# Annatk26/wire

Hardware: AMD Instinct MI355X
Metric: coord-samples/sec fwd+bwd, 4x256 complex WIRE MLP (higher is better)
Workload: dtype f32 (2xfp16 split operands with power-of-two scales, f16 MFMA, fp32 accumulate)

## Files before the change

wire_amd/csrc/wire_api.hip:

```cpp
#include <cmath>
#include <cstdarg>
#include <cstdio>
#include <string>

#include "wire_plan.h"

static thread_local std::string g_err;
int fail(int code, const char* fmt, ...) {
  char buf[512];
  va_list ap;
  va_start(ap, fmt);
  vsnprintf(buf, sizeof buf, fmt, ap);
  va_end(ap);
  g_err = buf;
  return code;
}
int wire_fail_(int code, const char* msg) { return fail(code, "%s", msg); }

extern "C" int wire_abi_version(void) { return WIRE_ABI_VERSION; }
extern "C" const char* wire_last_error(void) { return g_err.c_str(); }

std::mutex g_prof_mu;
std::atomic<bool> g_prof_on{false};
std::vector<ProfRec> g_prof_recs;
std::vector<std::pair<hipEvent_t, hipEvent_t>> g_prof_pool;

extern "C" int wire_prof_enable(int on) {
  std::lock_guard<std::mutex> lk(g_prof_mu);
  g_prof_on.store(on != 0);
  return WIRE_OK;
}
extern "C" int wire_prof_read(double* ms_total, int64_t* launches, double* flops_total) {
  std::lock_guard<std::mutex> lk(g_prof_mu);
  for (int i = 0; i < WIRE_PROF_CLASSES; ++i) { ms_total[i] = 0; launches[i] = 0; flops_total[i] = 0; }
  for (auto& r : g_prof_recs) {
    float ms = 0.f;
    if (hipEventSynchronize(r.b) == hipSuccess && hipEventElapsedTime(&ms, r.a, r.b) == hipSuccess) {
      ms_total[r.cls] += ms; launches[r.cls] += 1; flops_total[r.cls] += r.flops;
    }
    g_prof_pool.emplace_back(r.a, r.b);
  }
  g_prof_recs.clear();
  return WIRE_OK;
}

WireFamily wire_family_(int kind) {
  if (knob(K_SPLIT_BF16)) return FAM_X3;
  return (kind == WIRE_KIND_WIRE && knob(K_COMPLEX_3M)) ? FAM_3M : FAM_4M;
}
extern "C" int wire_tune_get(const char* key) {
  if (!key) return fail(WIRE_ERR_ARG, "null key");
  const int v = knob_get(key);
  return v >= 0 ? v : fail(WIRE_ERR_ARG, "unknown tuning key: %s", key);
}
extern "C" int wire_tune_set(const char* key, int value) {
  if (!key) return fail(WIRE_ERR_ARG, "null key");
  if (knob_set(key, value) == 0 || (g_glds_tune && g_glds_tune(key, value) == 0)) return WIRE_OK;
  return fail(WIRE_ERR_ARG, "unknown tuning key or bad value: %s=%d", key, value);
}

hipError_t layer_nt(hipStream_t s, const Plan& p, WireFamily f, const float* packed, int l, bool dg, int epi,
                    const float* A, int64_t n, GemmEpiParams ep, const unsigned* amax_a, const unsigned* amax_b,
                    unsigned* amax_out) {
  const int Pin = l == 0 ? p.Pin0 : p.P, Nc = dg ? Pin : p.Pl, Kd = dg ? p.Pl : Pin;
  switch (f) {
    case FAM_X2:
      ep.amax_a = amax_a; ep.amax_b = amax_b; ep.amax_out = amax_out;
      return launch_gemmx2h_nt(s, epi, A, Kd, packed + (dg ? p.off_dg_x2 : p.off_fwd_x2)[l], n, Nc, Kd, ep,
                               x2_waits(p.k_nt_bfirst, p.k_epi_early));
    case FAM_3M:
      return launch_gemm3m_nt(s, epi, A, Kd, packed + (dg ? p.off_dg_3m : p.off_fwd_3m)[l], Kd, n, Nc / 2, Kd / 2, ep);
    case FAM_X3: return launch_gemmx3_nt(s, epi, A, Kd, packed + (dg ? p.off_dg_x3 : p.off_fwd_x3)[l], n, Nc, Kd, ep);
    default: return launch_gemm_nt(s, epi, A, Kd, packed + (dg ? p.off_dg : p.off_fwd)[l], Kd, n, Nc, Kd, ep);
  }
}

int pack_hidden(hipStream_t s, const Plan& p, const void* const* params, float* packed, const std::vector<const float*>& hW,
                const std::vector<const float*>& hb) {
  for (int l0 = 1; l0 <= p.L; l0 += PACK_MAXB) {
    const int nb = (p.L - l0 + 1) < PACK_MAXB ? (p.L - l0 + 1) : PACK_MAXB;
    PackBatch pb{}, p3{};
    X3SplitBatch sf{}, sd{};
    for (int i = 0; i < nb; ++i) {
      const int l = l0 + i;
      pb.W[i] = hW[l];
      pb.b[i] = hb[l];
      pb.V[i] = p.per_layer == 4 ? (const float*)params[p.per_layer * l + 2] : nullptr;
      pb.c[i] = p.per_layer == 4 ? (const float*)params[p.per_layer * l + 3] : nullptr;
      pb.fwd[i] = packed + p.off_fwd[l]; pb.dg[i] = packed + p.off_dg[l]; pb.bias[i] = packed + p.off_bias[l];
      sf.src[i] = packed + p.off_fwd[l]; sf.dst[i] = packed + p.off_fwd_x3[l];
      sd.src[i] = packed + p.off_dg[l]; sd.dst[i] = packed + p.off_dg_x3[l];
      if (p.off_fwd_3m[l] >= 0) {
        p3.W[i] = pb.W[i]; p3.b[i] = pb.b[i];
        p3.fwd[i] = packed + p.off_fwd_3m[l]; p3.dg[i] = packed + p.off_dg_3m[l]; p3.bias[i] = packed + p.off_bias[l];
      }
    }
    HIPCHK(launch_pack_hidden_batch(s, p.kind, pb, nb, p.K, p.K, p.P, p.P, p.ws));
    if (p.Pl == p.P) {
      for (int i = 0; i < nb; ++i) { sf.src[nb + i] = sd.src[i]; sf.dst[nb + i] = sd.dst[i]; }
      HIPCHK(launch_x3_split_b_batch(s, sf, 2 * nb, p.P, p.Pl, p.P));
    } else {
      HIPCHK(launch_x3_split_b_batch(s, sf, nb, p.P, p.Pl, p.P));
      HIPCHK(launch_x3_split_b_batch(s, sd, nb, p.Pl, p.P, p.Pl));
    }
    if (p.off_fwd_3m[l0] >= 0)
      HIPCHK(launch_pack3m_batch(s, p3, nb, p.K, p.K, p.Kp, p.Kp));
    {
      X2AmaxBatch ab{};
      X2SplitBatch xf{}, xd{};
      for (int i = 0; i < nb; ++i) {
        const int l = l0 + i;
        unsigned* slots = reinterpret_cast<unsigned*>(packed + p.off_wamax + (int64_t)l * WIRE_AMAX_SLOTS);
        ab.src[i] = packed + p.off_fwd[l]; ab.slots[i] = slots;
        xf.src[i] = packed + p.off_fwd[l]; xf.dst[i] = packed + p.off_fwd_x2[l]; xf.slots[i] = slots;
        xd.src[i] = packed + p.off_dg[l]; xd.dst[i] = packed + p.off_dg_x2[l]; xd.slots[i] = slots;
      }
      HIPCHK(launch_amax_batch(s, ab, nb, (int64_t)p.Pl * p.P));
      HIPCHK(launch_x2_split_b_batch(s, xf, nb, p.P, p.Pl, p.P));
      HIPCHK(launch_x2_split_b_batch(s, xd, nb, p.Pl, p.P, p.Pl));
      for (int k = 0; k < p.S2 && p.off_fx >= 0 && fused_pre_scale(p.kind, p.w, pass_c(p, k)) > 0.f; ++k) {
        FxSplitBatch fx{};
        for (int i = 0; i < nb; ++i) {
          const int l = l0 + i;
          fx.src[i] = packed + p.off_fwd[l];
          fx.dst[i] = packed + fx_pass_off(p, k) + (int64_t)(l - 1) * fused_b_image_floats(p.P);
          fx.slots[i] = ab.slots[i];
        }
        HIPCHK(launch_fx_split_b_batch(s, fx, nb, p.P, p.P, fused_pre_scale(p.kind, p.w, pass_c(p, k))));
      }
      if (p.off_fxd >= 0) {
        FxSplitBatch fd{};
        int m = 0;
        for (int i = 0; i < nb; ++i) {
          const int l = l0 + i;
          fd.src[m] = packed + p.off_dg[l];
          fd.dst[m] = packed + p.off_fxd + (int64_t)(p.L - l) * fused_b_image_floats(p.P);
          fd.slots[m] = ab.slots[i];
          ++m;
        }
        if (m > 0) HIPCHK(launch_fx_split_b_batch(s, fd, m, p.Pl, p.P, 1.f));
      }
    }
  }
  return WIRE_OK;
}

extern "C" int wire_pack_params(void* stream, const wire_net_desc* d, const void* const* params,
                                float* packed) {
  Plan p; if (int rc = make_plan(d, p)) return rc;
  if (!params || !packed) return fail(WIRE_ERR_ARG, "null pointer");
  hipStream_t s = (hipStream_t)stream;
  ProfScope ps(s, 3, 0);
  for (int i = 0; i < p.ntens; ++i)
    if (!params[i]) return fail(WIRE_ERR_ARG, "params[%d] is null", i);
  HIPCHK(hipMemsetAsync(packed + p.off_wamax, 0, (size_t)(p.L + 1) * WIRE_AMAX_SLOTS * sizeof(float), s));
  if (p.first_gemm) {
    const float* W = (const float*)params[p.t0];
    const float* b = (const float*)params[p.t0 + 1];
    HIPCHK(launch_pack_hidden(s, p.kind, W, b, nullptr, nullptr, p.K, p.Din, p.P, p.Pin0, packed + p.off_fwd[0],
                              packed + p.off_dg[0], packed + p.off_bias[0]));
    HIPCHK(launch_x3_split_b(s, packed + p.off_fwd[0], p.Pin0, p.Pl, p.Pin0, packed + p.off_fwd_x3[0]));
    HIPCHK(launch_x3_split_b(s, packed + p.off_dg[0], p.Pl, p.Pin0, p.Pl, packed + p.off_dg_x3[0]));
    if (p.off_fx >= 0) {
      unsigned* slots0 = reinterpret_cast<unsigned*>(packed + p.off_wamax);
      HIPCHK(launch_amax(s, packed + p.off_fwd[0], (int64_t)p.Pl * p.Pin0, slots0));
      FxSplitBatch f0{};
      f0.src[0] = packed + p.off_fwd[0]; f0.dst[0] = packed + p.off_fx; f0.slots[0] = slots0;
      HIPCHK(launch_fx_split_b_batch(s, f0, 1, p.Pin0, p.P, 1.f, p.Pin0));
    }
    if (p.ms) {
      X2AmaxBatch ab{};
      X2SplitBatch xf{};
      ab.src[0] = xf.src[0] = packed + p.off_fwd[0];
      ab.slots[0] = reinterpret_cast<unsigned*>(packed + p.off_wamax);
      xf.dst[0] = packed + p.off_fwd_x2[0]; xf.slots[0] = ab.slots[0];
      HIPCHK(launch_amax_batch(s, ab, 1, (int64_t)p.Pl * p.Pin0));
      HIPCHK(launch_x2_split_b_batch(s, xf, 1, p.Pin0, p.Pl, p.Pin0));
    }
  }
  if (p.hier) return hier_pack(s, p, params, packed);
  if (p.mfn) return mfn_pack(s, p, params, packed);
  std::vector<const float*> hW(p.L + 1, nullptr), hb(p.L + 1, nullptr);
  for (int l = 1; l <= p.L; ++l) {
    hW[l] = (const float*)params[p.t0 + p.per_layer * l]; hb[l] = (const float*)params[p.t0 + p.per_layer * l + 1];
  }
  if (int rc = pack_hidden(s, p, params, packed, hW, hb)) return rc;
  HIPCHK(launch_pack_final(s, p.kind, (const float*)params[p.ntens - 2],
                           (const float*)params[p.ntens - 1], p.K, p.P, p.O, packed + p.off_wf,
                           packed + p.off_bf));
  if (!p.first_gemm || p.ms)
    for (int q = 0; q < p.per_layer; ++q) {
      if (q == 0 && p.ws != 1.f) {
        HIPCHK(launch_scale_copy(s, (const float*)params[first_tensor(p, 0)], p.tfloats[first_tensor(p, 0)], p.ws,
                                 packed + first_native_off(p, 0)));
        continue;
      }
      HIPCHK(hipMemcpyAsync(packed + first_native_off(p, q), params[first_tensor(p, q)], p.tfloats[first_tensor(p, q)] * 4,
                            hipMemcpyDeviceToDevice, s));
    }
  if (p.m2) {
    const M2Comb w = comb_of(p, packed);
    const float* dst[4] = {w.W1, w.b1, w.W2, w.b2};
    for (int q = 0; q < 4; ++q)
      HIPCHK(hipMemcpyAsync(const_cast<float*>(dst[q]), params[q], p.tfloats[q] * 4, hipMemcpyDeviceToDevice, s));
  }
  return WIRE_OK;
}

static FusedFwdParams fused_params(const Plan& p, const float* packed, const float* coords, int64_t n) {
  FusedFwdParams fp;
  fp.coords = coords; fp.n = n;
  if (p.first_gemm) {
    fp.pe_F = p.F; fp.bias0 = packed + p.off_bias[0]; fp.wamax0 = wamax_of(p, packed, 0);
  } else {
    fp.W0 = packed + first_native_off(p, 0); fp.b0 = packed + first_native_off(p, 1);
  }
  fp.wimg = reinterpret_cast<const unsigned char*>(packed + p.off_fx);
  fp.bias = packed + p.off_bias[1]; fp.bias_stride = p.L >= 2 ? p.off_bias[2] - p.off_bias[1] : 0;
  fp.wamax = wamax_of(p, packed, 1); fp.wamax_stride = WIRE_AMAX_SLOTS;
  fp.D = p.D; fp.K = p.K; fp.L = p.L; fp.O = p.O; fp.w1 = p.w1; fp.w = p.w; fp.s = p.s;
  fp.c_first = fused_pre_scale(p.kind, p.w1, p.s); fp.c_hidden = fused_pre_scale(p.kind, p.w, p.s);
  fp.k2_first = p.s * p.s * 1.44269502f / (fp.c_first * fp.c_first);
  fp.k2 = p.s * p.s * 1.44269502f / (fp.c_hidden * fp.c_hidden);
  return fp;
}

static int mlp_fwd_core(void* stream, const Plan& p, const Route& r, const float* packed, const float* coords, int64_t n,
                        float* y, void* act, int64_t act_bytes, const FusedFwdParams* loss = nullptr) {
  const bool save = r.mode != MODE_INFER;
  if (n < 0) return fail(WIRE_ERR_ARG, "negative n");
  if (n == 0) return WIRE_OK;
  if (!packed || !coords || (!r.fuse && !y) || !act) return fail(WIRE_ERR_ARG, "null pointer");
  const ActLayout a = act_layout(p, n, save);
  if (act_bytes < a.total * 4) return fail(WIRE_ERR_SIZE, "act buffer %lld < %lld bytes",
                                           (long long)act_bytes, (long long)a.total * 4);
  hipStream_t s = (hipStream_t)stream;
  float* A = (float*)act;
  if (r.fused_fwd) {
    FusedFwdParams fp = fused_params(p, packed, coords, n);
    fp.wf = packed + p.off_wf; fp.bfr = packed + p.off_bf; fp.y = y;
    if (p.m2) {
      for (int k = 0; k < p.S2; ++k) {
        FusedFwdParams f = fp;
        f.wimg = reinterpret_cast<const unsigned char*>(packed + fx_pass_off(p, k));
        f.s = pass_c(p, k);
        f.c_first = fused_pre_scale(p.kind, p.w1, f.s); f.c_hidden = fused_pre_scale(p.kind, p.w, f.s);
        f.y = A + a.ytr + (int64_t)k * n * p.O;
        ProfScope ps(s, 0, 2.0 * n * p.Pl * p.P * p.L);
        HIPCHK(launch_fused_fwd(s, p.kind, p.P, f));
      }
      ProfScope ps(s, 3, 0);
      HIPCHK(launch_m2_comb_fwd(s, comb_of(p, packed), p.S2, p.O, A + a.ytr, n, y));
      return WIRE_OK;
    }
    ProfScope ps(s, 0, 2.0 * n * p.Pl * p.P * p.L);
    HIPCHK(launch_fused_fwd(s, p.kind, p.P, fp));
    return WIRE_OK;
  }
  unsigned* const amax = reinterpret_cast<unsigned*>(A + a.amax);
  if (r.fam == FAM_X2)
    HIPCHK(hipMemsetAsync(amax, 0, (size_t)(p.L + 2 + (p.ms ? 1 : 0)) * WIRE_AMAX_SLOTS * sizeof(unsigned), s));
  unsigned* const pe_amax = reinterpret_cast<unsigned*>(A + a.pe_amax);
  if (p.ms) {
    MscaleC c{};
    for (int g = 0; g < p.T; ++g) c.c[g] = p.sc_c[g];
    ProfScope ps(s, 3, 0);
    HIPCHK(launch_mscale_first(s, coords, n, p.D, packed + first_native_off(p, 0), packed + first_native_off(p, 1), p.SHF,
                               c, p.ms_split, p.Pin0, r.pe_split,
                               r.fam0 == FAM_X2 && r.pe_split == 0.f ? pe_amax : nullptr, A + a.pe));
  } else if (p.first_gemm) {
    ProfScope ps(s, 3, 0);
    HIPCHK(launch_posenc(s, coords, n, p.D, p.F, p.Pin0, A + a.pe));
  }
  if (r.fused_train) {
    FusedFwdParams fp = fused_params(p, packed, coords, n);
    fp.inv_c_first = 1.f / fp.c_first; fp.inv_c_hidden = 1.f / fp.c_hidden;
    fp.lin0 = p.cplx ? nullptr : A + a.lin0;
    fp.lin = p.kind == WIRE_KIND_RELU ? nullptr : A + a.lin1; fp.lin_stride = a.np * p.Pl;
    fp.out = A + a.out0; fp.out_stride = a.np * p.P;
    fp.amax_out = amax;
    fp.rstore = r.rstore ? 1 : 0;
    if (r.fused_final) {
      fp.wf = packed + p.off_wf; fp.bfr = packed + p.off_bf;
      fp.target = loss->target; fp.idx = loss->idx; fp.first = loss->first; fp.gscale = loss->gscale;
      fp.y = loss->y; fp.rec = loss->rec; fp.g_lin = loss->g_lin; fp.part_w = loss->part_w; fp.part_b = loss->part_b;
      fp.loss_partial = loss->loss_partial; fp.amax_g = loss->amax_g;
    }
    ProfScope ps(s, 0, 2.0 * n * p.Pl * p.P * p.L);
    HIPCHK(launch_fused_fwd(s, p.kind, p.P, fp));
    return WIRE_OK;
  }
  auto out_l = [&](int l) { return save ? A + a.out0 + (int64_t)l * a.np * p.P : A + ((l & 1) ? a.pong : a.ping); };
  auto lin_l = [&](int l) -> float* {
    if (!save || p.kind == WIRE_KIND_RELU) return nullptr;
    return l == 0 ? A + a.lin0 : A + a.lin1 + (int64_t)(l - 1) * a.np * p.Pl;
  };
  auto at = [](float* b, int64_t off) -> float* { return b ? b + off : nullptr; };
  for (int k = 0; k < p.S2; ++k) {
    const float ck = pass_c(p, k);
    const int64_t ro = (int64_t)k * n;
    if (p.first_gemm) {
      GemmEpiParams ep; ep.bias = packed + p.off_bias[0]; ep.o0 = lin_l(0); ep.o1 = out_l(0);
      ep.ld0 = p.Pl; ep.ld1 = p.P; ep.omega = p.w1; ep.scale = p.s; ep.kvalid = p.K;
      if (r.fam == FAM_X2) ep.amax_out = amax;
      if (r.pe_split != 0.f) ep.a_split_inv = 1.f / r.pe_split;
      ProfScope ps(s, 0, 2.0 * n * p.Pl * p.Pin0);
      HIPCHK(layer_nt(s, p, r.fam0, packed, 0, false, epi_fwd(p.kind), A + a.pe, n, ep, pe_amax, wamax_of(p, packed, 0),
                      amax));
    } else {
      auto first = [&](int q) { return q < p.per_layer ? packed + first_native_off(p, q) : nullptr; };
      ProfScope ps(s, 3, 0);
      HIPCHK(launch_first_fwd(s, p.kind, coords, n, p.D, first(0), first(1), first(2), first(3), p.K, p.P, p.w1, ck,
                              p.cplx ? nullptr : at(lin_l(0), ro * p.P), out_l(0) + ro * p.P,
                              r.fam == FAM_X2 ? amax : nullptr));
    }
    for (int l = 1; l <= p.L; ++l) {
      GemmEpiParams ep; ep.bias = packed + p.off_bias[l]; ep.o0 = at(lin_l(l), ro * p.Pl); ep.o1 = out_l(l) + ro * p.P;
      ep.ld0 = p.Pl; ep.ld1 = p.P; ep.omega = p.w; ep.scale = ck; ep.kvalid = p.K;
      if (r.skip_out_L && l == p.L) ep.o1 = nullptr;
      const float s_in = r.out_scale[l - 1], s_out = r.out_scale[l];
      if (s_in != 0.f) ep.a_split_inv = 1.f / s_in;
      if (s_out != 0.f) ep.o1_split = s_out;
      ProfScope ps(s, 0, 2.0 * n * p.Pl * p.P);
      HIPCHK(layer_nt(s, p, r.fam, packed, l, false, epi_fwd(p.kind), out_l(l - 1) + ro * p.P, n, ep,
                      amax + (l - 1) * WIRE_AMAX_SLOTS, wamax_of(p, packed, l),
                      s_out != 0.f ? nullptr : amax + l * WIRE_AMAX_SLOTS));
    }
  }
  if (!r.fuse) {
    ProfScope ps(s, 3, 0);
    HIPCHK(launch_final_fwd(s, out_l(p.L), n * p.S2, p.P, p.O, packed + p.off_wf, packed + p.off_bf,
                            p.m2 ? A + a.ytr : y));
    if (p.m2 && r.mode != MODE_TRAIN) HIPCHK(launch_m2_comb_fwd(s, comb_of(p, packed), p.S2, p.O, A + a.ytr, n, y));
  }
  return WIRE_OK;
}

extern "C" int wire_mlp_fwd(void* stream, const wire_net_desc* d, const float* packed,
                            const float* coords, int64_t n, float* y, void* act, int64_t act_bytes,
                            int save_for_bwd) {
  Plan p; if (int rc = make_plan(d, p)) return rc;
  if (p.hier)
    return hier_fwd_core(stream, p, hier_route(p, n, save_for_bwd ? MODE_AUTOGRAD : MODE_INFER), packed, coords, n, y, act,
                         act_bytes);
  if (p.mfn)
    return mfn_fwd_core(stream, p, mfn_route(p, n, save_for_bwd ? MODE_AUTOGRAD : MODE_INFER), packed, coords, n, y, act,
                        act_bytes);
  return mlp_fwd_core(stream, p, make_route(p, n, save_for_bwd ? MODE_AUTOGRAD : MODE_INFER), packed, coords, n, y, act,
                      act_bytes);
}

namespace {
struct Bwd {
  const Plan& p; const Route& r; hipStream_t s;
  const float* packed; const float* coords; int64_t n;
  int64_t n1;
  const float* g_y;
  void* const* grads;
  float* g_coords; wire_grad_ready_fn ready; void* user;
  ActLayout a; ScratchLayout sc; CoordLayout cl;
  const float* A; float* Sx;
  float* gcur = nullptr; float* gnext = nullptr;
  int chain_rows = 0;

  const float* out_l(int l) const { return A + a.out0 + (int64_t)l * a.np * p.P; }
  const float* lin_l(int l) const { return l == 0 ? A + a.lin0 : A + a.lin1 + (int64_t)(l - 1) * a.np * p.Pl; }
  const float* first(int q) const { return packed + first_native_off(p, q); }
  unsigned* gslots(int l) const { return reinterpret_cast<unsigned*>(Sx + sc.gamax) + l * WIRE_AMAX_SLOTS; }
  const unsigned* oslots(int l) const { return reinterpret_cast<const unsigned*>(A + a.amax) + l * WIRE_AMAX_SLOTS; }
  float* grad(int t) const { return grads ? (float*)grads[t] : nullptr; }
  void done(int t, int count) const { if (ready) ready(user, t, count); }
  int64_t crp_set() const { return (int64_t)prereduce_room(colreduce_blocks(n)) * p.ldu * 5; }
  int final_stage();
  int first_point();
  int chain();
  int wgrad_batch();
  int layers();
  int coords_grad();
  int first_params();
  hipError_t hidden_tn(int l);
};

int Bwd::final_stage() {
  ProfScope ps(s, 3, 0);
  if (!r.fuse) {
    const float wL = (p.L == 0) ? p.w1 : p.w;
    if (p.L == 0 && p.cplx)
      HIPCHK(launch_final_bwd(s, p.kind, 1, g_y, n, p.O, packed + p.off_wf, nullptr, out_l(0), p.K, p.P, wL, p.s, gcur,
                              Sx + sc.fpw, Sx + sc.fpb));
    else
      for (int k = 0; k < p.S2; ++k) {
        const int64_t ro = (int64_t)k * n1, bo = (int64_t)k * final_bwd_blocks(n1);
        HIPCHK(launch_final_bwd(s, p.kind, 0, g_y + ro * p.O, n1, p.O, packed + p.off_wf, lin_l(p.L) + ro * p.Pl,
                                out_l(p.L) + ro * p.P, p.K, p.P, wL, pass_c(p, k), gcur + ro * p.P,
                                Sx + sc.fpw + bo * p.O * p.P, Sx + sc.fpb + bo * p.O,
                                r.fam == FAM_X2 ? gslots(p.L) : nullptr));
      }
    if (!grads) return WIRE_OK;
  }
  const int nbf = r.fused_final ? (int)((n + 127) / 128) : p.S2 * final_bwd_blocks(n1);
  HIPCHK(launch_final_reduce(s, p.kind, Sx + sc.fpw, Sx + sc.fpb, nbf, p.O, p.K, p.P, grad(p.ntens - 2),
                             grad(p.ntens - 1)));
  done(p.ntens - 2, 2);
  return WIRE_OK;
}

int Bwd::first_point() {
  ProfScope ps(s, 3, 0);
  if (p.kind == WIRE_KIND_WIRE)
    HIPCHK(launch_gabor_bwd_first_point(s, gcur, out_l(0), coords, p.D, first(0), first(1), n, p.K, p.P, p.w1, p.s,
                                        Sx + sc.gu, p.ldu));
  else
    HIPCHK(launch_gabor2d_bwd_first_point(s, gcur, out_l(0), coords, p.D, first(0), first(1), first(2), first(3), n, p.K,
                                          p.P, p.w1, p.s, Sx + sc.gu, p.ldu));
  return WIRE_OK;
}

int Bwd::chain() {
  const bool relu = p.kind == WIRE_KIND_RELU;
  FusedBwdParams bp;
  bp.n = n;
  bp.g = Sx + sc.gch; bp.g_stride = sc.gch_stride;
  bp.gamax = gslots(0);
  bp.aux = relu ? A + a.out0 : A + a.lin1 - a.np * p.Pl;
  bp.aux_stride = relu ? a.np * p.P : a.np * p.Pl;
  bp.wimg = reinterpret_cast<const unsigned char*>(packed + p.off_fxd);
  bp.wamax = wamax_of(p, packed, 1); bp.wamax_stride = WIRE_AMAX_SLOTS;
  bp.L = p.L; bp.w = p.w; bp.s = p.s;
  bp.rstore = r.rstore ? 1 : 0; bp.c_hidden = fused_pre_scale(p.kind, p.w, p.s);
  bp.aux0 = relu ? A + a.out0 : A + a.lin0;
  bp.w1 = p.w1;
  if (!p.first_gemm) { bp.coords = coords; bp.D = p.D; bp.crp = Sx + sc.crp; bp.C = p.K; }
  if (p.m2) {
    bp.n = n1;
    for (int k = 0; k < p.S2; ++k) {
      const int64_t ro = (int64_t)k * n1;
      FusedBwdParams b = bp;
      b.g = bp.g + ro * p.P; b.aux = bp.aux + ro * p.P; b.aux0 = bp.aux0 + ro * p.P;
      b.s = pass_c(p, k); b.c_hidden = fused_pre_scale(p.kind, p.w, pass_c(p, k));
      if (k > 0) b.crp = bp.crp + (int64_t)k * ((n1 + chain_rows - 1) / chain_rows) * p.K * 5;
      ProfScope ps(s, 1, 2.0 * n1 * p.Pl * p.P * p.L);
      HIPCHK(launch_fused_bwd(s, p.kind, p.P, b, &chain_rows));
    }
    return WIRE_OK;
  }
  ProfScope ps(s, 1, 2.0 * n * p.Pl * p.P * p.L);
  HIPCHK(launch_fused_bwd(s, p.kind, p.P, bp, &chain_rows));
  return WIRE_OK;
}

int Bwd::wgrad_batch() {
  const int l0 = r.wb_l0, nb = r.wb_n;
  const bool rs = r.rstore;
  const float s_z = rs ? 0.f : r.out_scale[l0 - 1];
  ProfScope ps(s, 2, 2.0 * n * p.Pl * p.P * nb);
  HIPCHK(launch_gemmx2_tn(s, Sx + sc.gch + l0 * sc.gch_stride, p.Pl, rs ? lin_l(l0 - 1) : out_l(l0 - 1), rs ? p.Pl : p.P,
                          n, p.Pl, p.P, r.wb_S, Sx + sc.slab, Sx + sc.bslab, gslots(l0), oslots(l0 - 1),
                          rs ? 1.f / 16384.f : (s_z != 0.f ? 1.f / s_z : 0.f), rs ? known_kind(p.kind).z_act : 0,
                          nb, sc.gch_stride, rs ? a.np * p.Pl : a.np * p.P, WIRE_AMAX_SLOTS));
  return WIRE_OK;
}

hipError_t Bwd::hidden_tn(int l) {
  const int S = r.tn_S;
  float* slab = Sx + sc.slab;
  float* bslab = Sx + sc.bslab;
  switch (r.tn_fam) {
    case FAM_3M: return launch_gemm3m_tn(s, gcur, p.P, out_l(l - 1), p.P, n, p.Kp, p.Kp, S, slab, bslab);
    case FAM_X2:
      if (r.rstore)
        return launch_gemmx2_tn(s, gcur, p.Pl, lin_l(l - 1), p.Pl, n, p.Pl, p.P, S, slab, bslab, gslots(l), nullptr,
                                1.f / 16384.f, known_kind(p.kind).z_act);
      return launch_gemmx2_tn(s, gcur, p.Pl, out_l(l - 1), p.P, n, p.Pl, p.P, S, slab, bslab, gslots(l), oslots(l - 1),
                              r.out_scale[l - 1] != 0.f ? 1.f / r.out_scale[l - 1] : 0.f);
    case FAM_X3: return launch_gemmx3_tn(s, gcur, p.Pl, out_l(l - 1), p.P, n, p.Pl, p.P, S, slab, bslab);
    default: return launch_gemm_tn(s, gcur, p.Pl, out_l(l - 1), p.P, n, p.Pl, p.P, S, slab, bslab);
  }
}

int Bwd::layers() {
  const int pl = p.per_layer;
  for (int l = p.L; l >= 1; --l) {
    if (r.chain) gcur = Sx + sc.gch + (int64_t)l * sc.gch_stride;
    if (grads) {
      const bool own = l < r.wb_l0;
      if (own) {
        ProfScope ps(s, 2, 2.0 * n * p.Pl * p.P);
        HIPCHK(hidden_tn(l));
      }
      const int S = own ? r.tn_S : r.wb_S;
      const int64_t m = own ? 0 : l - r.wb_l0;
      float* const slab = Sx + sc.slab + m * S * p.Pl * p.P;
      float* const bslab = Sx + sc.bslab + m * S * p.Pl;
      auto g = [&](int q) { return q < pl ? grad(p.t0 + pl * l + q) : nullptr; };
      ProfScope ps(s, 3, 0);
      if (r.tn_fam == FAM_3M)
        HIPCHK(launch_wgrad3m_reduce(s, slab, bslab, S, p.K, p.K, p.Kp, p.Kp, g(0), g(1)));
      else
        HIPCHK(launch_wgrad_reduce(s, p.kind, slab, bslab, S, p.K, p.K, p.Pl, p.P, g(0), g(1), g(2), g(3), p.ws));
      done(p.t0 + pl * l, pl);
    }
    if (r.chain) continue;
    const bool first_sums = grads && r.first_sums;
    GemmEpiParams ep;
    ep.scale = p.s; ep.kvalid = p.K; ep.ld1 = p.P; ep.i1 = out_l(l - 1);
    int epi;
    if (l > 1 || !p.cplx) {
      epi = epi_bwd(p.kind);
      ep.omega = (l - 1 == 0) ? p.w1 : p.w;
      ep.i0 = lin_l(l - 1); ep.o0 = gnext; ep.ld0 = p.Pl;
      ep.recompute_out = r.recompute_out && l >= 2;
      ep.lookahead = r.bwd_lookahead && ep.recompute_out;
      if (l == 1 && first_sums) { ep.coords = coords; ep.D = p.D; ep.cr_partial = Sx + sc.crp; ep.cr_C = p.K; }
    } else {
      epi = (p.kind == WIRE_KIND_WIRE) ? EPI_GABOR_BWD_FIRST : EPI_GABOR2D_BWD_FIRST;
      ep.omega = p.w1;
      ep.coords = coords; ep.D = p.D; ep.ldu = p.ldu; ep.o0 = Sx + sc.gu;
      if (first_sums) { ep.cr_partial = Sx + sc.crp; ep.cr_C = p.K; ep.cr_set = crp_set(); }
      ep.recompute_out = r.recompute_out0;
      ep.first_dn = r.first_dn;
      ep.W0 = first(0); ep.b0 = first(1);
      if (pl == 4) { ep.W0b = first(2); ep.b0b = first(3); }
    }
    if (!p.cplx && l == 1) ep.ld0 = p.P;
    if (l == 1 && g_coords && r.cg_epi) {
      ep.cg_partial = Sx + cl.cgp; ep.D = p.D;
      if (!p.cplx) ep.W0 = first(0);
    }
    for (int k = 0; k < p.S2; ++k) {
      const int64_t ro = (int64_t)k * n1;
      GemmEpiParams e = ep;
      if (k > 0) { e.scale = pass_c(p, k); e.i0 += ro * p.Pl; e.i1 += ro * p.P; e.o0 += ro * e.ld0; }
      ProfScope ps(s, 1, 2.0 * n1 * p.Pl * p.P);
      HIPCHK(layer_nt(s, p, r.fam, packed, l, true, epi, gcur + ro * p.Pl, n1, e, gslots(l), wamax_of(p, packed, l),
                      l >= 2 || r.tn0 == FAM_X2 ? gslots(l - 1) : nullptr));
    }
    float* t = gcur; gcur = gnext; gnext = t;
  }
  return WIRE_OK;
}

int Bwd::coords_grad() {
  if (!g_coords) return WIRE_OK;
  const float* gu = Sx + sc.gu;
  if (r.cg_epi) {
    HIPCHK(launch_coordgrad_reduce(s, Sx + cl.cgp, cl.ntiles, n, p.D, g_coords));
  } else if (p.kind == WIRE_KIND_WIRE) {
    HIPCHK(launch_coordgrad_rows(s, gu, p.ldu, nullptr, first(0), nullptr, p.K, p.D, n, g_coords));
  } else if (p.kind == WIRE_KIND_WIRE2D) {
    HIPCHK(launch_coordgrad_rows(s, gu, 2 * p.ldu, gu + p.ldu, first(0), first(2), p.K, p.D, n, g_coords));
  } else if (p.m2) {
    HIPCHK(launch_coordgrad_rows(s, gcur, p.P, nullptr, first(0), nullptr, p.K, p.D, n, Sx + cl.cgp));
    HIPCHK(launch_m2_sum_passes(s, Sx + cl.cgp, p.S2, n1, p.D, g_coords));
  } else if (!p.first_gemm) {
    HIPCHK(launch_coordgrad_rows(s, gcur, p.P, nullptr, first(0), nullptr, p.K, p.D, n, g_coords));
  } else {
    GemmEpiParams ep;
    ep.o0 = Sx + cl.gpe; ep.ld0 = p.Pin0;
    HIPCHK(layer_nt(s, p, FAM_4M, packed, 0, true, EPI_STORE, gcur, n, ep));
    HIPCHK(launch_posenc_bwd(s, coords, n, p.D, p.F, Sx + cl.gpe, p.Pin0, g_coords));
  }
  return WIRE_OK;
}

int Bwd::first_params() {
  if (!grads) return WIRE_OK;
  float* const crp = Sx + sc.crp;
  if (p.cplx) {
    const float* gu = Sx + sc.gu;
    if (r.first_sums) {
      HIPCHK(launch_colreduce_final(s, p.K, p.D, n, crp, grad(0), grad(1)));
      if (p.kind == WIRE_KIND_WIRE2D) HIPCHK(launch_colreduce_final(s, p.K, p.D, n, crp + crp_set(), grad(2), grad(3)));
    } else if (p.kind == WIRE_KIND_WIRE) {
      HIPCHK(launch_colreduce(s, gu, p.ldu, p.K, coords, p.D, n, crp, grad(0), grad(1)));
    } else {
      HIPCHK(launch_colreduce(s, gu, 2 * p.ldu, p.K, coords, p.D, n, crp, grad(0), grad(1)));
      HIPCHK(launch_colreduce(s, gu + p.ldu, 2 * p.ldu, p.K, coords, p.D, n, crp, grad(2), grad(3)));
    }
  } else if (!p.first_gemm && r.chain) {
    HIPCHK(launch_colreduce_final_blocks(s, p.K, p.D, p.S2 * (int)((n1 + chain_rows - 1) / chain_rows), crp, grad(p.t0),
                                         grad(p.t0 + 1), p.ws));
  } else if (!p.first_gemm && r.first_sums) {
    HIPCHK(launch_colreduce_final(s, p.K, p.D, n, crp, grad(0), grad(1), p.ws));
  } else if (!p.first_gemm) {
    HIPCHK(launch_colreduce(s, gcur, p.P, p.K, coords, p.D, n, crp, grad(p.t0), grad(p.t0 + 1), p.ws));
  } else if (r.tn0 == FAM_X2) {
    const int S = gemmx2_tn_splits(n, p.P, p.Pin0, sc.S);
    HIPCHK(launch_gemmx2_tn(s, gcur, p.P, A + a.pe, p.Pin0, n, p.P, p.Pin0, S, Sx + sc.slab, Sx + sc.bslab, gslots(0),
                            nullptr, 1.f / r.pe_split));
    HIPCHK(launch_wgrad_reduce(s, p.kind, Sx + sc.slab, Sx + sc.bslab, S, p.K, p.Din, p.P, p.Pin0, grad(p.t0),
                               grad(p.t0 + 1), nullptr, nullptr));
  } else {
    const float* g0 = r.chain ? Sx + sc.gch : gcur;
    const bool x3 = r.tn0 == FAM_X3;
    const int S = x3 ? gemmx3_tn_splits(n, p.P, p.Pin0, sc.S) : gemm_tn_splits(n, p.P, p.Pin0, sc.S);
    HIPCHK(x3 ? launch_gemmx3_tn(s, g0, p.P, A + a.pe, p.Pin0, n, p.P, p.Pin0, S, Sx + sc.slab, Sx + sc.bslab)
              : launch_gemm_tn(s, g0, p.P, A + a.pe, p.Pin0, n, p.P, p.Pin0, S, Sx + sc.slab, Sx + sc.bslab));
    HIPCHK(launch_wgrad_reduce(s, p.kind, Sx + sc.slab, Sx + sc.bslab, S, p.K, p.Din, p.P, p.Pin0, grad(p.t0),
                               grad(p.t0 + 1), nullptr, nullptr));
  }
  done(p.t0, p.per_layer);
  if (p.ms) done(0, 2);
  return WIRE_OK;
}
}

static int mlp_bwd_core(void* stream, const Plan& p, const Route& r, const float* packed, const float* coords, int64_t n,
                        const float* g_y, const void* act, int64_t act_bytes, void* scratch, int64_t scratch_bytes,
                        void* const* grads, wire_grad_ready_fn ready = nullptr, void* user = nullptr,
                        float* g_coords = nullptr, bool comb_done = false) {
  if (n <= 0) return fail(WIRE_ERR_ARG, "backward needs n > 0");
  if (!packed || !coords || (!r.fuse && !g_y && !comb_done) || !act || !scratch || (!grads && !g_coords))
    return fail(WIRE_ERR_ARG, "null pointer");
  if (grads)
    for (int i = p.ms ? p.t0 : 0; i < p.ntens; ++i) if (!grads[i]) return fail(WIRE_ERR_ARG, "grads[%d] is null", i);
  if (p.ms && g_coords) return fail(WIRE_ERR_ARG, "no coordinate gradient through the frozen first stage of kind %d",
                                    (int)WIRE_KIND_BSPLINE_MS);
  Bwd c{p, r, (hipStream_t)stream, packed, coords, n * p.S2, n, g_y, grads, g_coords, ready, user, act_layout(p, n, 1),
        scratch_layout(p, n), coord_layout(p, n), (const float*)act, (float*)scratch};
  const int64_t need = g_coords ? c.cl.total : c.sc.total;
  if (act_bytes < c.a.total * 4) return fail(WIRE_ERR_SIZE, "act buffer too small");
  if (scratch_bytes < need * 4) return fail(WIRE_ERR_SIZE, "scratch %lld < %lld bytes",
                                            (long long)scratch_bytes, (long long)need * 4);
  c.gcur = c.Sx + c.sc.ga;
  c.gnext = c.Sx + c.sc.gb;
  if (p.m2) {
    ProfScope ps(c.s, 3, 0);
    float* const part = c.Sx + c.sc.cpart;
    if (!comb_done)
      HIPCHK(launch_m2_comb_bwd(c.s, comb_of(p, packed), p.S2, p.O, c.A + c.a.ytr, n, M2Loss{}, g_y, c.Sx + c.sc.gtr,
                                grads ? part : nullptr, nullptr));
    if (r.chain) c.gcur = c.Sx + c.sc.gch + (int64_t)p.L * c.sc.gch_stride;
    if (grads) {
      HIPCHK(launch_m2_comb_reduce(c.s, part, n, p.S2, p.O,
                                   M2Grads{c.grad(0), c.grad(1), c.grad(2), c.grad(3)}));
      c.done(0, 4);
      for (int k = 0; k < p.S2 && !r.chain; ++k)
        HIPCHK(hipMemcpyAsync(c.Sx + c.sc.crep + (int64_t)k * n * p.D, coords, (size_t)n * p.D * sizeof(float),
                              hipMemcpyDeviceToDevice, c.s));
      if (!r.chain) c.coords = c.Sx + c.sc.crep;
    }
    c.g_y = c.Sx + c.sc.gtr;
  }
  if (r.fam == FAM_X2 && !r.fuse)
    HIPCHK(hipMemsetAsync(c.gslots(0), 0, (size_t)(p.L + 2) * WIRE_AMAX_SLOTS * sizeof(unsigned), c.s));
  int rc = c.final_stage();
  if (!rc && p.L == 0 && p.cplx) rc = c.first_point();
  if (!rc && r.chain) rc = c.chain();
  if (!rc && r.wb_n > 0) rc = c.wgrad_batch();
  if (!rc) rc = c.layers();
  if (rc) return rc;
  ProfScope ps(c.s, 3, 0);
  rc = c.coords_grad();
  return rc ? rc : c.first_params();
}

extern "C" int wire_mlp_bwd(void* stream, const wire_net_desc* d, const float* packed,
                            const float* coords, int64_t n, const float* g_y, const void* act,
                            int64_t act_bytes, void* scratch, int64_t scratch_bytes,
                            void* const* grads) {
  Plan p; if (int rc = make_plan(d, p)) return rc;
  if (!grads) return fail(WIRE_ERR_ARG, "null pointer");
  if (p.hier)
    return hier_bwd_core(stream, p, hier_route(p, n, MODE_AUTOGRAD), packed, coords, n, g_y, act, act_bytes, scratch,
                         scratch_bytes, grads, nullptr, nullptr, nullptr);
  if (p.mfn)
    return mfn_bwd_core(stream, p, mfn_route(p, n, MODE_AUTOGRAD), packed, coords, n, g_y, act, act_bytes, scratch,
                        scratch_bytes, grads, nullptr, nullptr, nullptr);
  return mlp_bwd_core(stream, p, make_route(p, n, MODE_AUTOGRAD), packed, coords, n, g_y, act, act_bytes, scratch,
                      scratch_bytes, grads);
}

extern "C" int wire_mlp_bwd_coords(void* stream, const wire_net_desc* d, const float* packed, const float* coords,
                                   int64_t n, const float* g_y, const void* act, int64_t act_bytes, void* scratch,
                                   int64_t scratch_bytes, void* const* grads_host, float* g_coords) {
  Plan p; if (int rc = make_plan(d, p)) return rc;
  if (!grads_host && !g_coords) return fail(WIRE_ERR_ARG, "wire_mlp_bwd_coords: neither grads_host nor g_coords");
  if (p.hier)
    return hier_bwd_core(stream, p, hier_route(p, n, MODE_AUTOGRAD), packed, coords, n, g_y, act, act_bytes, scratch,
                         scratch_bytes, grads_host, nullptr, nullptr, g_coords);
  if (p.mfn)
    return mfn_bwd_core(stream, p, mfn_route(p, n, MODE_AUTOGRAD), packed, coords, n, g_y, act, act_bytes, scratch,
                        scratch_bytes, grads_host, nullptr, nullptr, g_coords);
  return mlp_bwd_core(stream, p, make_route(p, n, MODE_AUTOGRAD), packed, coords, n, g_y, act, act_bytes, scratch,
                      scratch_bytes, grads_host, nullptr, nullptr, g_coords);
}

extern "C" int wire_train_fwd_bwd_hooked(void* stream, const wire_net_desc* d, const float* packed,
                                         const float* coords, int64_t n, const float* target, const int64_t* idx,
                                         int64_t first, float weight, float* y, float* g_y, float* loss_out,
                                         float* rec, float* partial, void* act, int64_t act_bytes, void* scratch,
                                         int64_t scratch_bytes, void* const* grads, wire_grad_ready_fn ready,
                                         void* user) {
  Plan p; if (int rc = make_plan(d, p)) return rc;
  if (n <= 0) return fail(WIRE_ERR_ARG, "wire_train_fwd_bwd needs n > 0");
  if (!target || !y || !g_y || !loss_out || !partial) return fail(WIRE_ERR_ARG, "null pointer");
  hipStream_t s = (hipStream_t)stream;
  if (p.hier) {
    const Route hr = hier_route(p, n, MODE_TRAIN);
    const HierScratch sc = hier_scratch(p, n);
    if (!scratch || scratch_bytes < sc.total * 4) return fail(WIRE_ERR_SIZE, "scratch too small");
    float* Sx = (float*)scratch;
    const double inv_no = 1.0 / ((double)n * (double)p.O);
    M2Loss ls;
    ls.target = target; ls.idx = idx; ls.first = first; ls.gscale = (float)(weight * 2.0 * inv_no);
    ls.y = y; ls.g_y = g_y; ls.rec = rec;
    if (int rc = hier_fwd_core(stream, p, hr, packed, coords, n, y, act, act_bytes, &ls, Sx + sc.lpart)) return rc;
    { ProfScope ps(s, 3, 0);
      HIPCHK(launch_mse_final(s, Sx + sc.lpart, hier_head_blocks(n), (float)(weight * inv_no), loss_out)); }
    return hier_bwd_core(stream, p, hr, packed, coords, n, g_y, act, act_bytes, scratch, scratch_bytes, grads, ready, user,
                         nullptr);
  }
  if (p.mfn) {
    const Route mr = mfn_route(p, n, MODE_TRAIN);
    if (int rc = mfn_fwd_core(stream, p, mr, packed, coords, n, y, act, act_bytes)) return rc;
    { ProfScope ps(s, 3, 0);
      HIPCHK(launch_mse_grad(s, y, target, idx, first, n, p.O, weight, g_y, loss_out, rec, partial)); }
    return mfn_bwd_core(stream, p, mr, packed, coords, n, g_y, act, act_bytes, scratch, scratch_bytes, grads, ready, user,
                        nullptr);
  }
  const Route r = make_route(p, n, MODE_TRAIN);
  if (p.m2) {
    const ScratchLayout sc = scratch_layout(p, n);
    if (!scratch || scratch_bytes < sc.total * 4) return fail(WIRE_ERR_SIZE, "scratch too small");
    if (!act || act_bytes < act_layout(p, n, 1).total * 4) return fail(WIRE_ERR_SIZE, "act buffer too small");
    if (int rc = mlp_fwd_core(stream, p, r, packed, coords, n, y, act, act_bytes)) return rc;
    float* Sx = (float*)scratch;
    const int nblk = m2_comb_blocks(n);
    float* const loss_part = Sx + sc.cpart + (int64_t)nblk * m2_comb_grad_floats(p.S2, p.O);
    const double inv_no = 1.0 / ((double)n * (double)p.O);
    M2Loss ls;
    ls.target = target; ls.idx = idx; ls.first = first; ls.gscale = (float)(weight * 2.0 * inv_no);
    ls.y = y; ls.g_y = g_y; ls.rec = rec;
    { ProfScope ps(s, 3, 0);
      HIPCHK(launch_m2_comb_bwd(s, comb_of(p, packed), p.S2, p.O, (const float*)act + act_layout(p, n, 1).ytr, n, ls,
                                nullptr, Sx + sc.gtr, Sx + sc.cpart, loss_part));
      HIPCHK(launch_mse_final(s, loss_part, nblk, (float)(weight * inv_no), loss_out)); }
    return mlp_bwd_core(stream, p, r, packed, coords, n, nullptr, act, act_bytes, scratch, scratch_bytes, grads, ready, user,
                        nullptr, true);
  }
  if (!r.fuse) {
    if (int rc = mlp_fwd_core(stream, p, r, packed, coords, n, y, act, act_bytes)) return rc;
    { ProfScope ps(s, 3, 0);
      HIPCHK(launch_mse_grad(s, y, target, idx, first, n, p.O, weight, g_y, loss_out, rec, partial)); }
    return mlp_bwd_core(stream, p, r, packed, coords, n, g_y, act, act_bytes, scratch, scratch_bytes, grads, ready, user);
  }
  const ActLayout a = act_layout(p, n, 1);
  const ScratchLayout sc = scratch_layout(p, n);
  if (!scratch || scratch_bytes < sc.total * 4) return fail(WIRE_ERR_SIZE, "scratch too small");
  const float* A = (const float*)act;
  float* Sx = (float*)scratch;
  unsigned* const gamax = reinterpret_cast<unsigned*>(Sx + sc.gamax);
  if (r.fam == FAM_X2) HIPCHK(hipMemsetAsync(gamax, 0, (size_t)(p.L + 2) * WIRE_AMAX_SLOTS * sizeof(unsigned), s));
  float* gL = r.chain ? Sx + sc.gch + (int64_t)p.L * sc.gch_stride : Sx + sc.ga;
  FusedFwdParams lp;
  const int fblocks = (int)((n + 127) / 128);
  const double inv_no = 1.0 / ((double)n * (double)p.O);
  lp.target = target; lp.idx = idx; lp.first = first; lp.gscale = (float)(weight * 2.0 * inv_no);
  lp.y = y; lp.rec = rec; lp.g_lin = gL; lp.part_w = Sx + sc.fpw; lp.part_b = Sx + sc.fpb; lp.loss_partial = Sx + sc.crp;
  lp.amax_g = gamax + p.L * WIRE_AMAX_SLOTS;
  if (int rc = mlp_fwd_core(stream, p, r, packed, coords, n, nullptr, act, act_bytes, &lp)) return rc;
  if (r.fused_final) {
    ProfScope ps(s, 3, 0);
    HIPCHK(launch_mse_final(s, Sx + sc.crp, fblocks, (float)(weight * inv_no), loss_out));
  } else {
    ProfScope ps(s, 3, 0);
    const float* linL = p.kind == WIRE_KIND_RELU ? nullptr : A + a.lin1 + (int64_t)(p.L - 1) * a.np * p.Pl;
    HIPCHK(launch_final_fused(s, p.kind, r.skip_out_L ? nullptr : A + a.out0 + (int64_t)p.L * a.np * p.P, linL, n, p.P,
                              p.O, p.K, packed + p.off_wf, packed + p.off_bf, target, idx, first, weight,
                              p.w, p.s, y, rec, gL, Sx + sc.fpw, Sx + sc.fpb, Sx + sc.crp, loss_out,
                              r.fam == FAM_X2 ? gamax + p.L * WIRE_AMAX_SLOTS : nullptr));
  }
  return mlp_bwd_core(stream, p, r, packed, coords, n, nullptr, act, act_bytes, scratch, scratch_bytes, grads, ready, user);
}
extern "C" int wire_train_fwd_bwd(void* stream, const wire_net_desc* d, const float* packed,
                                  const float* coords, int64_t n, const float* target, const int64_t* idx,
                                  int64_t first, float weight, float* y, float* g_y, float* loss_out,
                                  float* rec, float* partial, void* act, int64_t act_bytes, void* scratch,
                                  int64_t scratch_bytes, void* const* grads) {
  return wire_train_fwd_bwd_hooked(stream, d, packed, coords, n, target, idx, first, weight, y, g_y, loss_out, rec, partial,
                                   act, act_bytes, scratch, scratch_bytes, grads, nullptr, nullptr);
}
```

wire_amd/csrc/wire_final.hip:

```cpp
#include "wire_dev.h"
#include "wire_point.h"

__global__ __launch_bounds__(256) void final_fwd_kernel(const float* __restrict__ z, long long n,
                                                        int P, int O, const float* __restrict__ wf,
                                                        const float* __restrict__ bfr,
                                                        float* __restrict__ y) {
  extern __shared__ __attribute__((aligned(16))) float swf[];
  for (int i = threadIdx.x; i < O * P; i += blockDim.x) swf[i] = wf[i];
  __syncthreads();
  const int lane = threadIdx.x & 63;
  const int wave = threadIdx.x >> 6;
  const long long wstride = (long long)gridDim.x * 4;
  for (long long row = (long long)blockIdx.x * 4 + wave; row < n; row += wstride) {
    float acc[WIRE_MAXO];
#pragma unroll
    for (int o = 0; o < WIRE_MAXO; ++o) acc[o] = 0.f;
    const float* zr = z + row * P;
    for (int c = lane * 4; c < P; c += 256) {
      const f32x4 zv = *reinterpret_cast<const f32x4*>(zr + c);
#pragma unroll
      for (int o = 0; o < WIRE_MAXO; ++o)
        if (o < O) {
          const f32x4 wv = *reinterpret_cast<const f32x4*>(&swf[o * P + c]);
          acc[o] += zv[0] * wv[0] + zv[1] * wv[1] + zv[2] * wv[2] + zv[3] * wv[3];
        }
    }
#pragma unroll
    for (int o = 0; o < WIRE_MAXO; ++o)
      if (o < O) {
        float v = acc[o];
#pragma unroll
        for (int sft = 32; sft >= 1; sft >>= 1) v += __shfl_xor(v, sft);
        if (lane == o) y[row * O + o] = v + bfr[o];
      }
  }
}

hipError_t launch_final_fwd(hipStream_t s, const float* z, int64_t n, int P, int O,
                            const float* wf, const float* bfr, float* y) {
  if (n <= 0) return hipSuccess;
  if (O > WIRE_MAXO || (P & 3) || (int64_t)O * P > WIRE_FINAL_MAX_OP) return hipErrorInvalidValue;
  unsigned grid = cdiv(n, 4);
  if (grid > 4096) grid = 4096;
  hipLaunchKernelGGL(final_fwd_kernel, dim3(grid), dim3(256), (size_t)O * P * sizeof(float), s, z,
                     (long long)n, P, O, wf, bfr, y);
  return hipGetLastError();
}

int final_bwd_blocks(int64_t n) { return (int)((n + WIRE_FB_ROWS - 1) / WIRE_FB_ROWS); }

template <int KIND, bool RAW>
__global__ __launch_bounds__(256) void final_bwd_kernel(
    const float* __restrict__ g_y, long long n, int O, const float* __restrict__ wf,
    const float* __restrict__ lin, const float* __restrict__ out, int K, int P, float omega,
    float scale, float* __restrict__ g_lin, float* __restrict__ part_w,
    float* __restrict__ part_b, unsigned* __restrict__ amax_g) {
  constexpr bool cplx = (KIND == NK_WIRE || KIND == NK_WIRE2D);
  __shared__ float sgy[WIRE_FB_ROWS * WIRE_MAXO];
  float amx = 0.f;
  const long long r0 = (long long)blockIdx.x * WIRE_FB_ROWS;
  long long r1 = r0 + WIRE_FB_ROWS;
  if (r1 > n) r1 = n;
  const int nr = (int)(r1 - r0);
  for (int i = threadIdx.x; i < nr * O; i += blockDim.x) sgy[i] = g_y[r0 * O + i];
  __syncthreads();

  const int nfeat = cplx ? (P >> 1) : P;
  const int f = blockIdx.y * blockDim.x + threadIdx.x;
  if (f < nfeat) {
    const int c0 = cplx ? blk_col(f, 0) : f;
    float w0[WIRE_MAXO], w1[WIRE_MAXO], a0[WIRE_MAXO], a1[WIRE_MAXO];
#pragma unroll
    for (int o = 0; o < WIRE_MAXO; ++o) {
      w0[o] = 0.f; w1[o] = 0.f; a0[o] = 0.f; a1[o] = 0.f;
      if (o < O) {
        w0[o] = wf[(size_t)o * P + c0];
        if (cplx) w1[o] = wf[(size_t)o * P + c0 + 32];
      }
    }
    const float m2s2 = -2.f * scale * scale;
    const int Pl = (KIND == NK_WIRE2D) ? 2 * P : P;
    const int lc = (KIND == NK_WIRE2D) ? (((f >> 5) << 7) + (f & 31)) : c0;
    constexpr int RB = 8;
    for (int rb = 0; rb < nr; rb += RB) {
      float pr[RB], pi[RB], l0[RB], l1[RB], l2[RB], l3[RB];
#pragma unroll
      for (int q = 0; q < RB; ++q) {
        const int r = rb + q < nr ? rb + q : nr - 1;
        const long long row = r0 + r;
        pr[q] = out[row * P + c0];
        pi[q] = cplx ? out[row * P + c0 + 32] : 0.f;
        l0[q] = l1[q] = l2[q] = l3[q] = 0.f;
        if (!RAW) {
          if (KIND == NK_WIRE2D) {
            const float* L = lin + row * Pl + lc;
            l0[q] = L[0]; l1[q] = L[32]; l2[q] = L[64]; l3[q] = L[96];
          } else if (KIND != NK_RELU) {
            l0[q] = lin[row * P + c0];
            if (KIND == NK_WIRE) l1[q] = lin[row * P + c0 + 32];
          }
        }
      }
#pragma unroll
      for (int q = 0; q < RB; ++q) {
        const int r = rb + q;
        if (r < nr) {
          const long long row = r0 + r;
          float gr = 0.f, gi = 0.f;
#pragma unroll
          for (int o = 0; o < WIRE_MAXO; ++o)
            if (o < O) {
              const float g = sgy[r * O + o];
              gr = __builtin_fmaf(g, w0[o], gr);
              if (cplx) gi = __builtin_fmaf(g, w1[o], gi);
              a0[o] = __builtin_fmaf(g, pr[q], a0[o]);
              if (cplx) a1[o] = __builtin_fmaf(g, pi[q], a1[o]);
            }
          if (RAW) {
            g_lin[row * P + c0] = gr;
            if (cplx) g_lin[row * P + c0 + 32] = gi;
          } else if (KIND == NK_WIRE) {
            float gl_re, gl_im;
            gabor_bwd(gr, gi, l0[q], l1[q], pr[q], pi[q], omega, m2s2, gl_re, gl_im);
            g_lin[row * P + c0] = gl_re;
            g_lin[row * P + c0 + 32] = gl_im;
            amx = __builtin_fmaxf(amx, __builtin_fmaxf(__builtin_fabsf(gl_re), __builtin_fabsf(gl_im)));
          } else if (KIND == NK_WIRE2D) {
            const float c_r = __builtin_fmaf(pr[q], gr, pi[q] * gi);
            const float c_i = __builtin_fmaf(pr[q], gi, -(pi[q] * gr));
            const float t = m2s2 * c_r;
            float* Gp = g_lin + row * Pl + lc;
            const float g0 = __builtin_fmaf(t, l0[q], omega * c_i), g1 = __builtin_fmaf(t, l1[q], -(omega * c_r));
            const float g2 = t * l2[q], g3 = t * l3[q];
            Gp[0] = g0; Gp[32] = g1; Gp[64] = g2; Gp[96] = g3;
            amx = __builtin_fmaxf(amx, __builtin_fmaxf(__builtin_fmaxf(__builtin_fabsf(g0), __builtin_fabsf(g1)),
                                                       __builtin_fmaxf(__builtin_fabsf(g2), __builtin_fabsf(g3))));
          } else {
            constexpr int ACT = nk_real_act(KIND);
            const float gl = real_act_bwd<ACT>(gr, l0[q], pr[q], omega, scale);
            g_lin[row * P + c0] = gl;
            amx = __builtin_fmaxf(amx, __builtin_fabsf(gl));
          }
        }
      }
    }
    float* pw = part_w + (size_t)blockIdx.x * O * P;
#pragma unroll
    for (int o = 0; o < WIRE_MAXO; ++o)
      if (o < O) {
        pw[(size_t)o * P + c0] = a0[o];
        if (cplx) pw[(size_t)o * P + c0 + 32] = a1[o];
      }
  }
  if (blockIdx.y == 0 && threadIdx.x < O) {
    float sacc = 0.f;
    for (int r = 0; r < nr; ++r) sacc += sgy[r * O + threadIdx.x];
    part_b[(size_t)blockIdx.x * O + threadIdx.x] = sacc;
  }
  if (amax_g) wire_amax_publish(amax_g, amx, threadIdx.x & 63);
}

hipError_t launch_final_bwd(hipStream_t s, int kind, int raw, const float* g_y, int64_t n, int O,
                            const float* wf, const float* lin, const float* out, int K, int P,
                            float omega, float scale, float* g_lin, float* part_w,
                            float* part_b, unsigned* amax_g) {
  if (n <= 0) return hipSuccess;
  if (O > WIRE_MAXO) return hipErrorInvalidValue;
  const bool cplx = kind_is_cplx(kind);
  const int nfeat = cplx ? P / 2 : P;
  dim3 grid((unsigned)final_bwd_blocks(n), cdiv(nfeat, 256));
#define FB_LAUNCH(KK, RR)                                                                        \
  hipLaunchKernelGGL((final_bwd_kernel<KK, RR>), grid, dim3(256), 0, s, g_y, (long long)n, O, wf, \
                     lin, out, K, P, omega, scale, g_lin, part_w, part_b, amax_g)
  if (raw) {
    if (cplx) FB_LAUNCH(NK_WIRE, true); else FB_LAUNCH(NK_RELU, true);
    return hipGetLastError();
  }
  return with_kind(kind, [&](auto k) -> hipError_t {
    FB_LAUNCH(decltype(k)::value, false);
    return hipGetLastError();
  });
#undef FB_LAUNCH
}

#define FF_MAXO 4
#define FF_MAXPASS 2
#define FF_MAXROWS 512
static size_t final_fused_shm(int P, int O) {
  return ((size_t)4 * O * P + 4 * (FF_MAXO + 1) + (size_t)FF_MAXROWS * FF_MAXO) * sizeof(float) + (size_t)FF_MAXROWS * 8;
}
bool final_fused_supported(int P, int O) {
  return (P % 64) == 0 && P <= 512 * FF_MAXPASS && O <= FF_MAXO && final_fused_shm(P, O) <= 65536;
}

WIRE_DEVINL void ff_amax4(float& m, const f32x4& v) {
  m = __builtin_fmaxf(m, __builtin_fmaxf(__builtin_fmaxf(__builtin_fabsf(v[0]), __builtin_fabsf(v[1])),
                                         __builtin_fmaxf(__builtin_fabsf(v[2]), __builtin_fabsf(v[3]))));
}
template <int NPASS, int KIND, bool RECOMP, int OT, int RPW>
__global__ __launch_bounds__(256) void final_fused_kernel(
    const float* __restrict__ out, const float* __restrict__ lin, long long n, int P, int O, int kvalid,
    const float* __restrict__ wf, const float* __restrict__ bfr, const float* __restrict__ target,
    const int64_t* __restrict__ idx, long long first, float gscale, float omega, float scale,
    float* __restrict__ y, float* __restrict__ rec, float* __restrict__ g_lin, float* __restrict__ part_w,
    float* __restrict__ part_b, float* __restrict__ loss_partial, int rows_pb, unsigned* __restrict__ amax_g) {
  static_assert(!RECOMP || KIND != NK_RELU, "relu keeps out and has no lin to recompute it from");
  float amx = 0.f;
  static_assert(RPW == 1 || (RPW == 2 && NPASS == 1), "two rows per wave slot: one pass of at most 256 columns");
  constexpr int RL = 64 / RPW;
  constexpr bool HAS_LIN = (KIND != NK_RELU);
  constexpr int NL = (KIND == NK_WIRE2D) ? 4 : 2;
  extern __shared__ float sm[];
  const int lane = threadIdx.x & 63, wave = threadIdx.x >> 6;
  const int sub = lane / RL, lr_ = lane & (RL - 1);
  const int ngrp = P >> 6;
  const int Pl = (KIND == NK_WIRE2D) ? 2 * P : P;
  const long long r0 = (long long)blockIdx.x * rows_pb;
  long long r1 = r0 + rows_pb;
  if (r1 > n) r1 = n;
  const float m2s2 = -2.f * scale * scale;

  int col[NPASS], lcol[NPASS];
  bool live[NPASS];
  f32x4 wre[NPASS][OT], wim[NPASS][OT];
  f32x4 are[NPASS][OT], aim[NPASS][OT];
#pragma unroll
  for (int ps = 0; ps < NPASS; ++ps) {
    const int g = (lr_ >> 3) + 8 * ps;
    live[ps] = g < ngrp;
    col[ps] = (g << 6) + 4 * (lr_ & 7);
    lcol[ps] = (KIND == NK_WIRE2D) ? (g << 7) + 4 * (lr_ & 7) : col[ps];
#pragma unroll
    for (int o = 0; o < OT; ++o) {
      const f32x4 z4 = {0.f, 0.f, 0.f, 0.f};
      wre[ps][o] = z4; wim[ps][o] = z4; are[ps][o] = z4; aim[ps][o] = z4;
      if (live[ps] && o < O) {
        wre[ps][o] = *reinterpret_cast<const f32x4*>(wf + (size_t)o * P + col[ps]);
        wim[ps][o] = *reinterpret_cast<const f32x4*>(wf + (size_t)o * P + col[ps] + 32);
      }
    }
  }
  float bsum[OT];
#pragma unroll
  for (int o = 0; o < OT; ++o) bsum[o] = 0.f;
  float lsum = 0.f;

  float* s_tg = sm + (size_t)4 * O * P + 4 * (FF_MAXO + 1);
  long long* s_src = reinterpret_cast<long long*>(s_tg + FF_MAXROWS * FF_MAXO);
  for (int t = threadIdx.x; t < rows_pb; t += 256) {
    const long long grow = r0 + t;
    if (grow < r1) {
      const long long src = idx ? idx[grow] : first + grow;
      s_src[t] = src;
#pragma unroll
      for (int o = 0; o < OT; ++o)
        if (o < O) s_tg[t * FF_MAXO + o] = target[src * O + o];
    }
  }
  __syncthreads();

  constexpr int PF = RECOMP ? 3 : 2;
  f32x4 nzr[PF][NPASS], nzi[PF][NPASS], nl[PF][NPASS][NL];
  auto load_row = [&](const int slot, long long row) {
    row += sub;
#pragma unroll
    for (int ps = 0; ps < NPASS; ++ps) {
      const f32x4 z4 = {0.f, 0.f, 0.f, 0.f};
      nzr[slot][ps] = z4; nzi[slot][ps] = z4;
#pragma unroll
      for (int c = 0; c < NL; ++c) nl[slot][ps][c] = z4;
      if (live[ps] && row < r1) {
        if (!RECOMP) {
          const size_t o_ = (size_t)row * P + col[ps];
          nzr[slot][ps] = *reinterpret_cast<const f32x4*>(out + o_);
          nzi[slot][ps] = *reinterpret_cast<const f32x4*>(out + o_ + 32);
        }
        if (HAS_LIN) {
          const float* Lp = lin + (size_t)row * Pl + lcol[ps];
#pragma unroll
          for (int c = 0; c < NL; ++c) nl[slot][ps][c] = *reinterpret_cast<const f32x4*>(Lp + 32 * c);
        }
      }
    }
  };
  auto process = [&](const long long row_slot, f32x4 (&zr)[NPASS], f32x4 (&zi)[NPASS],
                     const f32x4 (&ll)[NPASS][NL]) {
    const long long row = row_slot + sub;
    const bool rl = row < r1;
    if (RECOMP && (KIND == NK_WIRE || KIND == NK_WIRE2D)) {
      const float w0l2e = omega * 1.44269502f, ns2l2e = -(scale * scale) * 1.44269502f;
#pragma unroll
      for (int ps = 0; ps < NPASS; ++ps) {
        const int f0 = ((col[ps] >> 6) << 5) + (col[ps] & 31);
#pragma unroll
        for (int j = 0; j < 4; ++j) {
          float a_, b_;
          if (KIND == NK_WIRE2D)
            gabor2d_fwd_lean(ll[ps][0][j], ll[ps][1][j], ll[ps][NL - 2][j], ll[ps][NL - 1][j], omega, scale, a_, b_);
          else
            gabor_fwd_lean(ll[ps][0][j], ll[ps][1][j], omega, w0l2e, ns2l2e, a_, b_);
          const bool valid = live[ps] && f0 + j < kvalid;
          zr[ps][j] = valid ? a_ : 0.f;
          zi[ps][j] = valid ? b_ : 0.f;
        }
      }
    } else if (RECOMP) {
      constexpr int ACT = nk_real_act(KIND);
#pragma unroll
      for (int ps = 0; ps < NPASS; ++ps)
#pragma unroll
        for (int j = 0; j < 4; ++j) {
          const float a_ = real_act_fwd_lean<ACT>(ll[ps][0][j], omega, scale);
          const float b_ = real_act_fwd_lean<ACT>(ll[ps][1][j], omega, scale);
          zr[ps][j] = (live[ps] && col[ps] + j < kvalid) ? a_ : 0.f;
          zi[ps][j] = (live[ps] && col[ps] + 32 + j < kvalid) ? b_ : 0.f;
        }
    }
    float yo[OT];
#pragma unroll
    for (int o = 0; o < OT; ++o) {
      float acc = 0.f;
#pragma unroll
      for (int ps = 0; ps < NPASS; ++ps)
#pragma unroll
        for (int j = 0; j < 4; ++j)
          acc = __builtin_fmaf(zr[ps][j], wre[ps][o][j], __builtin_fmaf(zi[ps][j], wim[ps][o][j], acc));
      yo[o] = acc;
    }
#pragma unroll
    for (int o = 0; o < OT; ++o)
      if (o < O) {
#pragma unroll
        for (int sft = RL / 2; sft >= 1; sft >>= 1) yo[o] += __shfl_xor(yo[o], sft);
      }
    const int lrow = rl ? (int)(row - r0) : 0;
    const long long src = s_src[lrow];
    float gy[OT];
#pragma unroll
    for (int o = 0; o < OT; ++o) {
      gy[o] = 0.f;
      if (o < O) {
        const float yy = yo[o] + bfr[o];
        const float dlt = rl ? yy - s_tg[lrow * FF_MAXO + o] : 0.f;
        gy[o] = gscale * dlt;
        if (lr_ == o && rl) {
          y[row * O + o] = yy;
          if (rec) rec[src * O + o] = yy;
        }
        lsum = __builtin_fmaf(dlt, dlt, lsum);
        bsum[o] += gy[o];
      }
    }
#pragma unroll
    for (int ps = 0; ps < NPASS; ++ps) {
      if (!live[ps] || !rl) continue;
      f32x4 gr = {0.f, 0.f, 0.f, 0.f}, gi = {0.f, 0.f, 0.f, 0.f};
#pragma unroll
      for (int o = 0; o < OT; ++o)
        if (o < O) {
          gr += gy[o] * wre[ps][o];
          gi += gy[o] * wim[ps][o];
          are[ps][o] += gy[o] * zr[ps];
          aim[ps][o] += gy[o] * zi[ps];
        }
      float* Gp = g_lin + (size_t)row * Pl + lcol[ps];
      if (KIND == NK_WIRE) {
        f32x4 glr, gli;
#pragma unroll
        for (int j = 0; j < 4; ++j) {
          float a_, b_;
          gabor_bwd(gr[j], gi[j], ll[ps][0][j], ll[ps][1][j], zr[ps][j], zi[ps][j], omega, m2s2, a_, b_);
          glr[j] = a_; gli[j] = b_;
        }
        *reinterpret_cast<f32x4*>(Gp) = glr;
        *reinterpret_cast<f32x4*>(Gp + 32) = gli;
        ff_amax4(amx, glr); ff_amax4(amx, gli);
      } else if (KIND == NK_WIRE2D) {
        f32x4 g0, g1, g2, g3;
#pragma unroll
        for (int j = 0; j < 4; ++j) {
          const float c_r = __builtin_fmaf(zr[ps][j], gr[j], zi[ps][j] * gi[j]);
          const float c_i = __builtin_fmaf(zr[ps][j], gi[j], -(zi[ps][j] * gr[j]));
          const float t = m2s2 * c_r;
          g0[j] = __builtin_fmaf(t, ll[ps][0][j], omega * c_i);
          g1[j] = __builtin_fmaf(t, ll[ps][1][j], -(omega * c_r));
          g2[j] = t * ll[ps][NL - 2][j];
          g3[j] = t * ll[ps][NL - 1][j];
        }
        *reinterpret_cast<f32x4*>(Gp) = g0;
        *reinterpret_cast<f32x4*>(Gp + 32) = g1;
        *reinterpret_cast<f32x4*>(Gp + 64) = g2;
        *reinterpret_cast<f32x4*>(Gp + 96) = g3;
        ff_amax4(amx, g0); ff_amax4(amx, g1); ff_amax4(amx, g2); ff_amax4(amx, g3);
      } else {
        constexpr int ACT = nk_real_act(KIND);
        f32x4 glr, gli;
#pragma unroll
        for (int j = 0; j < 4; ++j) {
          glr[j] = real_act_bwd<ACT>(gr[j], ll[ps][0][j], zr[ps][j], omega, scale);
          gli[j] = real_act_bwd<ACT>(gi[j], ll[ps][1][j], zi[ps][j], omega, scale);
        }
        *reinterpret_cast<f32x4*>(Gp) = glr;
        *reinterpret_cast<f32x4*>(Gp + 32) = gli;
        ff_amax4(amx, glr); ff_amax4(amx, gli);
      }
    }
  };
#pragma unroll
  for (int d = 0; d < PF; ++d) load_row(d, r0 + (wave + 4 * d) * RPW);
  for (long long row = r0 + wave * RPW; row < r1; row += 4 * RPW * PF) {
#pragma unroll
    for (int d = 0; d < PF; ++d) {
      const long long rr_ = row + 4 * RPW * d;
      if (rr_ < r1) {
        f32x4 zr[NPASS], zi[NPASS], ll[NPASS][NL];
#pragma unroll
        for (int ps = 0; ps < NPASS; ++ps) {
          zr[ps] = nzr[d][ps]; zi[ps] = nzi[d][ps];
#pragma unroll
          for (int c = 0; c < NL; ++c) ll[ps][c] = nl[d][ps][c];
        }
        load_row(d, rr_ + 4 * RPW * PF);
        process(rr_, zr, zi, ll);
      }
    }
  }

  float* swf = sm;
  float* sb = sm + 4 * O * P;
  if (RPW == 2) {
#pragma unroll
    for (int o = 0; o < OT; ++o) {
#pragma unroll
      for (int ps = 0; ps < NPASS; ++ps)
#pragma unroll
        for (int j = 0; j < 4; ++j) {
          are[ps][o][j] += __shfl_xor(are[ps][o][j], 32);
          aim[ps][o][j] += __shfl_xor(aim[ps][o][j], 32);
        }
      bsum[o] += __shfl_xor(bsum[o], 32);
    }
    lsum += __shfl_xor(lsum, 32);
  }
#pragma unroll
  for (int ps = 0; ps < NPASS; ++ps)
    if (live[ps] && sub == 0)
#pragma unroll
      for (int o = 0; o < OT; ++o)
        if (o < O) {
          *reinterpret_cast<f32x4*>(swf + ((size_t)wave * O + o) * P + col[ps]) = are[ps][o];
          *reinterpret_cast<f32x4*>(swf + ((size_t)wave * O + o) * P + col[ps] + 32) = aim[ps][o];
        }
  if (lane == 0) {
#pragma unroll
    for (int o = 0; o < OT; ++o) sb[wave * (FF_MAXO + 1) + o] = bsum[o];
    sb[wave * (FF_MAXO + 1) + FF_MAXO] = lsum;
  }
  __syncthreads();
  float* pw = part_w + (size_t)blockIdx.x * O * P;
  for (int e = threadIdx.x; e < O * P; e += 256)
    pw[e] = (swf[e] + swf[O * P + e]) + (swf[2 * O * P + e] + swf[3 * O * P + e]);
  if (threadIdx.x < O)
    part_b[(size_t)blockIdx.x * O + threadIdx.x] =
        (sb[threadIdx.x] + sb[(FF_MAXO + 1) + threadIdx.x]) +
        (sb[2 * (FF_MAXO + 1) + threadIdx.x] + sb[3 * (FF_MAXO + 1) + threadIdx.x]);
  if (threadIdx.x == 0)
    loss_partial[blockIdx.x] = (sb[FF_MAXO] + sb[(FF_MAXO + 1) + FF_MAXO]) +
                               (sb[2 * (FF_MAXO + 1) + FF_MAXO] + sb[3 * (FF_MAXO + 1) + FF_MAXO]);
  if (amax_g) wire_amax_publish(amax_g, amx, lane);
}

hipError_t launch_final_fused(hipStream_t s, int kind, const float* out, const float* lin, int64_t n, int P, int O,
                              int kvalid, const float* wf, const float* bfr, const float* target, const int64_t* idx,
                              int64_t first, float weight, float omega, float scale, float* y, float* rec,
                              float* g_lin, float* part_w, float* part_b, float* loss_partial,
                              float* loss_out, unsigned* amax_g) {
  if (n <= 0) return hipSuccess;
  if (!final_fused_supported(P, O)) return hipErrorInvalidValue;
  if (!out && kind == NK_RELU) return hipErrorInvalidValue;
  const int nbf = final_bwd_blocks(n);
  int rows_pb = WIRE_FB_ROWS;
  if (nbf > 768) {
    rows_pb = (int)((n + 767) / 768);
    rows_pb = (rows_pb + 7) & ~7;
    if (rows_pb > FF_MAXROWS) rows_pb = FF_MAXROWS;
  }
  const int nblk = (int)((n + rows_pb - 1) / rows_pb);
  if (nblk < nbf) {
    hipError_t e = hipMemsetAsync(part_w + (size_t)nblk * O * P, 0, (size_t)(nbf - nblk) * O * P * sizeof(float), s);
    if (e == hipSuccess) e = hipMemsetAsync(part_b + (size_t)nblk * O, 0, (size_t)(nbf - nblk) * O * sizeof(float), s);
    if (e != hipSuccess) return e;
  }
  const float inv = (float)(1.0 / ((double)n * (double)O));
  const size_t shm = final_fused_shm(P, O);
#define FF_LAUNCH(NP, RW, KD, RC, OT)                                                                        \
  hipLaunchKernelGGL((final_fused_kernel<NP, KD, RC, OT, RW>), dim3((unsigned)nblk), dim3(256), shm, s, out, \
                     lin, (long long)n, P, O, kvalid, wf, bfr, target, idx, (long long)first,                \
                     weight * 2.f * inv, omega, scale, y, rec, g_lin, part_w, part_b, loss_partial, rows_pb, amax_g)
#define FF_LAUNCH_O(NP, RW, KD, RC)                                                                          \
  switch (O) {                                                                                               \
    case 1: FF_LAUNCH(NP, RW, KD, RC, 1); break;                                                             \
    case 2: case 3: FF_LAUNCH(NP, RW, KD, RC, 3); break;                                                     \
    default: FF_LAUNCH(NP, RW, KD, RC, 4); break;                                                            \
  }
#define FF_LAUNCH_K(NP, RW)                                                                                  \
  if constexpr (KD == NK_RELU) { FF_LAUNCH_O(NP, RW, KD, false); }                                           \
  else if (out) { FF_LAUNCH_O(NP, RW, KD, false); } else { FF_LAUNCH_O(NP, RW, KD, true); }
  const hipError_t err = with_kind(kind, [&](auto k) -> hipError_t {
    constexpr int KD = decltype(k)::value;
    if (P <= 256) { FF_LAUNCH_K(1, 2) } else if (P <= 512) { FF_LAUNCH_K(1, 1) } else { FF_LAUNCH_K(2, 1) }
    return hipSuccess;
  });
  if (err != hipSuccess) return err;
#undef FF_LAUNCH_K
#undef FF_LAUNCH_O
#undef FF_LAUNCH
  return launch_mse_final(s, loss_partial, nblk, weight * inv, loss_out);
}
```

wire_amd/csrc/wire_knobs.h:

```cpp
#pragma once
#include <atomic>

enum Knob {
  K_COMPLEX_3M, K_SPLIT_BF16, K_SPLIT_F16, K_SPLIT_OUT, K_RECOMPUTE_OUT, K_FIRST_SUMS, K_FIRST_DN, K_BWD_LOOKAHEAD, K_FUSED_RSTORE, K_WGRAD_BATCH,
  K_FUSED_FWD, K_FUSED_TRAIN, K_FUSED_TRAIN_P384, K_FUSED_FINAL, K_FUSED_BWD, K_FUSED_BWD_W,
  K_NT_BK, K_X2_AMODE, K_NT_BFIRST, K_EPI_EARLY, K_X2_TN_ROWS, K_X2_TN_P384, K_X3_TALL, K_X3_TALL_REAL, K_X3_TN_TALL, K_X3_TN16, K_X3_H16,
  K_X3H_STAGGER,
  K_FX_ABLATE, K_FXB_ABLATE, K_TN_ABL,
  K_COUNT
};

extern std::atomic<int> g_knob[K_COUNT];
inline int knob(Knob k) { return g_knob[k].load(std::memory_order_relaxed); }

int knob_get(const char* key);
int knob_set(const char* key, int value);
```

wire_amd/csrc/wire_knobs.hip:

```cpp
#include <cerrno>
#include <climits>
#include <cstdio>
#include <cstdlib>
#include <cstring>
#include <string>

#include "wire_knobs.h"

std::atomic<int> g_knob[K_COUNT];

namespace {
struct KnobDef {
  Knob id;
  const char* key;
  const char* env;
  int dflt;
  bool flag;
  int lo, hi;
  int a, b;
};
constexpr KnobDef flag_knob(Knob id, const char* key, const char* env, int dflt) { return {id, key, env, dflt, true, 0, 1, -1, -1}; }
constexpr KnobDef range_knob(Knob id, const char* key, const char* env, int dflt, int lo, int hi, int a = -1) {
  return {id, key, env, dflt, false, lo, hi, a, -1};
}
constexpr KnobDef choice_knob(Knob id, const char* key, const char* env, int dflt, int a, int b) { return {id, key, env, dflt, false, 1, 0, a, b}; }
constexpr bool accepts(const KnobDef& d, int v) {
  return d.flag || (d.lo <= v && v <= d.hi) || (v >= 0 && (v == d.a || v == d.b));
}
#ifdef WIRE_FX_ABLATE
#define FX_ABLATE_KEY(k) k
#else
#define FX_ABLATE_KEY(k) nullptr
#endif

constexpr KnobDef kKnobs[] = {
    flag_knob(K_COMPLEX_3M, "complex_3m", nullptr, 1),
    flag_knob(K_SPLIT_BF16, "split_bf16", "WIRE_SPLIT_BF16", 1),
    flag_knob(K_SPLIT_F16, "split_f16", "WIRE_SPLIT_F16", 1),
    flag_knob(K_SPLIT_OUT, "split_out", "WIRE_SPLIT_OUT", 1),
    flag_knob(K_RECOMPUTE_OUT, "recompute_out", "WIRE_RECOMPUTE_OUT", 1),
    flag_knob(K_FIRST_SUMS, "first_sums", "WIRE_FIRST_SUMS", 1),
    flag_knob(K_FIRST_DN, "first_dn", "WIRE_FIRST_DN", 1),
    flag_knob(K_BWD_LOOKAHEAD, "bwd_lookahead", "WIRE_BWD_LOOKAHEAD", 1),
    flag_knob(K_FUSED_RSTORE, "fused_rstore", "WIRE_FUSED_RSTORE", 1),
    flag_knob(K_WGRAD_BATCH, "wgrad_batch", "WIRE_WGRAD_BATCH", 1),
    range_knob(K_FUSED_FWD, "fused_fwd", "WIRE_FUSED_FWD", 1, 0, 1),
    range_knob(K_FUSED_TRAIN, "fused_train", "WIRE_FUSED_TRAIN", 1, 0, 1),
    flag_knob(K_FUSED_TRAIN_P384, "fused_train_p384", "WIRE_FUSED_TRAIN_P384", 0),
    range_knob(K_FUSED_FINAL, "fused_final", "WIRE_FUSED_FINAL", 0, 0, 1),
    range_knob(K_FUSED_BWD, "fused_bwd", "WIRE_FUSED_BWD", 1, 0, 1),
    choice_knob(K_FUSED_BWD_W, "fused_bwd_w", "WIRE_FUSED_BWD_W", 8, 4, 8),
    choice_knob(K_NT_BK, "nt_bk", "WIRE_NT_BK", 16, 16, 32),
    range_knob(K_X2_AMODE, "x2_amode", "WIRE_X2_AMODE", 2, 0, 2),
    flag_knob(K_NT_BFIRST, "nt_bfirst", "WIRE_NT_BFIRST", 1),
    flag_knob(K_EPI_EARLY, "epi_early", "WIRE_EPI_EARLY", 1),
    range_knob(K_X2_TN_ROWS, "x2_tn_rows", "WIRE_X2_TN_ROWS", 0, 256, INT_MAX, 0),
    choice_knob(K_X2_TN_P384, "x2_tn_p384", "WIRE_X2_TN_P384", 8, 6, 8),
    range_knob(K_X3_TALL, "x3_tall", "WIRE_X3_TALL", 1, 0, 1),
    range_knob(K_X3_TALL_REAL, "x3_tall_real", "WIRE_X3_TALL_REAL", 0, 0, 1),
    range_knob(K_X3_TN_TALL, "x3_tn_tall", "WIRE_X3_TN_TALL", 0, 0, 1),
    range_knob(K_X3_TN16, "x3_tn16", "WIRE_X3_TN16", 1, 0, 1),
    range_knob(K_X3_H16, "x3_h16", "WIRE_X3_H16", 15, 0, 15),
    range_knob(K_X3H_STAGGER, "x3h_stagger", "WIRE_X3H_STAGGER", 0, 0, INT_MAX),
    range_knob(K_FX_ABLATE, FX_ABLATE_KEY("fx_ablate"), nullptr, 0, 0, 15),
    range_knob(K_FXB_ABLATE, FX_ABLATE_KEY("fxb_ablate"), nullptr, 0, 0, 127),
    range_knob(K_TN_ABL, nullptr, "WIRE_TN_ABL", 0, 0, 15),
};

constexpr bool rows_valid() {
  for (int i = 0; i < K_COUNT; ++i)
    if (kKnobs[i].id != i || !accepts(kKnobs[i], kKnobs[i].dflt)) return false;
  return true;
}
static_assert(sizeof kKnobs / sizeof kKnobs[0] == K_COUNT && rows_valid(), "one row per Knob, in enum order, default accepted");

const KnobDef* find(const char* key) {
  for (const KnobDef& d : kKnobs)
    if (d.key && !strcmp(d.key, key)) return &d;
  return nullptr;
}
std::string accepted(const KnobDef& d) {
  if (d.flag) return "any integer, 0 = off";
  std::string s;
  for (const int v : {d.a, d.b})
    if (v >= 0) s += (s.empty() ? "" : " or ") + std::to_string(v);
  if (d.lo <= d.hi) s += (s.empty() ? "" : " or ") + std::to_string(d.lo) + (d.hi == INT_MAX ? ".." : ".." + std::to_string(d.hi));
  return s;
}
int from_env(const KnobDef& d) {
  const char* s = d.env ? getenv(d.env) : nullptr;
  if (!s) return d.dflt;
  char* end = nullptr;
  errno = 0;
  const long v = strtol(s, &end, 10);
  if (end != s && *end == '\0' && errno == 0 && v >= INT_MIN && v <= INT_MAX && accepts(d, (int)v))
    return d.flag ? v != 0 : (int)v;
  fprintf(stderr, "libwire_hip: ignoring %s=%s (accepted: %s); using the default %d\n", d.env, s, accepted(d).c_str(), d.dflt);
  return d.dflt;
}
struct KnobLoader {
  KnobLoader() {
    for (const KnobDef& d : kKnobs) g_knob[d.id].store(from_env(d), std::memory_order_relaxed);
  }
} g_knob_loader;
}

int knob_get(const char* key) {
  const KnobDef* d = find(key);
  return d ? knob(d->id) : -1;
}
int knob_set(const char* key, int value) {
  const KnobDef* d = find(key);
  if (!d || !accepts(*d, value)) return -1;
  g_knob[d->id].store(d->flag ? value != 0 : value, std::memory_order_relaxed);
  return 0;
}
```

wire_amd/csrc/wire_pack.hip:

```cpp
#include "wire_dev.h"
#include "wire_point.h"

template <bool WS>
WIRE_DEVINL void pack_hidden_body(int kind, const float* __restrict__ W, const float* __restrict__ b,
                                  const float* __restrict__ V, const float* __restrict__ c, int K,
                                  int Kin, int P, int Pin, int Nc, float* __restrict__ Bt_fwd,
                                  float* __restrict__ Bt_dgrad, float* __restrict__ bias, float ws) {
  const int k = blockIdx.x * blockDim.x + threadIdx.x;
  const int j = blockIdx.y;
  if (k >= Pin) return;
  float val = 0.f, bv = 0.f;
  if (kind == NK_WIRE || kind == NK_WIRE2D) {
    int o, part;
    const float* Wm = W;
    const float* bm = b;
    if (kind == NK_WIRE) {
      blk_decode(j, o, part);
    } else {
      const int sub = (j >> 5) & 3;
      o = ((j >> 7) << 5) + (j & 31);
      part = sub & 1;
      if (sub >= 2) { Wm = V; bm = c; }
    }
    int i, ipart;
    blk_decode(k, i, ipart);
    if (o < K) {
      bv = bm[2 * o + part];
      if (i < Kin) {
        const float wr = Wm[((size_t)o * Kin + i) * 2];
        const float wi = Wm[((size_t)o * Kin + i) * 2 + 1];
        val = part == 0 ? (ipart == 0 ? wr : -wi) : (ipart == 0 ? wi : wr);
      }
    }
  } else {
    if (j < K) {
      bv = b[j];
      if (k < Kin) val = WS ? ws * W[(size_t)j * Kin + k] : W[(size_t)j * Kin + k];
    }
  }
  Bt_fwd[(size_t)j * Pin + k] = val;
  Bt_dgrad[(size_t)k * Nc + j] = val;
  if (k == 0) bias[j] = bv;
}
template <bool WS>
__global__ void pack_hidden_kernel(int kind, const float* __restrict__ W, const float* __restrict__ b,
                                   const float* __restrict__ V, const float* __restrict__ c, int K,
                                   int Kin, int P, int Pin, int Nc, float* __restrict__ Bt_fwd,
                                   float* __restrict__ Bt_dgrad, float* __restrict__ bias, float ws) {
  pack_hidden_body<WS>(kind, W, b, V, c, K, Kin, P, Pin, Nc, Bt_fwd, Bt_dgrad, bias, ws);
}
template <bool WS>
__global__ void pack_hidden_batch_kernel(int kind, PackBatch pb, int K, int Kin, int P, int Pin, int Nc, float ws) {
  const int z = blockIdx.z;
  pack_hidden_body<WS>(kind, pb.W[z], pb.b[z], pb.V[z], pb.c[z], K, Kin, P, Pin, Nc, pb.fwd[z], pb.dg[z], pb.bias[z], ws);
}
hipError_t launch_pack_hidden_batch(hipStream_t s, int kind, const PackBatch& pb, int nb, int K, int Kin, int P,
                                    int Pin, float wscale) {
  if (nb < 1 || nb > PACK_MAXB) return hipErrorInvalidValue;
  const int Nc = (kind == NK_WIRE2D) ? 2 * P : P;
  dim3 grid(cdiv(Pin, 128), (unsigned)Nc, (unsigned)nb);
  if (wscale != 1.f)
    hipLaunchKernelGGL(pack_hidden_batch_kernel<true>, grid, dim3(128), 0, s, kind, pb, K, Kin, P, Pin, Nc, wscale);
  else
    hipLaunchKernelGGL(pack_hidden_batch_kernel<false>, grid, dim3(128), 0, s, kind, pb, K, Kin, P, Pin, Nc, 1.f);
  return hipGetLastError();
}

hipError_t launch_pack_hidden(hipStream_t s, int kind, const float* W, const float* b,
                              const float* V, const float* c, int K, int Kin, int P, int Pin,
                              float* Bt_fwd, float* Bt_dgrad, float* bias, float wscale) {
  const int Nc = (kind == NK_WIRE2D) ? 2 * P : P;
  dim3 grid(cdiv(Pin, 128), (unsigned)Nc);
  if (wscale != 1.f)
    hipLaunchKernelGGL(pack_hidden_kernel<true>, grid, dim3(128), 0, s, kind, W, b, V, c, K, Kin, P, Pin,
                       Nc, Bt_fwd, Bt_dgrad, bias, wscale);
  else
    hipLaunchKernelGGL(pack_hidden_kernel<false>, grid, dim3(128), 0, s, kind, W, b, V, c, K, Kin, P, Pin,
                       Nc, Bt_fwd, Bt_dgrad, bias, 1.f);
  return hipGetLastError();
}

__global__ void scale_copy_kernel(const float* __restrict__ src, long long n, float c, float* __restrict__ dst) {
  const long long i = (long long)blockIdx.x * blockDim.x + threadIdx.x;
  if (i < n) dst[i] = c * src[i];
}
hipError_t launch_scale_copy(hipStream_t s, const float* src, int64_t n, float c, float* dst) {
  if (n <= 0) return hipSuccess;
  hipLaunchKernelGGL(scale_copy_kernel, dim3(cdiv(n, 256)), dim3(256), 0, s, src, (long long)n, c, dst);
  return hipGetLastError();
}

__global__ void pack_final_kernel(int kind, const float* __restrict__ Wf, const float* __restrict__ bf,
                                  int K, int P, int O, float* __restrict__ wf, float* __restrict__ bfr) {
  const int c = blockIdx.x * blockDim.x + threadIdx.x;
  const int o = blockIdx.y;
  if (c >= P) return;
  float val = 0.f;
  if (kind == NK_WIRE || kind == NK_WIRE2D) {
    int i, part;
    blk_decode(c, i, part);
    if (i < K) {
      const float w = Wf[((size_t)o * K + i) * 2 + part];
      val = part == 0 ? w : -w;
    }
    if (c == 0) bfr[o] = bf[2 * o];
  } else {
    if (c < K) val = Wf[(size_t)o * K + c];
    if (c == 0) bfr[o] = bf[o];
  }
  wf[(size_t)o * P + c] = val;
}

hipError_t launch_pack_final(hipStream_t s, int kind, const float* Wf, const float* bf, int K,
                             int P, int O, float* wf, float* bfr) {
  dim3 grid(cdiv(P, 128), (unsigned)O);
  hipLaunchKernelGGL(pack_final_kernel, grid, dim3(128), 0, s, kind, Wf, bf, K, P, O, wf, bfr);
  return hipGetLastError();
}

WIRE_DEVINL void pack3m_body(const float* __restrict__ W, const float* __restrict__ b, int K, int Kin,
                             int Kp, int Kpin, float* __restrict__ Wb_fwd, float* __restrict__ Wb_dg,
                             float* __restrict__ bias) {
  const int i = blockIdx.x * blockDim.x + threadIdx.x;
  const int o = blockIdx.y;
  if (i >= Kpin) return;
  float wr = 0.f, wi = 0.f;
  if (o < K && i < Kin) {
    wr = W[((size_t)o * Kin + i) * 2];
    wi = W[((size_t)o * Kin + i) * 2 + 1];
  }
  const int ci = blk_col(i, 0), co = blk_col(o, 0);
  Wb_fwd[(size_t)o * (2 * Kpin) + ci] = wr;
  Wb_fwd[(size_t)o * (2 * Kpin) + ci + 32] = wi;
  Wb_dg[(size_t)i * (2 * Kp) + co] = wr;
  Wb_dg[(size_t)i * (2 * Kp) + co + 32] = -wi;
  if (i == 0) {
    bias[co] = o < K ? b[2 * o] : 0.f;
    bias[co + 32] = o < K ? b[2 * o + 1] : 0.f;
  }
}
__global__ void pack3m_kernel(const float* __restrict__ W, const float* __restrict__ b, int K, int Kin,
                              int Kp, int Kpin, float* __restrict__ Wb_fwd, float* __restrict__ Wb_dg,
                              float* __restrict__ bias) {
  pack3m_body(W, b, K, Kin, Kp, Kpin, Wb_fwd, Wb_dg, bias);
}
__global__ void pack3m_batch_kernel(PackBatch pb, int K, int Kin, int Kp, int Kpin) {
  const int z = blockIdx.z;
  pack3m_body(pb.W[z], pb.b[z], K, Kin, Kp, Kpin, pb.fwd[z], pb.dg[z], pb.bias[z]);
}
hipError_t launch_pack3m_batch(hipStream_t s, const PackBatch& pb, int nb, int K, int Kin, int Kp, int Kpin) {
  if (nb < 1 || nb > PACK_MAXB) return hipErrorInvalidValue;
  dim3 grid(cdiv(Kpin, 64), (unsigned)Kp, (unsigned)nb);
  hipLaunchKernelGGL(pack3m_batch_kernel, grid, dim3(64), 0, s, pb, K, Kin, Kp, Kpin);
  return hipGetLastError();
}
hipError_t launch_pack3m(hipStream_t s, const float* W, const float* b, int K, int Kin, int Kp, int Kpin,
                         float* Wb_fwd, float* Wb_dg, float* bias) {
  dim3 grid(cdiv(Kpin, 64), (unsigned)Kp);
  hipLaunchKernelGGL(pack3m_kernel, grid, dim3(64), 0, s, W, b, K, Kin, Kp, Kpin, Wb_fwd, Wb_dg, bias);
  return hipGetLastError();
}
```

wire_amd/csrc/wire_plan.h:

```cpp
#pragma once
#include <hip/hip_runtime.h>

#include <atomic>
#include <mutex>
#include <utility>
#include <vector>

#include "../../include/wire_hip.h"
#include "wire_gemm.h"
#include "wire_point.h"

#ifndef WIRE_AMAX_SLOTS
#define WIRE_AMAX_SLOTS 64
#endif

int fail(int code, const char* fmt, ...);
int wire_fail_(int code, const char* msg);
#define HIPCHK(expr)                                                                   \
  do {                                                                                 \
    hipError_t e_ = (expr);                                                            \
    if (e_ != hipSuccess)                                                              \
      return fail(WIRE_ERR_HIP, "%s failed: %s (%s:%d)", #expr, hipGetErrorString(e_), \
                  __FILE__, __LINE__);                                                 \
  } while (0)

struct ProfRec { hipEvent_t a, b; int cls; double flops; };
extern std::mutex g_prof_mu;
extern std::atomic<bool> g_prof_on;
extern std::vector<ProfRec> g_prof_recs;
extern std::vector<std::pair<hipEvent_t, hipEvent_t>> g_prof_pool;

struct ProfScope {
  hipStream_t s; int cls; double flops; bool on; hipEvent_t a{}, b{};
  ProfScope(hipStream_t s_, int cls_, double flops_) : s(s_), cls(cls_), flops(flops_), on(false) {
    if (!g_prof_on.load(std::memory_order_relaxed)) return;
    std::lock_guard<std::mutex> lk(g_prof_mu);
    if (!g_prof_on.load(std::memory_order_relaxed)) return;
    on = true;
    if (!g_prof_pool.empty()) {
      a = g_prof_pool.back().first; b = g_prof_pool.back().second; g_prof_pool.pop_back();
    } else {
      (void)hipEventCreate(&a); (void)hipEventCreate(&b);
    }
    (void)hipEventRecord(a, s);
  }
  ~ProfScope() {
    if (!on) return;
    (void)hipEventRecord(b, s);
    std::lock_guard<std::mutex> lk(g_prof_mu);
    g_prof_recs.push_back({a, b, cls, flops});
  }
};

inline int rup(int v, int m) { return (v + m - 1) / m * m; }

struct Plan {
  int kind, D, K, L, O, F;
  float w1, w, s;
  float ws = 1.f;
  bool cplx, first_gemm, m3, x3, x2;
  int P, Pl, Din, Pin0, ldu, ntens, per_layer, Kp;
  int nsc = 0;
  float sc_c[WIRE_MS_MAX_SCALES] = {};
  bool ms = false;
  int SHF = 0, T = 0, ms_split = 0, t0 = 0;
  bool m2 = false;
  int S2 = 1;
  int64_t off_comb = -1;
  bool hier = false;
  int HS = 0, HL = 0;
  int64_t hj_fwd[WIRE_MS_MAX_SCALES] = {}, hj_fwd_x3[WIRE_MS_MAX_SCALES] = {}, hj_fwd_x2[WIRE_MS_MAX_SCALES] = {},
          hj_bias[WIRE_MS_MAX_SCALES] = {}, hj_half[WIRE_MS_MAX_SCALES] = {}, hj_wamax = -1, h_nat = -1;
  bool mfn = false;
  int64_t mf_tab = -1;
  std::vector<int64_t> off_fwd, off_dg, off_bias, off_fwd_x3, off_dg_x3, off_fwd_3m, off_dg_3m, off_fwd_x2, off_dg_x2;
  int64_t off_wf, off_bf, off_first, off_wamax, total_packed;
  int64_t off_fx;
  bool k_split_out, k_recompute_out, k_first_sums, k_first_dn, k_bwd_lookahead, k_nt_bfirst, k_epi_early, k_rstore, k_wgrad_batch, k_fused_fwd, k_fused_train, k_fused_bwd, k_fused_final,
       k_fused_train_p384;
  int64_t off_fxd;
  std::vector<int64_t> tfloats;
};

inline int first_tensor(const Plan& p, int q) { return p.ms ? q : p.t0 + q; }

inline int mfn_tw(const Plan& p, int l) { return 4 * (p.L + 1) + 2 * (l - 1); }
inline const float* mfn_tab(const Plan& p, const float* packed, int i) { return packed + p.mf_tab + (int64_t)i * p.P * 12; }

inline int hier_last(const Plan& p, int st) { return st == 0 ? p.HL : 2; }
inline int hier_t(const Plan& p, int st, int l) {
  return st == 0 ? 2 * l : 2 * (p.HL + 1) + 6 * (st - 1) + 2 * l;
}
inline int hier_th(const Plan& p, int st) { return 2 * (p.HL + 1) + 6 * (p.HS - 1) + 2 * st; }
inline int hier_v(const Plan& p, int st, int l) { return st == 0 ? l : p.HL + 3 * (st - 1) + 1; }
inline int hier_vhalf(const Plan& p, int st, int half) { return p.HL + 3 * (st - 1) + 2 + half; }
inline int64_t hier_nat_stride(const Plan& p) {
  return rup(p.K * p.D, 4) + rup(p.K, 4) + rup(p.O * p.K, 4) + rup(p.O, 4);
}
struct HierNat { const float* W0; const float* b0; const float* Wh; const float* bh; };
inline HierNat hier_nat(const Plan& p, const float* packed, int st) {
  HierNat h;
  const float* c = packed + p.h_nat + (int64_t)st * hier_nat_stride(p);
  h.W0 = c; c += rup(p.K * p.D, 4);
  h.b0 = c; c += rup(p.K, 4);
  h.Wh = c; c += rup(p.O * p.K, 4);
  h.bh = c;
  return h;
}

int make_plan(const wire_net_desc* d, Plan& p);

inline int64_t fx_hidden_off(const Plan& p) { return p.off_fx + (p.first_gemm ? (int64_t)p.P * p.Pin0 : 0); }
inline int64_t fx_pass_off(const Plan& p, int k) { return fx_hidden_off(p) + (int64_t)k * p.L * fused_b_image_floats(p.P); }
inline float pass_c(const Plan& p, int k) { return p.m2 ? p.sc_c[k] : p.s; }
inline int64_t first_native_off(const Plan& p, int q) {
  int64_t off = p.off_first;
  for (int i = 0; i < q; ++i) off += rup((int)p.tfloats[first_tensor(p, i)], 4);
  return off;
}
inline M2Comb comb_of(const Plan& p, const float* packed) {
  M2Comb w;
  const float* c = packed + p.off_comb;
  w.W1 = c; c += rup((int)p.tfloats[0], 4);
  w.b1 = c; c += rup((int)p.tfloats[1], 4);
  w.W2 = c; c += rup((int)p.tfloats[2], 4);
  w.b2 = c;
  return w;
}

struct ActLayout {
  int64_t pe, out0, lin0, lin1, total;
  int64_t ping, pong;
  int64_t amax;
  int64_t pe_amax;
  int64_t ytr;
  int64_t np;
};
ActLayout act_layout(const Plan& p, int64_t n1, int save);

struct ScratchLayout { int64_t ga, gb, gu, slab, bslab, fpw, fpb, crp, gamax, gch, gch_stride, gtr, cpart, crep, mh, mfp, total; int S; };
ScratchLayout scratch_layout(const Plan& p, int64_t n1);

struct CoordLayout { int64_t cgp, gpe, total; int ntiles; };
CoordLayout coord_layout(const Plan& p, int64_t n);

inline int epi_fwd(int kind) { return known_kind(kind).epi_fwd; }
inline int epi_bwd(int kind) { return known_kind(kind).epi_bwd; }

enum RouteMode { MODE_INFER, MODE_AUTOGRAD, MODE_TRAIN };
struct Route {
  RouteMode mode;
  WireFamily fam;
  WireFamily fam0;
  WireFamily tn0;
  float pe_split;
  WireFamily tn_fam;
  int tn_S;
  bool fused_fwd;
  bool fuse;
  bool fused_train;
  bool fused_final;
  bool chain;
  bool rstore;
  bool skip_out_L;
  bool recompute_out;
  bool recompute_out0;
  bool first_sums;
  bool cg_epi;
  bool bwd_lookahead;
  bool first_dn;
  int wb_l0, wb_n, wb_S;
  float act_scale;
  float out_scale[65];
};
Route make_route(const Plan& p, int64_t n, RouteMode mode);

inline const unsigned* wamax_of(const Plan& p, const float* packed, int l) {
  return reinterpret_cast<const unsigned*>(packed + p.off_wamax + (int64_t)l * WIRE_AMAX_SLOTS);
}
hipError_t layer_nt(hipStream_t s, const Plan& p, WireFamily f, const float* packed, int l, bool dg, int epi,
                    const float* A, int64_t n, GemmEpiParams ep, const unsigned* amax_a = nullptr,
                    const unsigned* amax_b = nullptr, unsigned* amax_out = nullptr);

Route mfn_route(const Plan& p, int64_t n, RouteMode mode);
int mfn_pack(hipStream_t s, const Plan& p, const void* const* params, float* packed);
int mfn_fwd_core(void* stream, const Plan& p, const Route& r, const float* packed, const float* coords, int64_t n, float* y,
                 void* act, int64_t act_bytes);
int mfn_bwd_core(void* stream, const Plan& p, const Route& r, const float* packed, const float* coords, int64_t n,
                 const float* g_y, const void* act, int64_t act_bytes, void* scratch, int64_t scratch_bytes,
                 void* const* grads, wire_grad_ready_fn ready, void* user, float* g_coords);

struct HierOut { int64_t off; int ld; int aset; };
struct HierAct {
  int64_t amax, total;
  std::vector<std::vector<int64_t>> lin;
  std::vector<std::vector<HierOut>> out;
  std::vector<int64_t> cat;
};
struct HierScratch { int64_t gamax, g[3], slab, bslab, fpw, fpb, crp, lpart, total, cgp, total_coords; int S; };

HierAct hier_act(const Plan& p, int64_t n, int save);
HierScratch hier_scratch(const Plan& p, int64_t n);
Route hier_route(const Plan& p, int64_t n, RouteMode mode);
int pack_hidden(hipStream_t s, const Plan& p, const void* const* params, float* packed, const std::vector<const float*>& hW,
                const std::vector<const float*>& hb);
int hier_pack(hipStream_t s, const Plan& p, const void* const* params, float* packed);
int hier_fwd_core(void* stream, const Plan& p, const Route& r, const float* packed, const float* coords, int64_t n, float* y,
                  void* act, int64_t act_bytes, const M2Loss* loss = nullptr, float* loss_part = nullptr);
int hier_bwd_core(void* stream, const Plan& p, const Route& r, const float* packed, const float* coords, int64_t n,
                  const float* g_y, const void* act, int64_t act_bytes, void* scratch, int64_t scratch_bytes,
                  void* const* grads, wire_grad_ready_fn ready, void* user, float* g_coords);
```

wire_amd/csrc/wire_point.h:

```cpp
#pragma once
#include <hip/hip_runtime.h>
#include <stdint.h>

#include "wire_gemm.h"

#define WIRE_MAXO 8
#define WIRE_FINAL_MAX_OP 16384
#define WIRE_FB_ROWS 256
static inline unsigned cdiv(int64_t a, int64_t b) { return (unsigned)((a + b - 1) / b); }
#define PRE_CHUNKS 32
static inline int prereduce_room(int nblk) { return nblk + PRE_CHUNKS; }

hipError_t launch_pack_hidden(hipStream_t s, int kind, const float* W, const float* b,
                              const float* V, const float* c, int K, int Kin, int P, int Pin,
                              float* Bt_fwd, float* Bt_dgrad, float* bias, float wscale = 1.f);
#define PACK_MAXB 16
struct PackBatch {
  const float* W[PACK_MAXB]; const float* b[PACK_MAXB]; const float* V[PACK_MAXB]; const float* c[PACK_MAXB];
  float* fwd[PACK_MAXB]; float* dg[PACK_MAXB]; float* bias[PACK_MAXB];
};
hipError_t launch_pack_hidden_batch(hipStream_t s, int kind, const PackBatch& pb, int nb, int K, int Kin, int P,
                                    int Pin, float wscale = 1.f);
hipError_t launch_scale_copy(hipStream_t s, const float* src, int64_t n, float c, float* dst);
hipError_t launch_pack3m_batch(hipStream_t s, const PackBatch& pb, int nb, int K, int Kin, int Kp, int Kpin);
hipError_t launch_pack_final(hipStream_t s, int kind, const float* Wf, const float* bf, int K,
                             int P, int O, float* wf, float* bfr);
hipError_t launch_pack3m(hipStream_t s, const float* W, const float* b, int K, int Kin, int Kp, int Kpin,
                         float* Wb_fwd, float* Wb_dg, float* bias);

hipError_t launch_first_fwd(hipStream_t s, int kind, const float* coords, int64_t n, int D,
                            const float* W0, const float* b0, const float* V0, const float* c0,
                            int K, int P, float omega, float scale, float* lin, float* out,
                            unsigned* amax_out = nullptr);

hipError_t launch_posenc(hipStream_t s, const float* coords, int64_t n, int D, int F, int Pin,
                         float* dst);

struct MscaleC { float c[8]; };
hipError_t launch_mscale_first(hipStream_t s, const float* coords, int64_t n, int D, const float* W0, const float* b0,
                               int SHF, const MscaleC& c, int split, int ld, float split_scale, unsigned* amax,
                               float* dst);

hipError_t launch_coordgrad_rows(hipStream_t s, const float* G, int ldg, const float* G2, const float* W, const float* V,
                                 int K, int D, int64_t n, float* g_x);
hipError_t launch_coordgrad_reduce(hipStream_t s, const float* partial, int ntiles, int64_t n, int D, float* g_x);
hipError_t launch_posenc_bwd(hipStream_t s, const float* coords, int64_t n, int D, int F, const float* g_pe, int ldpe,
                             float* g_x);

hipError_t launch_final_fwd(hipStream_t s, const float* z, int64_t n, int P, int O,
                            const float* wf, const float* bfr, float* y);

int final_bwd_blocks(int64_t n);
hipError_t launch_final_bwd(hipStream_t s, int kind, int raw, const float* g_y, int64_t n, int O,
                            const float* wf, const float* lin, const float* out, int K, int P,
                            float omega, float scale, float* g_lin, float* part_w,
                            float* part_b, unsigned* amax_g = nullptr);

bool final_fused_supported(int P, int O);
hipError_t launch_final_fused(hipStream_t s, int kind, const float* out, const float* lin, int64_t n, int P, int O,
                              int kvalid, const float* wf, const float* bfr, const float* target, const int64_t* idx,
                              int64_t first, float weight, float omega, float scale, float* y, float* rec,
                              float* g_lin, float* part_w, float* part_b, float* loss_partial,
                              float* loss_out, unsigned* amax_g = nullptr);

hipError_t launch_final_reduce(hipStream_t s, int kind, float* part_w, float* part_b,
                               int nblk, int O, int K, int P, float* gWf, float* gbf);

hipError_t launch_wgrad_reduce(hipStream_t s, int kind, const float* slab, const float* bslab,
                               int S, int K, int Kin, int Pm, int Pn, float* gW, float* gb,
                               float* gV, float* gc, float wscale = 1.f);

int colreduce_blocks(int64_t n);
hipError_t launch_colreduce_final(hipStream_t s, int C, int D, int64_t n, float* partial, float* gW0, float* gb0,
                                  float wscale = 1.f);
hipError_t launch_colreduce_final_blocks(hipStream_t s, int C, int D, int nblk, float* partial, float* gW0, float* gb0,
                                         float wscale = 1.f);
hipError_t launch_colreduce(hipStream_t s, const float* G, int ldg, int C, const float* x, int D,
                            int64_t n, float* partial, float* gW0, float* gb0, float wscale = 1.f);

hipError_t launch_wgrad3m_reduce(hipStream_t s, const float* slab, const float* bslab, int S, int K, int Kin,
                                 int Kp_o, int Kp_i, float* gW, float* gb);

hipError_t launch_c64_to_blocked(hipStream_t s, const float* src, int64_t n, int K, int P, float* dst);
hipError_t launch_blocked_to_c64(hipStream_t s, const float* src, int64_t n, int K, int P, float* dst);
hipError_t launch_pad_rows(hipStream_t s, const float* src, int64_t n, int K, int P, float* dst);
hipError_t launch_unpad_rows(hipStream_t s, const float* src, int64_t n, int K, int P, float* dst);

hipError_t launch_gabor_bwd_point(hipStream_t s, const float* g, const float* lin, const float* out,
                                  int64_t n, int P, float omega, float scale, float* g_lin);
hipError_t launch_gabor_bwd_first_point(hipStream_t s, const float* g, const float* out,
                                        const float* coords, int D, const float* W0, const float* b0,
                                        int64_t n, int K, int P, float omega, float scale, float* g_u,
                                        int ldu);

hipError_t launch_gabor2d_bwd_point(hipStream_t s, const float* g, const float* linsy, const float* out,
                                    int64_t n, int P, float omega, float scale, float* g_linsy);
hipError_t launch_gabor2d_bwd_first_point(hipStream_t s, const float* g, const float* out, const float* coords,
                                          int D, const float* W0, const float* b0, const float* V0,
                                          const float* c0, int64_t n, int K, int P, float omega, float scale,
                                          float* g_up, int ldu);

hipError_t launch_real_act_bwd_point(hipStream_t s, int kind, const float* g, const float* lin,
                                     const float* out, int64_t n, int P, float omega, float scale,
                                     float* g_lin);

int hparam_blocks(int64_t n);
hipError_t launch_gabor_hparam_grad(hipStream_t s, const float* g, const float* lin, const float* out, int64_t n,
                                    int K, int P, int is_first, float scale, float* partial, float* out2);
hipError_t launch_gabor2d_hparam_grad(hipStream_t s, const float* g, const float* linsy, const float* out, int64_t n,
                                      int K, int P, int is_first, float scale, float* partial, float* out2);

hipError_t launch_perm_indices(hipStream_t s, uint64_t seed, int64_t n_total, int64_t first, int64_t count,
                               int64_t* idx_out);
hipError_t launch_coords(hipStream_t s, const int64_t* idx, int64_t first, int64_t n,
                         const float* tx, int W, const float* ty, int H, const float* tz, int T,
                         float* coords);
hipError_t launch_mse_final(hipStream_t s, const float* partial, int nb, float lscale, float* loss_out);
hipError_t launch_mse_grad(hipStream_t s, const float* y, const float* target, const int64_t* idx,
                           int64_t first, int64_t n, int O, float weight, float* g_y,
                           float* loss_out, float* rec, float* partial);
hipError_t launch_avgpool_mse_grad(hipStream_t s, const float* y, int H, int W, int O, int scale,
                                   const float* gt_lr, float* g_y, float* rec_lr, float* loss_out,
                                   float* partial);
hipError_t launch_avgpool_mse_grad_frames(hipStream_t s, const float* y, int B, int H, int W, int O, int scale,
                                          const float* gt_lr, const float* mask, float* g_y, float* rec_lr,
                                          float* loss_out, float* partial);
hipError_t launch_coded_mse_grad(hipStream_t s, const float* y, int64_t p0, int64_t n_pix, int64_t NP, int T, int O,
                                 int nframes, int dup_last, const float* mask, const float* gt, float* g_y, float* est,
                                 float* loss_out, float* partial);
hipError_t launch_coded_fwd(hipStream_t s, const float* video, const float* masks, int T, int64_t NP, int nframes,
                            int dup_last, float* coded);
hipError_t launch_coded_bwd(hipStream_t s, const float* g_coded, const float* masks, int T, int64_t NP, int nframes,
                            int dup_last, float* g_video);
hipError_t launch_affine_coords(hipStream_t s, const double* mats, int B, int H, int W, float* coords);
hipError_t launch_adam(hipStream_t s, float* p, const float* g, float* m, float* v, int64_t count,
                       float step_size, float beta1, float beta2, float eps, float inv_sqrt_bc2);

hipError_t launch_metric(hipStream_t s, int mode, const float* rec, const float* gt, int64_t count, float thres,
                         float* out, float* partial);
#define SSIM_MAX_TAPS 11
struct SsimWin { float w[SSIM_MAX_TAPS]; };
int64_t ssim_tiles(int H, int W, int taps);
hipError_t launch_ssim(hipStream_t s, const float* x, const float* y, int H, int W, int O, int taps, const SsimWin& win,
                       float cov, float c1, float c2, float* out1, float* map, float* partial);
int64_t ssim_bwd_tiles(int H, int W);
int64_t ssim_loss_partials(int H, int W);
hipError_t launch_ssim_bwd(hipStream_t s, const float* x, const float* y, int H, int W, int O, int taps,
                           const SsimWin& win, float cov, float c1, float c2, const float* g_ssim, float* g_y);
hipError_t launch_ssim_mse_grad(hipStream_t s, const float* y, int H, int W, int O, const float* target, int taps,
                                const SsimWin& win, float cov, float c1, float c2, const int64_t* idx, int64_t first,
                                int64_t n_mse, float lambda, float* g_y, float* loss_out, float* rec, float* partial);

bool tv_shape_ok(int planes, int H, int W, int64_t pix_stride, int64_t plane_stride);
hipError_t launch_tv_fwd(hipStream_t s, const float* x, int planes, int H, int W, int64_t pix_stride,
                         int64_t plane_stride, float* tv_out, float* partial);
hipError_t launch_tv_bwd(hipStream_t s, const float* x, int planes, int H, int W, int64_t pix_stride,
                         int64_t plane_stride, const float* g_tv, float* g_x);
hipError_t launch_tv_mse_grad(hipStream_t s, const float* y, int H, int W, int O, const float* target,
                              const int64_t* idx, int64_t first, int64_t n_mse, float lambda_tv, float* g_y,
                              float* loss_out, float* rec, float* partial);
hipError_t launch_tv_add_grad(hipStream_t s, const float* y, int H, int W, int T, int O, float lambda_s,
                              float lambda_t, const float* data_loss, float* g_y, float* loss_out, float* partial);

hipError_t launch_track_best(hipStream_t s, const float* metric, float* best, int force, const float* src,
                             float* dst, int64_t count, int* updated);
hipError_t launch_sigmoid(hipStream_t s, float* x, int64_t count);

hipError_t launch_radon_fwd(hipStream_t s, const float* img, const float* angles, int H, int W, int A, float* sino);
hipError_t launch_radon_bwd(hipStream_t s, const float* g_sino, const float* angles, int H, int W, int A,
                            float* g_img);

#define M2_MAX_SCALES 8
#define M2_H 128
#define M2_COMB_MAXBLK 512
struct M2Comb { const float* W1; const float* b1; const float* W2; const float* b2; };
struct M2Grads { float* W1; float* b1; float* W2; float* b2; };
struct M2Loss {
  const float* target = nullptr; const int64_t* idx = nullptr; int64_t first = 0; float gscale = 0.f;
  float* y = nullptr; float* g_y = nullptr; float* rec = nullptr;
};
__host__ __device__ inline int m2_comb_grad_floats(int S, int O) {
  return M2_H * S * O + M2_H + O * M2_H + O;
}
int m2_comb_blocks(int64_t n);
hipError_t launch_m2_comb_fwd(hipStream_t s, const M2Comb& w, int S, int O, const float* t, int64_t n, float* y);
hipError_t launch_m2_comb_bwd(hipStream_t s, const M2Comb& w, int S, int O, const float* t, int64_t n, const M2Loss& ls,
                              const float* g_y, float* g_t, float* part, float* loss_part);
hipError_t launch_m2_comb_reduce(hipStream_t s, const float* part, int64_t n, int S, int O, const M2Grads& g);
hipError_t launch_m2_sum_passes(hipStream_t s, const float* g, int S, int64_t n, int D, float* out);

hipError_t launch_hier_first_fwd(hipStream_t s, const float* coords, int64_t n, int D, const float* W0, const float* b0,
                                 int K, int P, float c, float* lin, float* out, int ldo, unsigned* amax_out);
#define HIER_HEAD_MAXBLK 1024
int hier_head_blocks(int64_t n);
hipError_t launch_hier_head_fwd(hipStream_t s, const float* x, int ldx, const float* Wh, const float* bh, int64_t n, int K,
                                int P, int O, int acc, float* y, const M2Loss& ls, float* loss_part);
hipError_t launch_hier_head_bwd(hipStream_t s, const float* g_y, int64_t n, int O, const float* Wh, const float* x, int ldx,
                                const float* lin, const float* add, int K, int P, float c, float* g_lin, float* part_w,
                                float* part_b, unsigned* amax_g);
hipError_t launch_hier_pack_join(hipStream_t s, const float* W, const float* b, int K, int P, float* fwd, float* bias,
                                 float* Wa, float* Wb);
hipError_t launch_hier_join_reduce(hipStream_t s, const float* slab, const float* bslab, int S, int K, int P, float* gW,
                                   float* gb);

hipError_t launch_mfn_pack_table(hipStream_t s, const float* mu, const float* gamma, const float* w, const float* c, int K,
                                 int D, int P, float* tab);
hipError_t launch_mfn_filter_fwd(hipStream_t s, const float* tab, const float* coords, int64_t n, int D, int K, int P,
                                 const float* mul, float* out, unsigned* amax_out);
hipError_t launch_mfn_filter_fwd_native(hipStream_t s, const float* mu, const float* gamma, const float* w, const float* c,
                                        const float* coords, int64_t n, int D, int K, float* out);
hipError_t launch_mfn_final_bwd(hipStream_t s, const float* g_y, int64_t n, int O, const float* wf, const float* z,
                                const float* lin, const float* tab, const float* coords, int D, int P, float* g_lin,
                                float* hbuf, float* part_w, float* part_b, unsigned* amax_g);
int mfn_sums_blocks(int64_t n);
hipError_t launch_mfn_filter_sums(hipStream_t s, const float* tab, const float* coords, int64_t n, int D, int K,
                                  const float* hbuf, int ldh, float* part, float* g_mu, float* g_gamma, float* g_w,
                                  float* g_c);
hipError_t launch_mfn_filter_sums_native(hipStream_t s, const float* mu, const float* gamma, const float* w, const float* c,
                                         const float* coords, int64_t n, int D, int K, const float* hbuf, float* part,
                                         float* g_mu, float* g_gamma, float* g_w, float* g_c);
hipError_t launch_mfn_filter_gx(hipStream_t s, const float* tab, const float* coords, int64_t n, int D, int K,
                                const float* hbuf, int ldh, int acc, float* g_x);
hipError_t launch_mfn_filter_gx_native(hipStream_t s, const float* mu, const float* gamma, const float* w, const float* c,
                                       const float* coords, int64_t n, int D, int K, const float* hbuf, float* g_x);
```

wire_amd/csrc/wire_reduce.hip:

```cpp
#include "wire_dev.h"
#include "wire_point.h"

__global__ __launch_bounds__(256) void prereduce_kernel(const float* __restrict__ in, int nblk, int C, int per,
                                                        float* __restrict__ out) {
  const int c = blockIdx.x * 256 + threadIdx.x;
  const int ch = blockIdx.y;
  if (c >= C) return;
  const int b0 = ch * per;
  int b1 = b0 + per;
  if (b1 > nblk) b1 = nblk;
  float a0 = 0.f, a1 = 0.f, a2 = 0.f, a3 = 0.f;
  int b = b0;
  for (; b + 3 < b1; b += 4) {
    a0 += in[(size_t)b * C + c];
    a1 += in[(size_t)(b + 1) * C + c];
    a2 += in[(size_t)(b + 2) * C + c];
    a3 += in[(size_t)(b + 3) * C + c];
  }
  for (; b < b1; ++b) a0 += in[(size_t)b * C + c];
  out[(size_t)ch * C + c] = (a0 + a1) + (a2 + a3);
}
static int prereduce(hipStream_t s, const float* in, int nblk, int C, float* out) {
  if (nblk <= 2 * PRE_CHUNKS) return nblk;
  const int per = (nblk + PRE_CHUNKS - 1) / PRE_CHUNKS;
  const int nch = (nblk + per - 1) / per;
  hipLaunchKernelGGL(prereduce_kernel, dim3(cdiv(C, 256), (unsigned)nch), dim3(256), 0, s, in, nblk, C, per, out);
  return nch;
}

__global__ __launch_bounds__(256) void final_reduce_kernel(int kind, const float* __restrict__ part_w,
                                    const float* __restrict__ part_b, int nblk, int O, int K, int P,
                                    float* __restrict__ gWf, float* __restrict__ gbf) {
  __shared__ float red[2][4][64];
  const int tx = threadIdx.x & 63, ty = threadIdx.x >> 6;
  const int i = blockIdx.x * 64 + tx;
  const int o = blockIdx.y;
  const bool cplx = (kind == NK_WIRE || kind == NK_WIRE2D);
  float sr = 0.f, si = 0.f;
  if (i < K) {
    const int c = cplx ? blk_col(i, 0) : i;
    for (int b = ty; b < nblk; b += 4) {
      const float* pw = part_w + ((size_t)b * O + o) * P;
      sr += pw[c];
      if (cplx) si += pw[c + 32];
    }
  }
  red[0][ty][tx] = sr;
  red[1][ty][tx] = si;
  __syncthreads();
  if (ty == 0 && i < K) {
    sr = (red[0][0][tx] + red[0][1][tx]) + (red[0][2][tx] + red[0][3][tx]);
    si = (red[1][0][tx] + red[1][1][tx]) + (red[1][2][tx] + red[1][3][tx]);
    if (cplx) {
      gWf[((size_t)o * K + i) * 2] = sr;
      gWf[((size_t)o * K + i) * 2 + 1] = -si;
    } else {
      gWf[(size_t)o * K + i] = sr;
    }
  }
  if (blockIdx.x == 0 && threadIdx.x == 0) {
    float sb = 0.f;
    for (int b = 0; b < nblk; ++b) sb += part_b[(size_t)b * O + o];
    if (cplx) { gbf[2 * o] = sb; gbf[2 * o + 1] = 0.f; } else gbf[o] = sb;
  }
}

hipError_t launch_final_reduce(hipStream_t s, int kind, float* part_w, float* part_b,
                               int nblk, int O, int K, int P, float* gWf, float* gbf) {
  float* w2 = part_w + (size_t)nblk * O * P;
  float* b2 = part_b + (size_t)nblk * O;
  const int nw = prereduce(s, part_w, nblk, O * P, w2);
  const int nb = prereduce(s, part_b, nblk, O, b2);
  dim3 grid(cdiv(K, 64), (unsigned)O);
  hipLaunchKernelGGL(final_reduce_kernel, grid, dim3(256), 0, s, kind, nw == nblk ? part_w : w2,
                     nb == nblk ? part_b : b2, nw == nblk ? nblk : nw, O, K, P, gWf, gbf);
  return hipGetLastError();
}

template <bool WS>
__global__ __launch_bounds__(256) void wgrad_reduce_kernel(int kind, const float* __restrict__ slab,
                                    const float* __restrict__ bslab, int S, int K, int Kin, int Pm,
                                    int Pn, float* __restrict__ gW, float* __restrict__ gb,
                                    float* __restrict__ gV, float* __restrict__ gc, float ws) {
  __shared__ float red[4][4][64];
  const int tx = threadIdx.x & 63, q = threadIdx.x >> 6;
  const int i = blockIdx.x * 64 + tx;
  const int o = blockIdx.y;
  const size_t sstride = (size_t)Pm * Pn;
  const bool cplx = (kind == NK_WIRE || kind == NK_WIRE2D);
  const int nmat = (kind == NK_WIRE2D) ? 2 : 1;
  for (int mat = 0; mat < nmat; ++mat) {
    int r_re, r_im = 0;
    if (kind == NK_WIRE) { r_re = blk_col(o, 0); r_im = r_re + 32; }
    else if (kind == NK_WIRE2D) { r_re = ((o >> 5) << 7) + 64 * mat + (o & 31); r_im = r_re + 32; }
    else r_re = o;
    float sr = 0.f, si = 0.f, br = 0.f, bi = 0.f;
    if (i < Kin) {
      if (cplx) {
        const int c_re = blk_col(i, 0), c_im = c_re + 32;
        const size_t a = (size_t)r_re * Pn + c_re, b = (size_t)r_im * Pn + c_im, c = (size_t)r_im * Pn + c_re,
                     d = (size_t)r_re * Pn + c_im;
#pragma unroll 4
        for (int sp = q; sp < S; sp += 4) {
          const float* m = slab + sp * sstride;
          sr += m[a] + m[b];
          si += m[c] - m[d];
        }
      } else {
        const size_t a = (size_t)o * Pn + i;
#pragma unroll 4
        for (int sp = q; sp < S; sp += 4) sr += slab[sp * sstride + a];
      }
    }
    if (tx == 0 && blockIdx.x == 0)
      for (int sp = q; sp < S; sp += 4) {
        br += bslab[(size_t)sp * Pm + r_re];
        if (cplx) bi += bslab[(size_t)sp * Pm + r_im];
      }
    red[0][q][tx] = sr; red[1][q][tx] = si; red[2][q][tx] = br; red[3][q][tx] = bi;
    __syncthreads();
    if (q == 0) {
      float* gWm = mat == 0 ? gW : gV;
      float* gbm = mat == 0 ? gb : gc;
      const float wr = (red[0][0][tx] + red[0][1][tx]) + (red[0][2][tx] + red[0][3][tx]);
      const float wi = (red[1][0][tx] + red[1][1][tx]) + (red[1][2][tx] + red[1][3][tx]);
      if (i < Kin) {
        if (cplx) {
          gWm[((size_t)o * Kin + i) * 2] = wr;
          gWm[((size_t)o * Kin + i) * 2 + 1] = wi;
        } else {
          gWm[(size_t)o * Kin + i] = WS ? ws * wr : wr;
        }
      }
      if (tx == 0 && blockIdx.x == 0) {
        const float b0 = (red[2][0][0] + red[2][1][0]) + (red[2][2][0] + red[2][3][0]);
        const float b1 = (red[3][0][0] + red[3][1][0]) + (red[3][2][0] + red[3][3][0]);
        if (cplx) { gbm[2 * o] = b0; gbm[2 * o + 1] = b1; }
        else gbm[o] = b0;
      }
    }
    __syncthreads();
  }
}

hipError_t launch_wgrad_reduce(hipStream_t s, int kind, const float* slab, const float* bslab,
                               int S, int K, int Kin, int Pm, int Pn, float* gW, float* gb,
                               float* gV, float* gc, float wscale) {
  dim3 grid(cdiv(Kin, 64), (unsigned)K);
  if (wscale != 1.f)
    hipLaunchKernelGGL(wgrad_reduce_kernel<true>, grid, dim3(256), 0, s, kind, slab, bslab, S, K, Kin, Pm,
                       Pn, gW, gb, gV, gc, wscale);
  else
    hipLaunchKernelGGL(wgrad_reduce_kernel<false>, grid, dim3(256), 0, s, kind, slab, bslab, S, K, Kin, Pm,
                       Pn, gW, gb, gV, gc, 1.f);
  return hipGetLastError();
}

#define CR_ROWS 256
int colreduce_blocks(int64_t n) { return (int)((n + CR_ROWS - 1) / CR_ROWS); }

__global__ __launch_bounds__(256) void colreduce_kernel(const float* __restrict__ G, int ldg, int C,
                                                        const float* __restrict__ x, int D,
                                                        long long n, float* __restrict__ partial) {
  __shared__ float red[4][64][20];
  const int tx = threadIdx.x & 63, ty = threadIdx.x >> 6;
  const int c0 = (blockIdx.y * 64 + tx) * 4;
  const long long r0 = (long long)blockIdx.x * CR_ROWS;
  long long r1 = r0 + CR_ROWS;
  if (r1 > n) r1 = n;
  float acc[4][5];
#pragma unroll
  for (int q = 0; q < 4; ++q)
#pragma unroll
    for (int d = 0; d < 5; ++d) acc[q][d] = 0.f;
  if (c0 < ldg) {
    for (long long row = r0 + ty; row < r1; row += 4) {
      const f32x4 g = *reinterpret_cast<const f32x4*>(G + row * ldg + c0);
      float xv[4] = {0.f, 0.f, 0.f, 0.f};
      for (int d = 0; d < D; ++d) xv[d] = x[row * D + d];
#pragma unroll
      for (int q = 0; q < 4; ++q) {
#pragma unroll
        for (int d = 0; d < 4; ++d) acc[q][d] = __builtin_fmaf(g[q], xv[d], acc[q][d]);
        acc[q][4] += g[q];
      }
    }
  }
#pragma unroll
  for (int q = 0; q < 4; ++q)
#pragma unroll
    for (int d = 0; d < 5; ++d) red[ty][tx][q * 5 + d] = acc[q][d];
  __syncthreads();
  if (ty == 0) {
#pragma unroll
    for (int q = 0; q < 4; ++q) {
      const int c = c0 + q;
      if (c < C) {
        float* p = partial + ((size_t)blockIdx.x * C + c) * 5;
#pragma unroll
        for (int d = 0; d < 5; ++d)
          p[d] = (red[0][tx][q * 5 + d] + red[1][tx][q * 5 + d]) + (red[2][tx][q * 5 + d] + red[3][tx][q * 5 + d]);
      }
    }
  }
}

template <bool WS>
__global__ __launch_bounds__(256) void colreduce_final_kernel(const float* __restrict__ partial, int nblk,
                                                              int C, int D, float* __restrict__ gW0,
                                                              float* __restrict__ gb0, float ws) {
  __shared__ float red[4][64][5];
  const int tx = threadIdx.x & 63, ty = threadIdx.x >> 6;
  const int c = blockIdx.x * 64 + tx;
  float acc[5] = {0.f, 0.f, 0.f, 0.f, 0.f};
  if (c < C) {
    for (int b = ty; b < nblk; b += 4) {
      const float* p = partial + ((size_t)b * C + c) * 5;
#pragma unroll
      for (int d = 0; d < 5; ++d) acc[d] += p[d];
    }
  }
#pragma unroll
  for (int d = 0; d < 5; ++d) red[ty][tx][d] = acc[d];
  __syncthreads();
  if (ty == 0 && c < C) {
#pragma unroll
    for (int d = 0; d < 5; ++d) acc[d] = (red[0][tx][d] + red[1][tx][d]) + (red[2][tx][d] + red[3][tx][d]);
    for (int d = 0; d < D; ++d) gW0[c * D + d] = WS ? ws * acc[d] : acc[d];
    gb0[c] = acc[4];
  }
}

hipError_t launch_colreduce_final(hipStream_t s, int C, int D, int64_t n, float* partial, float* gW0, float* gb0,
                                  float wscale) {
  return launch_colreduce_final_blocks(s, C, D, colreduce_blocks(n), partial, gW0, gb0, wscale);
}
hipError_t launch_colreduce_final_blocks(hipStream_t s, int C, int D, int nblk, float* partial, float* gW0, float* gb0,
                                         float wscale) {
  if (D > 4 || nblk < 1) return hipErrorInvalidValue;
  float* p2 = partial + (size_t)nblk * C * 5;
  const int nb = prereduce(s, partial, nblk, C * 5, p2);
  if (wscale != 1.f)
    hipLaunchKernelGGL(colreduce_final_kernel<true>, dim3(cdiv(C, 64)), dim3(256), 0, s, nb == nblk ? partial : p2, nb,
                       C, D, gW0, gb0, wscale);
  else
    hipLaunchKernelGGL(colreduce_final_kernel<false>, dim3(cdiv(C, 64)), dim3(256), 0, s, nb == nblk ? partial : p2, nb,
                       C, D, gW0, gb0, 1.f);
  return hipGetLastError();
}
hipError_t launch_colreduce(hipStream_t s, const float* G, int ldg, int C, const float* x, int D,
                            int64_t n, float* partial, float* gW0, float* gb0, float wscale) {
  if (D > 4 || (ldg & 3)) return hipErrorInvalidValue;
  const int nblk = colreduce_blocks(n);
  dim3 grid((unsigned)nblk, cdiv(C, 256));
  hipLaunchKernelGGL(colreduce_kernel, grid, dim3(256), 0, s, G, ldg, C, x, D, (long long)n, partial);
  return launch_colreduce_final(s, C, D, n, partial, gW0, gb0, wscale);
}

__global__ __launch_bounds__(256) void wgrad3m_reduce_kernel(const float* __restrict__ slab,
                                      const float* __restrict__ bslab, int S, int K, int Kin, int Kp_o,
                                      int Kp_i, float* __restrict__ gW, float* __restrict__ gb) {
  __shared__ float red[2][4][64];
  const int tx = threadIdx.x & 63, ty = threadIdx.x >> 6;
  const int i = blockIdx.x * 64 + tx;
  const int o = blockIdx.y;
  const size_t plane = (size_t)Kp_o * Kp_i;
  float sr = 0.f, si = 0.f;
  if (i < Kin) {
    for (int s = ty; s < S; s += 4) {
      const float* p = slab + (size_t)s * 3 * plane + (size_t)o * Kp_i + i;
      const float p1 = p[0], p2 = p[plane], p3 = p[2 * plane];
      sr += p1 + p2;
      si += (p3 - p1) + p2;
    }
  }
  red[0][ty][tx] = sr;
  red[1][ty][tx] = si;
  __syncthreads();
  if (ty == 0 && i < Kin) {
    gW[((size_t)o * Kin + i) * 2] = (red[0][0][tx] + red[0][1][tx]) + (red[0][2][tx] + red[0][3][tx]);
    gW[((size_t)o * Kin + i) * 2 + 1] = (red[1][0][tx] + red[1][1][tx]) + (red[1][2][tx] + red[1][3][tx]);
  }
  if (blockIdx.x == 0 && threadIdx.x == 0) {
    float br = 0.f, bi = 0.f;
    for (int s = 0; s < S; ++s) {
      br += bslab[((size_t)s * 2 + 0) * Kp_o + o];
      bi += bslab[((size_t)s * 2 + 1) * Kp_o + o];
    }
    gb[2 * o] = br;
    gb[2 * o + 1] = bi;
  }
}
hipError_t launch_wgrad3m_reduce(hipStream_t s, const float* slab, const float* bslab, int S, int K, int Kin,
                                 int Kp_o, int Kp_i, float* gW, float* gb) {
  dim3 grid(cdiv(Kin, 64), (unsigned)K);
  hipLaunchKernelGGL(wgrad3m_reduce_kernel, grid, dim3(256), 0, s, slab, bslab, S, K, Kin, Kp_o, Kp_i, gW, gb);
  return hipGetLastError();
}
```

wire_amd/csrc/wire_train.hip:

```cpp
#include "wire_dev.h"
#include "wire_point.h"

__device__ __host__ inline unsigned long long perm_splitmix(unsigned long long z) {
  z += 0x9e3779b97f4a7c15ull;
  z = (z ^ (z >> 30)) * 0xbf58476d1ce4e5b9ull;
  z = (z ^ (z >> 27)) * 0x94d049bb133111ebull;
  return z ^ (z >> 31);
}
struct PermKeys { unsigned long long m[4], k[4]; };
__device__ inline unsigned long long perm_apply(unsigned long long x, unsigned long long n, int b, int sh,
                                                const PermKeys& K) {
  const unsigned long long mask = (b >= 64) ? ~0ull : ((1ull << b) - 1ull);
  do {
#pragma unroll
    for (int r = 0; r < 4; ++r) {
      x = (x * K.m[r] + K.k[r]) & mask;
      x ^= x >> sh;
    }
  } while (x >= n);
  return x;
}
__global__ void perm_indices_kernel(PermKeys K, long long n_total, int b, int sh, long long first, long long count,
                                    int64_t* __restrict__ idx_out) {
  const long long r = (long long)blockIdx.x * blockDim.x + threadIdx.x;
  if (r >= count) return;
  idx_out[r] = (int64_t)perm_apply((unsigned long long)(first + r), (unsigned long long)n_total, b, sh, K);
}
hipError_t launch_perm_indices(hipStream_t s, uint64_t seed, int64_t n_total, int64_t first, int64_t count,
                               int64_t* idx_out) {
  if (count <= 0) return hipSuccess;
  if (n_total < 1 || first < 0 || first + count > n_total) return hipErrorInvalidValue;
  int b = 0;
  while (b < 63 && (1ull << b) < (unsigned long long)n_total) ++b;
  if (b == 0) b = 1;
  const int sh = b / 2 > 0 ? b / 2 : 1;
  PermKeys K;
  for (int r = 0; r < 4; ++r) {
    K.m[r] = perm_splitmix(seed * 8 + r) | 1ull;
    K.k[r] = perm_splitmix(seed * 8 + 4 + r);
  }
  hipLaunchKernelGGL(perm_indices_kernel, dim3(cdiv(count, 256)), dim3(256), 0, s, K, (long long)n_total, b, sh,
                     (long long)first, (long long)count, idx_out);
  return hipGetLastError();
}

__global__ void coords_kernel(const int64_t* __restrict__ idx, long long first, long long n,
                              const float* __restrict__ tx, int W, const float* __restrict__ ty,
                              int H, const float* __restrict__ tz, int T,
                              float* __restrict__ coords) {
  const long long r = (long long)blockIdx.x * blockDim.x + threadIdx.x;
  if (r >= n) return;
  long long id = idx ? idx[r] : first + r;
  if (tz) {
    const long long k = id % T;
    id /= T;
    const long long j = id % W, i = id / W;
    coords[r * 3 + 0] = tx[j];
    coords[r * 3 + 1] = ty[i];
    coords[r * 3 + 2] = tz[k];
  } else {
    const long long j = id % W, i = id / W;
    coords[r * 2 + 0] = tx[j];
    coords[r * 2 + 1] = ty[i];
  }
}
hipError_t launch_coords(hipStream_t s, const int64_t* idx, int64_t first, int64_t n,
                         const float* tx, int W, const float* ty, int H, const float* tz, int T,
                         float* coords) {
  if (n <= 0) return hipSuccess;
  hipLaunchKernelGGL(coords_kernel, dim3(cdiv(n, 256)), dim3(256), 0, s, idx, (long long)first,
                     (long long)n, tx, W, ty, H, tz, T, coords);
  return hipGetLastError();
}

#define MSE_BLOCKS 1024
__global__ __launch_bounds__(256) void mse_grad_kernel(const float* __restrict__ y,
                                                       const float* __restrict__ target,
                                                       const int64_t* __restrict__ idx,
                                                       long long first, long long n, int O,
                                                       float gscale, float* __restrict__ g_y,
                                                       float* __restrict__ rec,
                                                       float* __restrict__ partial) {
  __shared__ float red[256];
  const long long total = n * O;
  float acc = 0.f;
  for (long long e = (long long)blockIdx.x * blockDim.x + threadIdx.x; e < total;
       e += (long long)gridDim.x * blockDim.x) {
    const long long r = e / O;
    const int o = (int)(e - r * O);
    const long long src = idx ? idx[r] : first + r;
    const float yy = y[e];
    const float d = yy - target[src * O + o];
    g_y[e] = gscale * d;
    if (rec) rec[src * O + o] = yy;
    acc = __builtin_fmaf(d, d, acc);
  }
  acc = wire_block_tree_sum(acc, red);
  if (threadIdx.x == 0) partial[blockIdx.x] = acc;
}
__global__ void mse_final_kernel(const float* __restrict__ partial, int nb, float lscale,
                                 float* __restrict__ loss_out) {
  __shared__ float red[256];
  float acc = 0.f;
  for (int i = threadIdx.x; i < nb; i += 256) acc += partial[i];
  acc = wire_block_tree_sum(acc, red);
  if (threadIdx.x == 0) loss_out[0] = acc * lscale;
}
static unsigned mse_blocks(long long n) { return n < (long long)MSE_BLOCKS * 256 ? cdiv(n, 256) : MSE_BLOCKS; }
hipError_t launch_mse_final(hipStream_t s, const float* partial, int nb, float lscale, float* loss_out) {
  hipLaunchKernelGGL(mse_final_kernel, dim3(1), dim3(256), 0, s, partial, nb, lscale, loss_out);
  return hipGetLastError();
}
hipError_t launch_mse_grad(hipStream_t s, const float* y, const float* target, const int64_t* idx,
                           int64_t first, int64_t n, int O, float weight, float* g_y,
                           float* loss_out, float* rec, float* partial) {
  if (n <= 0) return hipSuccess;
  const unsigned nb = mse_blocks(n * O);
  const float inv = (float)(1.0 / ((double)n * (double)O));
  hipLaunchKernelGGL(mse_grad_kernel, dim3(nb), dim3(256), 0, s, y, target, idx, (long long)first,
                     (long long)n, O, weight * 2.f * inv, g_y, rec, partial);
  return launch_mse_final(s, partial, (int)nb, weight * inv, loss_out);
}

__global__ __launch_bounds__(256) void avgpool_mse_grad_kernel(const float* __restrict__ y, int H, int W, int O,
                                                               int sc, int H2, int W2,
                                                               const float* __restrict__ gt_lr, float gscale,
                                                               float* __restrict__ g_y,
                                                               float* __restrict__ rec_lr,
                                                               float* __restrict__ partial) {
  __shared__ float red[256];
  const long long total = (long long)H2 * W2 * O;
  const float inv = 1.f / (float)(sc * sc);
  float acc = 0.f;
  for (long long e = (long long)blockIdx.x * blockDim.x + threadIdx.x; e < total;
       e += (long long)gridDim.x * blockDim.x) {
    const long long pix = e / O;
    const int o = (int)(e - pix * O);
    const int pi = (int)(pix / W2), pj = (int)(pix - (long long)pi * W2);
    const float* src = y + ((size_t)(pi * sc) * W + (size_t)pj * sc) * O + o;
    float sum = 0.f;
    for (int a = 0; a < sc; ++a)
      for (int b = 0; b < sc; ++b) sum += src[((size_t)a * W + b) * O];
    const float pool = sum * inv;
    const float d = pool - gt_lr[e];
    if (rec_lr) rec_lr[e] = pool;
    const float g = gscale * d;
    float* dst = g_y + ((size_t)(pi * sc) * W + (size_t)pj * sc) * O + o;
    for (int a = 0; a < sc; ++a)
      for (int b = 0; b < sc; ++b) dst[((size_t)a * W + b) * O] = g;
    acc = __builtin_fmaf(d, d, acc);
  }
  acc = wire_block_tree_sum(acc, red);
  if (threadIdx.x == 0) partial[blockIdx.x] = acc;
}
hipError_t launch_avgpool_mse_grad(hipStream_t s, const float* y, int H, int W, int O, int scale,
                                   const float* gt_lr, float* g_y, float* rec_lr, float* loss_out,
                                   float* partial) {
  const int H2 = H / scale, W2 = W / scale;
  if (H2 < 1 || W2 < 1) return hipErrorInvalidValue;
  if (H2 * scale != H || W2 * scale != W) {
    hipError_t e = hipMemsetAsync(g_y, 0, (size_t)H * W * O * sizeof(float), s);
    if (e != hipSuccess) return e;
  }
  const long long total = (long long)H2 * W2 * O;
  const unsigned nb = mse_blocks(total);
  const double invn = 1.0 / (double)total;
  hipLaunchKernelGGL(avgpool_mse_grad_kernel, dim3(nb), dim3(256), 0, s, y, H, W, O, scale, H2, W2, gt_lr,
                     (float)(2.0 * invn / ((double)scale * scale)), g_y, rec_lr, partial);
  return launch_mse_final(s, partial, (int)nb, (float)invn, loss_out);
}

#define APF_CAP 1024
__global__ __launch_bounds__(256) void avgpool_frames_kernel(const float* __restrict__ y, int B, int H, int W, int O,
                                                             int sc, int H2, int W2, int TP, int ntile,
                                                             const float* __restrict__ gt_lr,
                                                             const float* __restrict__ mask, float gscale,
                                                             float* __restrict__ g_y, float* __restrict__ rec_lr,
                                                             float* __restrict__ partial) {
  __shared__ float colsum[APF_CAP], gpool[APF_CAP], red[256];
  const long long rowf = (long long)W * O;
  const int pf = sc * O;
  const float inv = 1.f / ((float)sc * (float)sc);
  const long long njobs = (long long)B * H2 * ntile;
  const int tid = threadIdx.x;
  float acc = 0.f;
  for (long long job = blockIdx.x; job < njobs; job += gridDim.x) {
    const int t = (int)(job % ntile);
    const long long fr = job / ntile;
    const int pi = (int)(fr % H2);
    const long long f = fr / H2;
    const int p0 = t * TP;
    const int np = W2 - p0 < TP ? W2 - p0 : TP;
    const int nx = np * pf;
    const long long x0 = (long long)p0 * pf;
    const long long hr0 = (f * H + (long long)pi * sc) * rowf + x0;
    for (int x = tid; x < nx; x += 256) {
      const float* src = y + hr0 + x;
      float s = 0.f;
      for (int a = 0; a < sc; ++a) s += src[a * rowf];
      colsum[x] = s;
    }
    __syncthreads();
    const long long pbase = ((f * H2 + pi) * W2 + p0) * O;
    for (int e = tid; e < np * O; e += 256) {
      const int pl = e / O, o = e - pl * O;
      const float* cs = colsum + pl * pf + o;
      float s = 0.f;
      for (int b = 0; b < sc; ++b) s += cs[b * O];
      const float pool = s * inv;
      const float m = mask ? mask[pbase + e] : 1.f;
      const float d = __fmul_rn(pool, m) - __fmul_rn(gt_lr[pbase + e], m);
      if (rec_lr) rec_lr[pbase + e] = pool;
      gpool[e] = gscale * (d * m);
      acc = __builtin_fmaf(d, d, acc);
    }
    __syncthreads();
    const int nxw = t == ntile - 1 ? (int)(rowf - x0) : nx;
    for (int a = 0; a < sc; ++a) {
      float* dst = g_y + hr0 + a * rowf;
      for (int x = tid; x < nxw; x += 256) {
        const int pl = x / pf;
        dst[x] = x < nx ? gpool[pl * O + (x - pl * pf) % O] : 0.f;
      }
    }
    if (pi == H2 - 1)
      for (int i = H2 * sc; i < H; ++i) {
        float* dst = g_y + (f * H + i) * rowf + x0;
        for (int x = tid; x < nxw; x += 256) dst[x] = 0.f;
      }
  }
  acc = wire_block_tree_sum(acc, red);
  if (tid == 0) partial[blockIdx.x] = acc;
}
__global__ __launch_bounds__(256) void avgpool_frames_direct_kernel(const float* __restrict__ y, int B, int H, int W,
                                                                    int O, int sc, int H2, int W2,
                                                                    const float* __restrict__ gt_lr,
                                                                    const float* __restrict__ mask, float gscale,
                                                                    float* __restrict__ g_y,
                                                                    float* __restrict__ rec_lr,
                                                                    float* __restrict__ partial) {
  __shared__ float red[256];
  const long long total = (long long)B * H2 * W2 * O;
  const long long rowf = (long long)W * O;
  const float inv = 1.f / ((float)sc * (float)sc);
  float acc = 0.f;
  for (long long e = (long long)blockIdx.x * blockDim.x + threadIdx.x; e < total;
       e += (long long)gridDim.x * blockDim.x) {
    const long long pix = e / O;
    const int o = (int)(e - pix * O);
    const int pj = (int)(pix % W2);
    const long long fr = pix / W2;
    const int pi = (int)(fr % H2);
    const long long f = fr / H2;
    const long long off = (f * H + (long long)pi * sc) * rowf + (long long)pj * sc * O + o;
    float sum = 0.f;
    for (int a = 0; a < sc; ++a)
      for (int b = 0; b < sc; ++b) sum += y[off + a * rowf + (long long)b * O];
    const float pool = sum * inv;
    const float m = mask ? mask[e] : 1.f;
    const float d = __fmul_rn(pool, m) - __fmul_rn(gt_lr[e], m);
    if (rec_lr) rec_lr[e] = pool;
    const float g = gscale * (d * m);
    for (int a = 0; a < sc; ++a)
      for (int b = 0; b < sc; ++b) g_y[off + a * rowf + (long long)b * O] = g;
    acc = __builtin_fmaf(d, d, acc);
  }
  acc = wire_block_tree_sum(acc, red);
  if (threadIdx.x == 0) partial[blockIdx.x] = acc;
}
hipError_t launch_avgpool_mse_grad_frames(hipStream_t s, const float* y, int B, int H, int W, int O, int scale,
                                          const float* gt_lr, const float* mask, float* g_y, float* rec_lr,
                                          float* loss_out, float* partial) {
  const int H2 = H / scale, W2 = W / scale;
  if (B < 1 || O < 1 || H2 < 1 || W2 < 1) return hipErrorInvalidValue;
  const double total = (double)B * H2 * W2 * O;
  const float gscale = (float)(2.0 / total / ((double)scale * scale));
  unsigned nb;
  if ((long long)scale * O <= APF_CAP) {
    const int cap = APF_CAP / (scale * O);
    const int TP = W2 < cap ? W2 : cap;
    const int ntile = (W2 + TP - 1) / TP;
    const long long njobs = (long long)B * H2 * ntile;
    nb = njobs < MSE_BLOCKS ? (unsigned)njobs : MSE_BLOCKS;
    hipLaunchKernelGGL(avgpool_frames_kernel, dim3(nb), dim3(256), 0, s, y, B, H, W, O, scale, H2, W2, TP, ntile,
                       gt_lr, mask, gscale, g_y, rec_lr, partial);
  } else {
    if (H2 * scale != H || W2 * scale != W) {
      hipError_t e = hipMemsetAsync(g_y, 0, (size_t)B * H * W * O * sizeof(float), s);
      if (e != hipSuccess) return e;
    }
    const long long n = (long long)total;
    nb = mse_blocks(n);
    hipLaunchKernelGGL(avgpool_frames_direct_kernel, dim3(nb), dim3(256), 0, s, y, B, H, W, O, scale, H2, W2, gt_lr,
                       mask, gscale, g_y, rec_lr, partial);
  }
  return launch_mse_final(s, partial, (int)nb, (float)(1.0 / total), loss_out);
}

#define CV_CAP 1024
__global__ __launch_bounds__(256) void coded_mse_grad_kernel(const float* __restrict__ y, long long p0,
                                                             long long n_pix, long long NP, int T, int O, int nf,
                                                             int C, int dup, int TP, int PS,
                                                             const float* __restrict__ mask,
                                                             const float* __restrict__ gt, float gscale,
                                                             float* __restrict__ g_y, float* __restrict__ est,
                                                             float* __restrict__ partial) {
  __shared__ float ym[CV_CAP], ms[CV_CAP], gd[CV_CAP], red[256];
  const int pf = T * O;
  const long long njobs = (n_pix + TP - 1) / TP;
  const long long cstride = NP * O;
  const int tid = threadIdx.x;
  float acc = 0.f;
  for (long long job = blockIdx.x; job < njobs; job += gridDim.x) {
    const long long l0 = job * TP;
    const int np = n_pix - l0 < TP ? (int)(n_pix - l0) : TP;
    const int nx = np * pf;
    const long long base = l0 * pf;
    const float* mrow = mask + (p0 + l0) * T;
    for (int x = tid; x < nx; x += 256) {
      const int pl = x / pf, r = x - pl * pf;
      const float m = mrow[pl * T + r / O];
      ms[pl * PS + r] = m;
      ym[pl * PS + r] = m * y[base + x];
    }
    __syncthreads();
    const int ne = np * O;
    const long long cbase = (p0 + l0) * O;
    for (int e = tid; e < C * ne; e += 256) {
      const int c = e / ne, r = e - c * ne;
      const int pl = r / O, o = r - pl * O;
      const int k0 = c * nf, k1 = k0 + nf < T ? k0 + nf : T;
      const float* src = ym + pl * PS + o;
      float s = 0.f;
      for (int k = k0; k < k1; ++k) s += src[k * O];
      const long long ci = c * cstride + cbase + r;
      float d = s - gt[ci];
      if (est) est[ci] = s;
      acc = __builtin_fmaf(d, d, acc);
      if (dup && c == C - 1) {
        const float d2 = s - gt[ci + cstride];
        if (est) est[ci + cstride] = s;
        acc = __builtin_fmaf(d2, d2, acc);
        d += d2;
      }
      gd[e] = gscale * d;
    }
    __syncthreads();
    for (int x = tid; x < nx; x += 256) {
      const int pl = x / pf, r = x - pl * pf;
      const int k = r / O, o = r - k * O;
      g_y[base + x] = ms[pl * PS + r] * gd[(k / nf) * ne + pl * O + o];
    }
    __syncthreads();
  }
  acc = wire_block_tree_sum(acc, red);
  if (tid == 0) partial[blockIdx.x] = acc;
}
__global__ __launch_bounds__(256) void coded_mse_grad_direct_kernel(const float* __restrict__ y, long long p0,
                                                                    long long n_pix, long long NP, int T, int O,
                                                                    int nf, int C, int dup,
                                                                    const float* __restrict__ mask,
                                                                    const float* __restrict__ gt, float gscale,
                                                                    float* __restrict__ g_y, float* __restrict__ est,
                                                                    float* __restrict__ partial) {
  __shared__ float red[256];
  const long long total = n_pix * O;
  const long long cstride = NP * O;
  float acc = 0.f;
  for (long long e = (long long)blockIdx.x * blockDim.x + threadIdx.x; e < total;
       e += (long long)gridDim.x * blockDim.x) {
    const long long pl = e / O;
    const int o = (int)(e - pl * O);
    const float* yp = y + pl * T * O + o;
    float* gp = g_y + pl * T * O + o;
    const float* mp = mask + (p0 + pl) * T;
    for (int c = 0; c < C; ++c) {
      const int k0 = c * nf, k1 = k0 + nf < T ? k0 + nf : T;
      float s = 0.f;
      for (int k = k0; k < k1; ++k) s += mp[k] * yp[(long long)k * O];
      const long long ci = c * cstride + (p0 + pl) * O + o;
      float d = s - gt[ci];
      if (est) est[ci] = s;
      acc = __builtin_fmaf(d, d, acc);
      if (dup && c == C - 1) {
        const float d2 = s - gt[ci + cstride];
        if (est) est[ci + cstride] = s;
        acc = __builtin_fmaf(d2, d2, acc);
        d += d2;
      }
      const float g = gscale * d;
      for (int k = k0; k < k1; ++k) gp[(long long)k * O] = mp[k] * g;
    }
  }
  acc = wire_block_tree_sum(acc, red);
  if (threadIdx.x == 0) partial[blockIdx.x] = acc;
}
hipError_t launch_coded_mse_grad(hipStream_t s, const float* y, int64_t p0, int64_t n_pix, int64_t NP, int T, int O,
                                 int nframes, int dup_last, const float* mask, const float* gt, float* g_y, float* est,
                                 float* loss_out, float* partial) {
  if (T < 1 || O < 1 || nframes < 1 || n_pix < 1 || NP < 1) return hipErrorInvalidValue;
  const int C = (int)(((long long)T + nframes - 1) / nframes);
  const double count = (double)(C + dup_last) * (double)NP * O;
  const float gscale = (float)(2.0 / count);
  const long long pf = (long long)T * O;
  const long long PS = pf | 1;
  unsigned nb;
  if (PS <= CV_CAP) {
    const long long cap = CV_CAP / PS;
    const int TP = (int)(n_pix < cap ? n_pix : cap);
    const long long njobs = (n_pix + TP - 1) / TP;
    nb = njobs < MSE_BLOCKS ? (unsigned)njobs : MSE_BLOCKS;
    hipLaunchKernelGGL(coded_mse_grad_kernel, dim3(nb), dim3(256), 0, s, y, (long long)p0, (long long)n_pix,
                       (long long)NP, T, O, nframes, C, dup_last, TP, (int)PS, mask, gt, gscale, g_y, est, partial);
  } else {
    const long long n = (long long)n_pix * O;
    nb = mse_blocks(n);
    hipLaunchKernelGGL(coded_mse_grad_direct_kernel, dim3(nb), dim3(256), 0, s, y, (long long)p0, (long long)n_pix,
                       (long long)NP, T, O, nframes, C, dup_last, mask, gt, gscale, g_y, est, partial);
  }
  return launch_mse_final(s, partial, (int)nb, (float)(1.0 / count), loss_out);
}

__global__ __launch_bounds__(256) void coded_fwd_kernel(const float* __restrict__ video, const float* __restrict__ masks,
                                                        int T, long long NP, int nf, int C, int dup,
                                                        float* __restrict__ coded) {
  const long long e = (long long)blockIdx.x * blockDim.x + threadIdx.x;
  if (e >= C * NP) return;
  const int c = (int)(e / NP);
  const long long p = e - c * NP;
  const int k0 = c * nf, k1 = k0 + nf < T ? k0 + nf : T;
  float s = 0.f;
  for (int k = k0; k < k1; ++k) s += video[k * NP + p] * masks[k * NP + p];
  coded[e] = s;
  if (dup && c == C - 1) coded[e + NP] = s;
}
__global__ __launch_bounds__(256) void coded_bwd_kernel(const float* __restrict__ g_coded,
                                                        const float* __restrict__ masks, int T, long long NP, int nf,
                                                        int C, int dup, float* __restrict__ g_video) {
  const long long e = (long long)blockIdx.x * blockDim.x + threadIdx.x;
  if (e >= T * NP) return;
  const int k = (int)(e / NP);
  const long long p = e - k * NP;
  const int c = k / nf;
  float g = g_coded[c * NP + p];
  if (dup && c == C - 1) g += g_coded[C * NP + p];
  g_video[e] = masks[e] * g;
}
hipError_t launch_coded_fwd(hipStream_t s, const float* video, const float* masks, int T, int64_t NP, int nframes,
                            int dup_last, float* coded) {
  const int C = (int)(((long long)T + nframes - 1) / nframes);
  hipLaunchKernelGGL(coded_fwd_kernel, dim3(cdiv((long long)C * NP, 256)), dim3(256), 0, s, video, masks, T,
                     (long long)NP, nframes, C, dup_last, coded);
  return hipGetLastError();
}
hipError_t launch_coded_bwd(hipStream_t s, const float* g_coded, const float* masks, int T, int64_t NP, int nframes,
                            int dup_last, float* g_video) {
  const int C = (int)(((long long)T + nframes - 1) / nframes);
  hipLaunchKernelGGL(coded_bwd_kernel, dim3(cdiv((long long)T * NP, 256)), dim3(256), 0, s, g_coded, masks, T,
                     (long long)NP, nframes, C, dup_last, g_video);
  return hipGetLastError();
}

__global__ void affine_coords_kernel(const double* __restrict__ mats, long long n, int H, int W,
                                     float* __restrict__ coords) {
#pragma clang fp contract(off)
  const long long r = (long long)blockIdx.x * blockDim.x + threadIdx.x;
  if (r >= n) return;
  const long long hw = (long long)H * W;
  const long long f = r / hw, p = r - f * hw;
  const double i = (double)(p / W), j = (double)(p % W);
  const double* m = mats + f * 6;
  const double xn = m[0] * j + m[1] * i + m[2];
  const double yn = m[3] * j + m[4] * i + m[5];
  coords[r * 2 + 0] = (float)(2.0 * xn / (double)W - 1.0);
  coords[r * 2 + 1] = (float)(2.0 * yn / (double)H - 1.0);
}
hipError_t launch_affine_coords(hipStream_t s, const double* mats, int B, int H, int W, float* coords) {
  const long long n = (long long)B * H * W;
  hipLaunchKernelGGL(affine_coords_kernel, dim3(cdiv(n, 256)), dim3(256), 0, s, mats, n, H, W, coords);
  return hipGetLastError();
}

__global__ void adam_kernel(float* __restrict__ p, const float* __restrict__ g,
                            float* __restrict__ m, float* __restrict__ v, long long count,
                            float step_size, float beta1, float beta2, float eps,
                            float inv_sqrt_bc2) {
  const long long i = (long long)blockIdx.x * blockDim.x + threadIdx.x;
  if (i >= count) return;
  const float gg = g[i];
  const float mm = __builtin_fmaf(beta1, m[i], (1.f - beta1) * gg);
  const float vv = __builtin_fmaf(beta2, v[i], (1.f - beta2) * gg * gg);
  m[i] = mm;
  v[i] = vv;
  const float denom = __builtin_fmaf(__builtin_sqrtf(vv), inv_sqrt_bc2, eps);
  p[i] = p[i] - step_size * (mm / denom);
}
hipError_t launch_adam(hipStream_t s, float* p, const float* g, float* m, float* v, int64_t count,
                       float step_size, float beta1, float beta2, float eps, float inv_sqrt_bc2) {
  if (count <= 0) return hipSuccess;
  hipLaunchKernelGGL(adam_kernel, dim3(cdiv(count, 256)), dim3(256), 0, s, p, g, m, v,
                     (long long)count, step_size, beta1, beta2, eps, inv_sqrt_bc2);
  return hipGetLastError();
}

#define MET_BLOCKS 1024
__global__ __launch_bounds__(256) void metric_kernel(int mode, const float* __restrict__ rec,
                                                     const float* __restrict__ gt, long long count,
                                                     float thres, float* __restrict__ partial) {
  __shared__ float r0[256], r1[256];
  float a = 0.f, b = mode == 0 ? -3.4e38f : 0.f;
  for (long long e = (long long)blockIdx.x * 256 + threadIdx.x; e < count; e += (long long)gridDim.x * 256) {
    const float x = gt[e], y = rec[e];
    if (mode == 0) {
      const float d = x - y;
      a = __builtin_fmaf(d, d, a);
      b = x > b ? x : b;
    } else {
      const bool p = y >= thres, q = x != 0.f;
      a += (p && q) ? 1.f : 0.f;
      b += (p || q) ? 1.f : 0.f;
    }
  }
  r0[threadIdx.x] = a; r1[threadIdx.x] = b;
  __syncthreads();
  for (int sft = 128; sft >= 1; sft >>= 1) {
    if (threadIdx.x < sft) {
      r0[threadIdx.x] += r0[threadIdx.x + sft];
      r1[threadIdx.x] = mode == 0 ? (r1[threadIdx.x] > r1[threadIdx.x + sft] ? r1[threadIdx.x] : r1[threadIdx.x + sft])
                                  : r1[threadIdx.x] + r1[threadIdx.x + sft];
    }
    __syncthreads();
  }
  if (threadIdx.x == 0) { partial[2 * blockIdx.x] = r0[0]; partial[2 * blockIdx.x + 1] = r1[0]; }
}
__global__ void metric_final_kernel(int mode, const float* __restrict__ partial, int nb, float* __restrict__ out) {
  __shared__ float r0[256], r1[256];
  float a = 0.f, b = mode == 0 ? -3.4e38f : 0.f;
  for (int i = threadIdx.x; i < nb; i += 256) {
    a += partial[2 * i];
    const float v = partial[2 * i + 1];
    b = mode == 0 ? (v > b ? v : b) : b + v;
  }
  r0[threadIdx.x] = a; r1[threadIdx.x] = b;
  __syncthreads();
  for (int sft = 128; sft >= 1; sft >>= 1) {
    if (threadIdx.x < sft) {
      r0[threadIdx.x] += r0[threadIdx.x + sft];
      r1[threadIdx.x] = mode == 0 ? (r1[threadIdx.x] > r1[threadIdx.x + sft] ? r1[threadIdx.x] : r1[threadIdx.x + sft])
                                  : r1[threadIdx.x] + r1[threadIdx.x + sft];
    }
    __syncthreads();
  }
  if (threadIdx.x == 0) { out[0] = r0[0]; out[1] = r1[0]; }
}
hipError_t launch_metric(hipStream_t s, int mode, const float* rec, const float* gt, int64_t count, float thres,
                         float* out, float* partial) {
  if (count <= 0) return hipErrorInvalidValue;
  unsigned nb = cdiv(count, 256);
  if (nb > MET_BLOCKS) nb = MET_BLOCKS;
  hipLaunchKernelGGL(metric_kernel, dim3(nb), dim3(256), 0, s, mode, rec, gt, (long long)count, thres, partial);
  hipLaunchKernelGGL(metric_final_kernel, dim3(1), dim3(256), 0, s, mode, partial, (int)nb, out);
  return hipGetLastError();
}

__global__ void best_copy_kernel(const float* __restrict__ metric, const float* __restrict__ best, int force,
                                 const float* __restrict__ src, float* __restrict__ dst, long long count) {
  if (!(force || metric[0] < best[0])) return;
  const long long i = ((long long)blockIdx.x * blockDim.x + threadIdx.x) * 4;
  if (i + 3 < count) {
    *reinterpret_cast<f32x4*>(dst + i) = *reinterpret_cast<const f32x4*>(src + i);
  } else {
    for (long long j = i; j < count; ++j) dst[j] = src[j];
  }
}
__global__ void best_scalar_kernel(const float* __restrict__ metric, float* __restrict__ best, int force,
                                   int* __restrict__ updated) {
  const bool take = force || metric[0] < best[0];
  if (take) best[0] = metric[0];
  if (updated) updated[0] = take ? 1 : 0;
}
hipError_t launch_track_best(hipStream_t s, const float* metric, float* best, int force, const float* src,
                             float* dst, int64_t count, int* updated) {
  if (count > 0)
    hipLaunchKernelGGL(best_copy_kernel, dim3(cdiv(count, 1024)), dim3(256), 0, s, metric, best, force, src, dst,
                       (long long)count);
  hipLaunchKernelGGL(best_scalar_kernel, dim3(1), dim3(1), 0, s, metric, best, force, updated);
  return hipGetLastError();
}

__global__ void sigmoid_kernel(float* __restrict__ x, long long count) {
  const long long i = (long long)blockIdx.x * blockDim.x + threadIdx.x;
  if (i >= count) return;
  const float v = x[i];
  if (v != v) return;
  const float a = -fminf(fabsf(v), 128.f);
  const float e = a < -64.f ? wire_exp(a + 32.f) * 1.2664165549e-14f : wire_exp(a);
  x[i] = v >= 0.f ? 1.f / (1.f + e) : e / (1.f + e);
}
hipError_t launch_sigmoid(hipStream_t s, float* x, int64_t count) {
  if (count <= 0) return hipSuccess;
  hipLaunchKernelGGL(sigmoid_kernel, dim3(cdiv(count, 256)), dim3(256), 0, s, x, (long long)count);
  return hipGetLastError();
}

template <bool BWD>
__global__ __launch_bounds__(256) void radon_kernel(const float* __restrict__ img, const float* __restrict__ angles,
                                                    int H, int W, int A, float* __restrict__ sino,
                                                    const float* __restrict__ g_sino, float* __restrict__ g_img) {
  const int j = blockIdx.x * blockDim.x + threadIdx.x;
  const int a = blockIdx.y;
  if (j >= W) return;
  const float th = angles[a] * 0.017453292519943295f;
  float sn, cs;
  wire_sincos(th, sn, cs);
  const float cx = 0.5f * (float)(W - 1), cy = 0.5f * (float)(H - 1);
  const float xj = (float)j - cx;
  const float g = BWD ? g_sino[(size_t)a * W + j] : 0.f;
  float acc = 0.f;
  for (int i = 0; i < H; ++i) {
    const float yi = (float)i - cy;
    const float x = __builtin_fmaf(cs, xj, -(sn * yi)) + cx;
    const float y = __builtin_fmaf(sn, xj, cs * yi) + cy;
    const float xf = floorf(x), yf = floorf(y);
    const int x0 = (int)xf, y0 = (int)yf;
    if (x0 < -1 || x0 >= W || y0 < -1 || y0 >= H) continue;
    const float wx1 = x - xf, wy1 = y - yf, wx0 = 1.f - wx1, wy0 = 1.f - wy1;
    const bool vx0 = x0 >= 0, vx1 = x0 + 1 < W, vy0 = y0 >= 0, vy1 = y0 + 1 < H;
    if (!BWD) {
      float v = 0.f;
      if (vy0) {
        const float* r = img + (size_t)y0 * W;
        if (vx0) v += wy0 * wx0 * r[x0];
        if (vx1) v += wy0 * wx1 * r[x0 + 1];
      }
      if (vy1) {
        const float* r = img + (size_t)(y0 + 1) * W;
        if (vx0) v += wy1 * wx0 * r[x0];
        if (vx1) v += wy1 * wx1 * r[x0 + 1];
      }
      acc += v;
    } else {
      if (vy0) {
        float* r = g_img + (size_t)y0 * W;
        if (vx0) atomicAdd(r + x0, g * wy0 * wx0);
        if (vx1) atomicAdd(r + x0 + 1, g * wy0 * wx1);
      }
      if (vy1) {
        float* r = g_img + (size_t)(y0 + 1) * W;
        if (vx0) atomicAdd(r + x0, g * wy1 * wx0);
        if (vx1) atomicAdd(r + x0 + 1, g * wy1 * wx1);
      }
    }
  }
  if (!BWD) sino[(size_t)a * W + j] = acc;
}
hipError_t launch_radon_fwd(hipStream_t s, const float* img, const float* angles, int H, int W, int A, float* sino) {
  dim3 grid(cdiv(W, 256), (unsigned)A);
  hipLaunchKernelGGL(radon_kernel<false>, grid, dim3(256), 0, s, img, angles, H, W, A, sino, nullptr, nullptr);
  return hipGetLastError();
}
hipError_t launch_radon_bwd(hipStream_t s, const float* g_sino, const float* angles, int H, int W, int A,
                            float* g_img) {
  hipError_t e = hipMemsetAsync(g_img, 0, (size_t)H * W * sizeof(float), s);
  if (e != hipSuccess) return e;
  dim3 grid(cdiv(W, 256), (unsigned)A);
  hipLaunchKernelGGL(radon_kernel<true>, grid, dim3(256), 0, s, nullptr, angles, H, W, A, nullptr, g_sino, g_img);
  return hipGetLastError();
}
```

Measured before the change: 46.75 million.

## Fuse edge kernels: merge memsets, copies, and final reductions into fewer launches

Cuts the number of small kernel launches at the start and end of a training step. The two amax memsets become one clear kernel, and native-parameter copies plus the slot clear are folded into the pack kernel. The final-layer gradient prereduce, colreduce and MSE loss finalization are also replaced by single-pass chunked reduction kernels. This trades launch and memset overhead for larger one-block-per-column reductions with 1024 threads, and adds new code paths with coverage conditions that could diverge.

Measured after the change: 46.97 million (median of 6 runs). No clear change (+0.5%).

```diff
diff --git a/wire_amd/csrc/wire_api.hip b/wire_amd/csrc/wire_api.hip
--- a/wire_amd/csrc/wire_api.hip
+++ b/wire_amd/csrc/wire_api.hip
@@ -76,7 +76,7 @@
 }
 
 int pack_hidden(hipStream_t s, const Plan& p, const void* const* params, float* packed, const std::vector<const float*>& hW,
-                const std::vector<const float*>& hb) {
+                const std::vector<const float*>& hb, const PackExtra* extra) {
   for (int l0 = 1; l0 <= p.L; l0 += PACK_MAXB) {
     const int nb = (p.L - l0 + 1) < PACK_MAXB ? (p.L - l0 + 1) : PACK_MAXB;
     PackBatch pb{}, p3{};
@@ -95,6 +95,7 @@
         p3.fwd[i] = packed + p.off_fwd_3m[l]; p3.dg[i] = packed + p.off_dg_3m[l]; p3.bias[i] = packed + p.off_bias[l];
       }
     }
+    if (extra && l0 == 1) pb.x = *extra;
     HIPCHK(launch_pack_hidden_batch(s, p.kind, pb, nb, p.K, p.K, p.P, p.P, p.ws));
     if (p.Pl == p.P) {
       for (int i = 0; i < nb; ++i) { sf.src[nb + i] = sd.src[i]; sf.dst[nb + i] = sd.dst[i]; }
@@ -116,8 +117,13 @@
         xd.src[i] = packed + p.off_dg[l]; xd.dst[i] = packed + p.off_dg_x2[l]; xd.slots[i] = slots;
       }
       HIPCHK(launch_amax_batch(s, ab, nb, (int64_t)p.Pl * p.P));
-      HIPCHK(launch_x2_split_b_batch(s, xf, nb, p.P, p.Pl, p.P));
-      HIPCHK(launch_x2_split_b_batch(s, xd, nb, p.Pl, p.P, p.Pl));
+      if (extra && p.Pl == p.P) {
+        for (int i = 0; i < nb; ++i) { xf.src[nb + i] = xd.src[i]; xf.dst[nb + i] = xd.dst[i]; xf.slots[nb + i] = xd.slots[i]; }
+        HIPCHK(launch_x2_split_b_batch(s, xf, 2 * nb, p.P, p.Pl, p.P));
+      } else {
+        HIPCHK(launch_x2_split_b_batch(s, xf, nb, p.P, p.Pl, p.P));
+        HIPCHK(launch_x2_split_b_batch(s, xd, nb, p.Pl, p.P, p.Pl));
+      }
       for (int k = 0; k < p.S2 && p.off_fx >= 0 && fused_pre_scale(p.kind, p.w, pass_c(p, k)) > 0.f; ++k) {
         FxSplitBatch fx{};
         for (int i = 0; i < nb; ++i) {
@@ -153,7 +159,17 @@
   ProfScope ps(s, 3, 0);
   for (int i = 0; i < p.ntens; ++i)
     if (!params[i]) return fail(WIRE_ERR_ARG, "params[%d] is null", i);
-  HIPCHK(hipMemsetAsync(packed + p.off_wamax, 0, (size_t)(p.L + 1) * WIRE_AMAX_SLOTS * sizeof(float), s));
+  const bool edge = knob(K_EDGE_FUSED) && !p.first_gemm && !p.hier && !p.mfn && !p.m2 && p.L >= 1 && p.per_layer <= 4;
+  PackExtra px{};
+  if (edge) {
+    px.clr = reinterpret_cast<unsigned*>(packed + p.off_wamax); px.nclr = (p.L + 1) * WIRE_AMAX_SLOTS;
+    for (int q = p.ws != 1.f ? 1 : 0; q < p.per_layer; ++q) {
+      px.csrc[q] = (const float*)params[first_tensor(p, q)]; px.cdst[q] = packed + first_native_off(p, q);
+      px.cn[q] = (int)p.tfloats[first_tensor(p, q)];
+    }
+  } else {
+    HIPCHK(hipMemsetAsync(packed + p.off_wamax, 0, (size_t)(p.L + 1) * WIRE_AMAX_SLOTS * sizeof(float), s));
+  }
   if (p.first_gemm) {
     const float* W = (const float*)params[p.t0];
     const float* b = (const float*)params[p.t0 + 1];
@@ -184,7 +200,7 @@
   for (int l = 1; l <= p.L; ++l) {
     hW[l] = (const float*)params[p.t0 + p.per_layer * l]; hb[l] = (const float*)params[p.t0 + p.per_layer * l + 1];
   }
-  if (int rc = pack_hidden(s, p, params, packed, hW, hb)) return rc;
+  if (int rc = pack_hidden(s, p, params, packed, hW, hb, edge ? &px : nullptr)) return rc;
   HIPCHK(launch_pack_final(s, p.kind, (const float*)params[p.ntens - 2],
                            (const float*)params[p.ntens - 1], p.K, p.P, p.O, packed + p.off_wf,
                            packed + p.off_bf));
@@ -195,6 +211,7 @@
                                  packed + first_native_off(p, 0)));
         continue;
       }
+      if (edge) continue;
       HIPCHK(hipMemcpyAsync(packed + first_native_off(p, q), params[first_tensor(p, q)], p.tfloats[first_tensor(p, q)] * 4,
                             hipMemcpyDeviceToDevice, s));
     }
@@ -226,7 +243,8 @@
 }
 
 static int mlp_fwd_core(void* stream, const Plan& p, const Route& r, const float* packed, const float* coords, int64_t n,
-                        float* y, void* act, int64_t act_bytes, const FusedFwdParams* loss = nullptr) {
+                        float* y, void* act, int64_t act_bytes, const FusedFwdParams* loss = nullptr,
+                        bool slots_cleared = false) {
   const bool save = r.mode != MODE_INFER;
   if (n < 0) return fail(WIRE_ERR_ARG, "negative n");
   if (n == 0) return WIRE_OK;
@@ -258,7 +276,7 @@
     return WIRE_OK;
   }
   unsigned* const amax = reinterpret_cast<unsigned*>(A + a.amax);
-  if (r.fam == FAM_X2)
+  if (r.fam == FAM_X2 && !slots_cleared)
     HIPCHK(hipMemsetAsync(amax, 0, (size_t)(p.L + 2 + (p.ms ? 1 : 0)) * WIRE_AMAX_SLOTS * sizeof(unsigned), s));
   unsigned* const pe_amax = reinterpret_cast<unsigned*>(A + a.pe_amax);
   if (p.ms) {
@@ -362,6 +380,7 @@
   const float* A; float* Sx;
   float* gcur = nullptr; float* gnext = nullptr;
   int chain_rows = 0;
+  const FinalTail* tail = nullptr;
 
   const float* out_l(int l) const { return A + a.out0 + (int64_t)l * a.np * p.P; }
   const float* lin_l(int l) const { return l == 0 ? A + a.lin0 : A + a.lin1 + (int64_t)(l - 1) * a.np * p.Pl; }
@@ -400,7 +419,7 @@
   }
   const int nbf = r.fused_final ? (int)((n + 127) / 128) : p.S2 * final_bwd_blocks(n1);
   HIPCHK(launch_final_reduce(s, p.kind, Sx + sc.fpw, Sx + sc.fpb, nbf, p.O, p.K, p.P, grad(p.ntens - 2),
-                             grad(p.ntens - 1)));
+                             grad(p.ntens - 1), tail));
   done(p.ntens - 2, 2);
   return WIRE_OK;
 }
@@ -608,7 +627,7 @@
 static int mlp_bwd_core(void* stream, const Plan& p, const Route& r, const float* packed, const float* coords, int64_t n,
                         const float* g_y, const void* act, int64_t act_bytes, void* scratch, int64_t scratch_bytes,
                         void* const* grads, wire_grad_ready_fn ready = nullptr, void* user = nullptr,
-                        float* g_coords = nullptr, bool comb_done = false) {
+                        float* g_coords = nullptr, bool comb_done = false, const FinalTail* tail = nullptr) {
   if (n <= 0) return fail(WIRE_ERR_ARG, "backward needs n > 0");
   if (!packed || !coords || (!r.fuse && !g_y && !comb_done) || !act || !scratch || (!grads && !g_coords))
     return fail(WIRE_ERR_ARG, "null pointer");
@@ -624,6 +643,7 @@
                                             (long long)scratch_bytes, (long long)need * 4);
   c.gcur = c.Sx + c.sc.ga;
   c.gnext = c.Sx + c.sc.gb;
+  c.tail = tail;
   if (p.m2) {
     ProfScope ps(c.s, 3, 0);
     float* const part = c.Sx + c.sc.cpart;
@@ -751,7 +771,13 @@
   const float* A = (const float*)act;
   float* Sx = (float*)scratch;
   unsigned* const gamax = reinterpret_cast<unsigned*>(Sx + sc.gamax);
-  if (r.fam == FAM_X2) HIPCHK(hipMemsetAsync(gamax, 0, (size_t)(p.L + 2) * WIRE_AMAX_SLOTS * sizeof(unsigned), s));
+  const bool edge = knob(K_EDGE_FUSED) != 0 && final_bwd_blocks(n) > 2 * PRE_CHUNKS;
+  const bool clear2 = edge && r.fam == FAM_X2 && act && act_bytes >= a.total * 4;
+  if (clear2)
+    HIPCHK(launch_clear2(s, gamax, (int64_t)(p.L + 2) * WIRE_AMAX_SLOTS, reinterpret_cast<unsigned*>((float*)act + a.amax),
+                         (int64_t)(p.L + 2 + (p.ms ? 1 : 0)) * WIRE_AMAX_SLOTS));
+  else if (r.fam == FAM_X2) HIPCHK(hipMemsetAsync(gamax, 0, (size_t)(p.L + 2) * WIRE_AMAX_SLOTS * sizeof(unsigned), s));
+  FinalTail tail;
   float* gL = r.chain ? Sx + sc.gch + (int64_t)p.L * sc.gch_stride : Sx + sc.ga;
   FusedFwdParams lp;
   const int fblocks = (int)((n + 127) / 128);
@@ -759,8 +785,10 @@
   lp.target = target; lp.idx = idx; lp.first = first; lp.gscale = (float)(weight * 2.0 * inv_no);
   lp.y = y; lp.rec = rec; lp.g_lin = gL; lp.part_w = Sx + sc.fpw; lp.part_b = Sx + sc.fpb; lp.loss_partial = Sx + sc.crp;
   lp.amax_g = gamax + p.L * WIRE_AMAX_SLOTS;
-  if (int rc = mlp_fwd_core(stream, p, r, packed, coords, n, nullptr, act, act_bytes, &lp)) return rc;
-  if (r.fused_final) {
+  if (int rc = mlp_fwd_core(stream, p, r, packed, coords, n, nullptr, act, act_bytes, &lp, clear2)) return rc;
+  if (r.fused_final && edge) {
+    tail.loss_partial = Sx + sc.crp; tail.nloss = fblocks; tail.lscale = (float)(weight * inv_no); tail.loss_out = loss_out;
+  } else if (r.fused_final) {
     ProfScope ps(s, 3, 0);
     HIPCHK(launch_mse_final(s, Sx + sc.crp, fblocks, (float)(weight * inv_no), loss_out));
   } else {
@@ -769,9 +797,10 @@
     HIPCHK(launch_final_fused(s, p.kind, r.skip_out_L ? nullptr : A + a.out0 + (int64_t)p.L * a.np * p.P, linL, n, p.P,
                               p.O, p.K, packed + p.off_wf, packed + p.off_bf, target, idx, first, weight,
                               p.w, p.s, y, rec, gL, Sx + sc.fpw, Sx + sc.fpb, Sx + sc.crp, loss_out,
-                              r.fam == FAM_X2 ? gamax + p.L * WIRE_AMAX_SLOTS : nullptr));
-  }
-  return mlp_bwd_core(stream, p, r, packed, coords, n, nullptr, act, act_bytes, scratch, scratch_bytes, grads, ready, user);
+                              r.fam == FAM_X2 ? gamax + p.L * WIRE_AMAX_SLOTS : nullptr, edge ? &tail : nullptr));
+  }
+  return mlp_bwd_core(stream, p, r, packed, coords, n, nullptr, act, act_bytes, scratch, scratch_bytes, grads, ready, user,
+                      nullptr, false, edge ? &tail : nullptr);
 }
 extern "C" int wire_train_fwd_bwd(void* stream, const wire_net_desc* d, const float* packed,
                                   const float* coords, int64_t n, const float* target, const int64_t* idx,
diff --git a/wire_amd/csrc/wire_final.hip b/wire_amd/csrc/wire_final.hip
--- a/wire_amd/csrc/wire_final.hip
+++ b/wire_amd/csrc/wire_final.hip
@@ -474,7 +474,7 @@
                               int kvalid, const float* wf, const float* bfr, const float* target, const int64_t* idx,
                               int64_t first, float weight, float omega, float scale, float* y, float* rec,
                               float* g_lin, float* part_w, float* part_b, float* loss_partial,
-                              float* loss_out, unsigned* amax_g) {
+                              float* loss_out, unsigned* amax_g, FinalTail* tail) {
   if (n <= 0) return hipSuccess;
   if (!final_fused_supported(P, O)) return hipErrorInvalidValue;
   if (!out && kind == NK_RELU) return hipErrorInvalidValue;
@@ -486,7 +486,7 @@
     if (rows_pb > FF_MAXROWS) rows_pb = FF_MAXROWS;
   }
   const int nblk = (int)((n + rows_pb - 1) / rows_pb);
-  if (nblk < nbf) {
+  if (nblk < nbf && !tail) {
     hipError_t e = hipMemsetAsync(part_w + (size_t)nblk * O * P, 0, (size_t)(nbf - nblk) * O * P * sizeof(float), s);
     if (e == hipSuccess) e = hipMemsetAsync(part_b + (size_t)nblk * O, 0, (size_t)(nbf - nblk) * O * sizeof(float), s);
     if (e != hipSuccess) return e;
@@ -515,5 +515,9 @@
 #undef FF_LAUNCH_K
 #undef FF_LAUNCH_O
 #undef FF_LAUNCH
+  if (tail) {
+    tail->nw = nblk; tail->loss_partial = loss_partial; tail->nloss = nblk; tail->lscale = weight * inv; tail->loss_out = loss_out;
+    return hipGetLastError();
+  }
   return launch_mse_final(s, loss_partial, nblk, weight * inv, loss_out);
 }
diff --git a/wire_amd/csrc/wire_knobs.h b/wire_amd/csrc/wire_knobs.h
--- a/wire_amd/csrc/wire_knobs.h
+++ b/wire_amd/csrc/wire_knobs.h
@@ -5,7 +5,7 @@
   K_COMPLEX_3M, K_SPLIT_BF16, K_SPLIT_F16, K_SPLIT_OUT, K_RECOMPUTE_OUT, K_FIRST_SUMS, K_FIRST_DN, K_BWD_LOOKAHEAD, K_FUSED_RSTORE, K_WGRAD_BATCH,
   K_FUSED_FWD, K_FUSED_TRAIN, K_FUSED_TRAIN_P384, K_FUSED_FINAL, K_FUSED_BWD, K_FUSED_BWD_W,
   K_NT_BK, K_X2_AMODE, K_NT_BFIRST, K_EPI_EARLY, K_X2_TN_ROWS, K_X2_TN_P384, K_X3_TALL, K_X3_TALL_REAL, K_X3_TN_TALL, K_X3_TN16, K_X3_H16,
-  K_X3H_STAGGER,
+  K_X3H_STAGGER, K_EDGE_FUSED,
   K_FX_ABLATE, K_FXB_ABLATE, K_TN_ABL,
   K_COUNT
 };
diff --git a/wire_amd/csrc/wire_knobs.hip b/wire_amd/csrc/wire_knobs.hip
--- a/wire_amd/csrc/wire_knobs.hip
+++ b/wire_amd/csrc/wire_knobs.hip
@@ -62,6 +62,7 @@
     range_knob(K_X3_TN16, "x3_tn16", "WIRE_X3_TN16", 1, 0, 1),
     range_knob(K_X3_H16, "x3_h16", "WIRE_X3_H16", 15, 0, 15),
     range_knob(K_X3H_STAGGER, "x3h_stagger", "WIRE_X3H_STAGGER", 0, 0, INT_MAX),
+    flag_knob(K_EDGE_FUSED, "edge_fused", "WIRE_EDGE_FUSED", 1),
     range_knob(K_FX_ABLATE, FX_ABLATE_KEY("fx_ablate"), nullptr, 0, 0, 15),
     range_knob(K_FXB_ABLATE, FX_ABLATE_KEY("fxb_ablate"), nullptr, 0, 0, 127),
     range_knob(K_TN_ABL, nullptr, "WIRE_TN_ABL", 0, 0, 15),
diff --git a/wire_amd/csrc/wire_pack.hip b/wire_amd/csrc/wire_pack.hip
--- a/wire_amd/csrc/wire_pack.hip
+++ b/wire_amd/csrc/wire_pack.hip
@@ -52,6 +52,13 @@
 template <bool WS>
 __global__ void pack_hidden_batch_kernel(int kind, PackBatch pb, int K, int Kin, int P, int Pin, int Nc, float ws) {
   const int z = blockIdx.z;
+  if (pb.x.nclr > 0) {
+    const int nthr = gridDim.x * gridDim.y * gridDim.z * blockDim.x;
+    const int t0 = ((blockIdx.z * gridDim.y + blockIdx.y) * gridDim.x + blockIdx.x) * blockDim.x + threadIdx.x;
+    for (int i = t0; i < pb.x.nclr; i += nthr) pb.x.clr[i] = 0u;
+    for (int q = 0; q < 4; ++q)
+      for (int i = t0; i < pb.x.cn[q]; i += nthr) pb.x.cdst[q][i] = pb.x.csrc[q][i];
+  }
   pack_hidden_body<WS>(kind, pb.W[z], pb.b[z], pb.V[z], pb.c[z], K, Kin, P, Pin, Nc, pb.fwd[z], pb.dg[z], pb.bias[z], ws);
 }
 hipError_t launch_pack_hidden_batch(hipStream_t s, int kind, const PackBatch& pb, int nb, int K, int Kin, int P,
diff --git a/wire_amd/csrc/wire_plan.h b/wire_amd/csrc/wire_plan.h
--- a/wire_amd/csrc/wire_plan.h
+++ b/wire_amd/csrc/wire_plan.h
@@ -203,7 +203,7 @@
 HierScratch hier_scratch(const Plan& p, int64_t n);
 Route hier_route(const Plan& p, int64_t n, RouteMode mode);
 int pack_hidden(hipStream_t s, const Plan& p, const void* const* params, float* packed, const std::vector<const float*>& hW,
-                const std::vector<const float*>& hb);
+                const std::vector<const float*>& hb, const PackExtra* extra = nullptr);
 int hier_pack(hipStream_t s, const Plan& p, const void* const* params, float* packed);
 int hier_fwd_core(void* stream, const Plan& p, const Route& r, const float* packed, const float* coords, int64_t n, float* y,
                   void* act, int64_t act_bytes, const M2Loss* loss = nullptr, float* loss_part = nullptr);
diff --git a/wire_amd/csrc/wire_point.h b/wire_amd/csrc/wire_point.h
--- a/wire_amd/csrc/wire_point.h
+++ b/wire_amd/csrc/wire_point.h
@@ -15,9 +15,14 @@
                               const float* V, const float* c, int K, int Kin, int P, int Pin,
                               float* Bt_fwd, float* Bt_dgrad, float* bias, float wscale = 1.f);
 #define PACK_MAXB 16
+struct PackExtra {
+  unsigned* clr; int nclr;
+  const float* csrc[4]; float* cdst[4]; int cn[4];
+};
 struct PackBatch {
   const float* W[PACK_MAXB]; const float* b[PACK_MAXB]; const float* V[PACK_MAXB]; const float* c[PACK_MAXB];
   float* fwd[PACK_MAXB]; float* dg[PACK_MAXB]; float* bias[PACK_MAXB];
+  PackExtra x;
 };
 hipError_t launch_pack_hidden_batch(hipStream_t s, int kind, const PackBatch& pb, int nb, int K, int Kin, int P,
                                     int Pin, float wscale = 1.f);
@@ -61,10 +66,15 @@
                               int kvalid, const float* wf, const float* bfr, const float* target, const int64_t* idx,
                               int64_t first, float weight, float omega, float scale, float* y, float* rec,
                               float* g_lin, float* part_w, float* part_b, float* loss_partial,
-                              float* loss_out, unsigned* amax_g = nullptr);
-
+                              float* loss_out, unsigned* amax_g = nullptr,
+                              struct FinalTail* tail = nullptr);
+
+struct FinalTail {
+  int nw = -1;
+  const float* loss_partial = nullptr; int nloss = 0; float lscale = 0.f; float* loss_out = nullptr;
+};
 hipError_t launch_final_reduce(hipStream_t s, int kind, float* part_w, float* part_b,
-                               int nblk, int O, int K, int P, float* gWf, float* gbf);
+                               int nblk, int O, int K, int P, float* gWf, float* gbf, const FinalTail* tail = nullptr);
 
 hipError_t launch_wgrad_reduce(hipStream_t s, int kind, const float* slab, const float* bslab,
                                int S, int K, int Kin, int Pm, int Pn, float* gW, float* gb,
@@ -116,6 +126,7 @@
                          const float* tx, int W, const float* ty, int H, const float* tz, int T,
                          float* coords);
 hipError_t launch_mse_final(hipStream_t s, const float* partial, int nb, float lscale, float* loss_out);
+hipError_t launch_clear2(hipStream_t s, unsigned* a, int64_t na, unsigned* b, int64_t nb);
 hipError_t launch_mse_grad(hipStream_t s, const float* y, const float* target, const int64_t* idx,
                            int64_t first, int64_t n, int O, float weight, float* g_y,
                            float* loss_out, float* rec, float* partial);
diff --git a/wire_amd/csrc/wire_reduce.hip b/wire_amd/csrc/wire_reduce.hip
--- a/wire_amd/csrc/wire_reduce.hip
+++ b/wire_amd/csrc/wire_reduce.hip
@@ -1,5 +1,6 @@
 #include "wire_dev.h"
 #include "wire_point.h"
+#include "wire_knobs.h"
 
 __global__ __launch_bounds__(256) void prereduce_kernel(const float* __restrict__ in, int nblk, int C, int per,
                                                         float* __restrict__ out) {
@@ -65,8 +66,108 @@
   }
 }
 
+WIRE_DEVINL float pre_chunk_sum(const float* __restrict__ in, int C, int c, int b0, int b1, int nw) {
+  float a0 = 0.f, a1 = 0.f, a2 = 0.f, a3 = 0.f;
+  int b = b0;
+  for (; b + 3 < b1; b += 4) {
+    a0 += b < nw ? in[(size_t)b * C + c] : 0.f;
+    a1 += b + 1 < nw ? in[(size_t)(b + 1) * C + c] : 0.f;
+    a2 += b + 2 < nw ? in[(size_t)(b + 2) * C + c] : 0.f;
+    a3 += b + 3 < nw ? in[(size_t)(b + 3) * C + c] : 0.f;
+  }
+  for (; b < b1; ++b) a0 += b < nw ? in[(size_t)b * C + c] : 0.f;
+  return (a0 + a1) + (a2 + a3);
+}
+#define RT_COLS 32
+#define RT_LANES 32
+static_assert(RT_LANES >= PRE_CHUNKS && RT_COLS * RT_LANES == 1024, "one chunk per lane, 1024 threads");
+
+__global__ __launch_bounds__(1024) void final_tail_kernel(int kind, const float* __restrict__ part_w,
+                                  const float* __restrict__ part_b, int nblk, int nw, int per, int nch, int O, int K, int P,
+                                  float* __restrict__ gWf, float* __restrict__ gbf, const float* __restrict__ loss_partial,
+                                  int nloss, float lscale, float* __restrict__ loss_out) {
+  __shared__ float ch[2][RT_LANES][RT_COLS];
+  __shared__ float red[2][4][RT_COLS];
+  const int tx = threadIdx.x & (RT_COLS - 1), ty = threadIdx.x / RT_COLS;
+  const int o = blockIdx.y;
+  const bool cplx = (kind == NK_WIRE || kind == NK_WIRE2D);
+  if (blockIdx.x == gridDim.x - 1) {
+    float* const flat = &ch[0][0][0];
+    if (threadIdx.x < nch) {
+      const int b0 = threadIdx.x * per;
+      flat[threadIdx.x] = pre_chunk_sum(part_b, O, o, b0, b0 + per < nblk ? b0 + per : nblk, nw);
+    }
+    __syncthreads();
+    if (threadIdx.x == 0) {
+      float sb = 0.f;
+      for (int b = 0; b < nch; ++b) sb += flat[b];
+      if (cplx) { gbf[2 * o] = sb; gbf[2 * o + 1] = 0.f; } else gbf[o] = sb;
+    }
+    if (o != 0 || !loss_out) return;
+    __syncthreads();
+    float acc = 0.f;
+    if (threadIdx.x < 256) {
+      for (int i = threadIdx.x; i < nloss; i += 256) acc += loss_partial[i];
+      flat[threadIdx.x] = acc;
+    }
+    __syncthreads();
+    for (int sft = 128; sft >= 1; sft >>= 1) {
+      if (threadIdx.x < sft) flat[threadIdx.x] += flat[threadIdx.x + sft];
+      __syncthreads();
+    }
+    if (threadIdx.x == 0) loss_out[0] = flat[0] * lscale;
+    return;
+  }
+  const int i = blockIdx.x * RT_COLS + tx;
+  const int c = cplx ? blk_col(i, 0) : i;
+  const int C = O * P;
+  float sr = 0.f, si = 0.f, cr = 0.f, ci = 0.f;
+  if (i < K && ty < nch) {
+    const int b0 = ty * per, b1 = b0 + per < nblk ? b0 + per : nblk;
+    cr = pre_chunk_sum(part_w, C, o * P + c, b0, b1, nw);
+    if (cplx) ci = pre_chunk_sum(part_w, C, o * P + c + 32, b0, b1, nw);
+  }
+  ch[0][ty][tx] = cr;
+  ch[1][ty][tx] = ci;
+  __syncthreads();
+  if (ty < 4 && i < K)
+    for (int b = ty; b < nch; b += 4) {
+      sr += ch[0][b][tx];
+      if (cplx) si += ch[1][b][tx];
+    }
+  if (ty < 4) { red[0][ty][tx] = sr; red[1][ty][tx] = si; }
+  __syncthreads();
+  if (ty == 0 && i < K) {
+    sr = (red[0][0][tx] + red[0][1][tx]) + (red[0][2][tx] + red[0][3][tx]);
+    si = (red[1][0][tx] + red[1][1][tx]) + (red[1][2][tx] + red[1][3][tx]);
+    if (cplx) {
+      gWf[((size_t)o * K + i) * 2] = sr;
+      gWf[((size_t)o * K + i) * 2 + 1] = -si;
+    } else {
+      gWf[(size_t)o * K + i] = sr;
+    }
+  }
+}
+
+static void pre_chunks(int nblk, int& per, int& nch) {
+  per = 0; nch = 0;
+  if (nblk <= 2 * PRE_CHUNKS) return;
+  per = (nblk + PRE_CHUNKS - 1) / PRE_CHUNKS;
+  nch = (nblk + per - 1) / per;
+}
+
 hipError_t launch_final_reduce(hipStream_t s, int kind, float* part_w, float* part_b,
-                               int nblk, int O, int K, int P, float* gWf, float* gbf) {
+                               int nblk, int O, int K, int P, float* gWf, float* gbf, const FinalTail* tail) {
+  int per, nch;
+  pre_chunks(nblk, per, nch);
+  if (tail && nch == 0) return hipErrorInvalidValue;
+  if (tail || (nch > 0 && knob(K_EDGE_FUSED))) {
+    const int nw = tail && tail->nw >= 0 && tail->nw < nblk ? tail->nw : nblk;
+    hipLaunchKernelGGL(final_tail_kernel, dim3(cdiv(K, RT_COLS) + 1, (unsigned)O), dim3(1024), 0, s, kind, part_w, part_b,
+                       nblk, nw, per, nch, O, K, P, gWf, gbf, tail ? tail->loss_partial : nullptr, tail ? tail->nloss : 0,
+                       tail ? tail->lscale : 0.f, tail ? tail->loss_out : nullptr);
+    return hipGetLastError();
+  }
   float* w2 = part_w + (size_t)nblk * O * P;
   float* b2 = part_b + (size_t)nblk * O;
   const int nw = prereduce(s, part_w, nblk, O * P, w2);
@@ -235,9 +336,50 @@
                                   float wscale) {
   return launch_colreduce_final_blocks(s, C, D, colreduce_blocks(n), partial, gW0, gb0, wscale);
 }
+template <bool WS>
+__global__ __launch_bounds__(1024) void colreduce_tail_kernel(const float* __restrict__ partial, int nblk, int per,
+                                                               int nch, int C, int D, float* __restrict__ gW0,
+                                                               float* __restrict__ gb0, float ws) {
+  __shared__ float ch[RT_LANES][RT_COLS];
+  __shared__ float red[4][RT_COLS];
+  const int tx = threadIdx.x & (RT_COLS - 1), ty = threadIdx.x / RT_COLS;
+  const int f = blockIdx.x * RT_COLS + tx, F = C * 5;
+  float cs = 0.f;
+  if (f < F && ty < nch) {
+    const int b0 = ty * per;
+    cs = pre_chunk_sum(partial, F, f, b0, b0 + per < nblk ? b0 + per : nblk, nblk);
+  }
+  ch[ty][tx] = cs;
+  __syncthreads();
+  if (ty < 4) {
+    float acc = 0.f;
+    if (f < F)
+      for (int b = ty; b < nch; b += 4) acc += ch[b][tx];
+    red[ty][tx] = acc;
+  }
+  __syncthreads();
+  if (ty == 0 && f < F) {
+    const float acc = (red[0][tx] + red[1][tx]) + (red[2][tx] + red[3][tx]);
+    const int c = f / 5, d = f - c * 5;
+    if (d == 4) gb0[c] = acc;
+    else if (d < D) gW0[c * D + d] = WS ? ws * acc : acc;
+  }
+}
+
 hipError_t launch_colreduce_final_blocks(hipStream_t s, int C, int D, int nblk, float* partial, float* gW0, float* gb0,
                                          float wscale) {
   if (D > 4 || nblk < 1) return hipErrorInvalidValue;
+  int per, nch;
+  pre_chunks(nblk, per, nch);
+  if (knob(K_EDGE_FUSED) && nch > 0) {
+    if (wscale != 1.f)
+      hipLaunchKernelGGL(colreduce_tail_kernel<true>, dim3(cdiv(C * 5, RT_COLS)), dim3(1024), 0, s, partial, nblk, per, nch, C, D,
+                         gW0, gb0, wscale);
+    else
+      hipLaunchKernelGGL(colreduce_tail_kernel<false>, dim3(cdiv(C * 5, RT_COLS)), dim3(1024), 0, s, partial, nblk, per, nch, C,
+                         D, gW0, gb0, 1.f);
+    return hipGetLastError();
+  }
   float* p2 = partial + (size_t)nblk * C * 5;
   const int nb = prereduce(s, partial, nblk, C * 5, p2);
   if (wscale != 1.f)
diff --git a/wire_amd/csrc/wire_train.hip b/wire_amd/csrc/wire_train.hip
--- a/wire_amd/csrc/wire_train.hip
+++ b/wire_amd/csrc/wire_train.hip
@@ -70,6 +70,17 @@
   if (n <= 0) return hipSuccess;
   hipLaunchKernelGGL(coords_kernel, dim3(cdiv(n, 256)), dim3(256), 0, s, idx, (long long)first,
                      (long long)n, tx, W, ty, H, tz, T, coords);
+  return hipGetLastError();
+}
+
+__global__ void clear2_kernel(unsigned* __restrict__ a, long long na, unsigned* __restrict__ b, long long nb) {
+  const long long i = (long long)blockIdx.x * blockDim.x + threadIdx.x;
+  if (i < na) a[i] = 0u;
+  else if (i - na < nb) b[i - na] = 0u;
+}
+hipError_t launch_clear2(hipStream_t s, unsigned* a, int64_t na, unsigned* b, int64_t nb) {
+  if (na + nb <= 0) return hipSuccess;
+  hipLaunchKernelGGL(clear2_kernel, dim3(cdiv(na + nb, 256)), dim3(256), 0, s, a, (long long)na, b, (long long)nb);
   return hipGetLastError();
 }
 
```
